# Vegeta2020/SE-SSD

Measured on AMD Instinct MI355X. Metric: KITTI frames/sec (voxelize->backbone->head->NMS), higher is better.
Workload: dtype f32

## Files before the change

### se-ssd_amd/csrc/dense_conv.hip

```cpp
#include "common.hpp"
#include "sessd_hip_types.h"

namespace {

using f32x16 = __attribute__((ext_vector_type(16))) float;

struct ConvArgs {
  const float* in;
  const float* wpk;
  float* out;
  const float* scale;
  const float* shift;
  const float* residual;
  int cin, hin, win;
  int cout, cout_pad, hout, wout;
  int ht, wt;
  int in_mul, out_mul, out_py, out_px;
  int relu;
  int cgroup;
  int dy[9], dx[9];
  int dc[9];
  const int* tile_list;
  const int* n_list;
  int list_cap, ntiles2, tw2, lbatch;
// ... 610 lines not shown
      }
    }
  }
}

template <int NTAPS, int CT, int PT, int WC, int WP, bool DEEP = false>
int launch_conv(const ConvArgs* A, int nconv, int batch, hipStream_t stream) {
  const int npix = A[0].ht * A[0].wt;
  dim3 grid(sessd_divup(npix, WP * PT * 32) * sessd_divup(A[0].cout_pad, WC * CT * 32), 1, batch * (nconv > 1 ? 4 : 1));
  if (nconv == 1) {
    SESSD_LAUNCH((conv2d_mfma_kernel<NTAPS, CT, PT, WC, WP, DEEP>), grid, dim3(256), 0, stream, A[0]);
  } else {
    ConvArgs4 A4;
    for (int i = 0; i < 4; ++i) A4.c[i] = A[i];
    SESSD_LAUNCH((conv2d_mfma4_kernel<NTAPS, CT, PT, WC, WP, DEEP>), grid, dim3(256), 0, stream, A4);
  }
  SESSD_CHECK_LAUNCH();
  return SESSD_OK;
}

template <int CT, int PT, int WC, int WP, bool DEEP>
int launch_conv8(const ConvArgs* A, int batch, hipStream_t stream) {
  const int npix = A[0].ht * A[0].wt;
  const bool list = A[0].tile_list != nullptr;
  dim3 grid(sessd_divup(npix * (list ? batch : 1), WP * PT * 32) * sessd_divup(A[0].cout_pad, WC * CT * 32), 1, (list ? 1 : batch) * 8);
  ConvArgs8 A8;
  for (int i = 0; i < 8; ++i) A8.c[i] = A[i];
  if (list)
    SESSD_LAUNCH((conv2d_mfma8_kernel<4, CT, PT, WC, WP, DEEP, true>), grid, dim3(256), 0, stream, A8);
  else
    SESSD_LAUNCH((conv2d_mfma8_kernel<4, CT, PT, WC, WP, DEEP>), grid, dim3(256), 0, stream, A8);
  SESSD_CHECK_LAUNCH();
  return SESSD_OK;
}

template <int CT, int PT, int WC, int WP, bool DEEP>
int launch_conv_list(const ConvArgs& A, int batch, hipStream_t stream) {
  const int npix = A.ht * A.wt;
  dim3 grid(sessd_divup(npix * batch, WP * PT * 32) * sessd_divup(A.cout_pad, WC * CT * 32), 1, 1);
  SESSD_LAUNCH((conv2d_mfma_kernel<4, CT, PT, WC, WP, DEEP, true>), grid, dim3(256), 0, stream, A);
  SESSD_CHECK_LAUNCH();
  return SESSD_OK;
}

template <int NTAPS>
int dispatch_tile(const ConvArgs* A, int nconv, int batch, int tile_cfg, hipStream_t stream) {
  switch (tile_cfg) {
    case 0: return launch_conv<NTAPS, 2, 2, 2, 2>(A, nconv, batch, stream);
    case 1: return launch_conv<NTAPS, 2, 1, 2, 2>(A, nconv, batch, stream);
    case 2: return launch_conv<NTAPS, 1, 2, 4, 1>(A, nconv, batch, stream);
    case 3: return launch_conv<NTAPS, 1, 1, 4, 1>(A, nconv, batch, stream);
    case 4: return launch_conv<NTAPS, 1, 1, 1, 4>(A, nconv, batch, stream);
    case 5: return launch_conv<NTAPS, 2, 1, 4, 1>(A, nconv, batch, stream);
    case 6: return launch_conv<NTAPS, 2, 1, 1, 4>(A, nconv, batch, stream);
    case 7: return launch_conv<NTAPS, 2, 2, 1, 4>(A, nconv, batch, stream);
    case 8: return launch_conv<NTAPS, 4, 1, 1, 4>(A, nconv, batch, stream);
    case 11: return launch_conv<NTAPS, 1, 1, 1, 4, true>(A, nconv, batch, stream);
    case 12: return launch_conv<NTAPS, 1, 1, 4, 1, true>(A, nconv, batch, stream);
    case 13: if (nconv == 1) return launch_conv<NTAPS, 1, 2, 4, 1, true>(A, nconv, batch, stream); return SESSD_EINVAL;
    default: return SESSD_EINVAL;
  }
}

inline bool out_fits(int cout, int hout, int wout) { return (long long)cout * hout * wout * 4 < 0x7fffffffLL; }

int fill_args(ConvArgs& A, const float* in, int cin, int hin, int win, const float* wpk, int ntaps, const int* dy,
              const int* dx, int in_mul, int tile_h, int tile_w, float* out, int cout, int hout, int wout, int out_mul,
              int py, int px, const float* scale, const float* shift, int relu, const float* residual) {
  A.in = in; A.wpk = wpk; A.out = out; A.scale = scale; A.shift = shift; A.residual = residual;
  A.cin = cin; A.hin = hin; A.win = win;
  A.cout = cout; A.cout_pad = sessd_divup(cout, 32) * 32; A.hout = hout; A.wout = wout;
  A.ht = tile_h; A.wt = tile_w;
  A.in_mul = in_mul; A.out_mul = out_mul; A.out_py = py; A.out_px = px;
  A.relu = relu;
  A.tile_list = nullptr; A.n_list = nullptr; A.list_cap = 0; A.ntiles2 = 1; A.tw2 = 1; A.lbatch = 1;
  int group = 1;
  const int pairs = cin / 2;
  if (ntaps == 1 && pairs % 4 == 0) group = 4;
  else if (ntaps == 2 && pairs % 2 == 0) group = 2;
  A.cgroup = group;
  const int eff = ntaps * group;
  for (int v = 0; v < 9; ++v) {
    const int t = v < eff ? v % ntaps : 0, g = v < eff ? v / ntaps : 0;
    A.dy[v] = dy[t]; A.dx[v] = dx[t]; A.dc[v] = g;
  }
  return eff;
}

}

extern "C" {

int sessd_conv2d_mfma(const float* in, int batch, int cin, int hin, int win, const float* wpk, int ntaps,
                      const int* taps_dy, const int* taps_dx, int in_mul, int tile_h, int tile_w, float* out, int cout,
                      int hout, int wout, int out_mul, int out_py, int out_px, const float* scale, const float* shift,
                      int relu, const float* residual, int tile_cfg, hipStream_t stream) {
  if (cin % 2 || ntaps < 1 || ntaps > 9 || batch < 1 || cout < 1 || !out_fits(cout, hout, wout)) return SESSD_EINVAL;
  ConvArgs A;
  const int eff = fill_args(A, in, cin, hin, win, wpk, ntaps, taps_dy, taps_dx, in_mul, tile_h, tile_w, out, cout, hout,
                            wout, out_mul, out_py, out_px, scale, shift, relu, residual);
  if (tile_cfg == 10) {
    if (eff != 9 || in_mul != 1 || out_mul != 1 || cin % 16 || hin != tile_h || win != tile_w) return SESSD_EINVAL;
    dim3 grid(sessd_divup(tile_h * tile_w, 32), sessd_divup(A.cout_pad, 128), batch);
    SESSD_LAUNCH(conv3x3s1_lds_kernel, grid, dim3(256), 0, stream, A);
    SESSD_CHECK_LAUNCH();
    return SESSD_OK;
  }
  switch (eff) {
    case 1: return dispatch_tile<1>(&A, 1, batch, tile_cfg, stream);
    case 2: return dispatch_tile<2>(&A, 1, batch, tile_cfg, stream);
    case 4: return dispatch_tile<4>(&A, 1, batch, tile_cfg, stream);
    case 9: return dispatch_tile<9>(&A, 1, batch, tile_cfg, stream);
    default: return SESSD_EINVAL;
  }
}

int sessd_conv3x3_winograd(const float* in, int batch, int cin, int h, int w, const float* upk, float* out, int cout,
                           const float* scale, const float* shift, int relu, const float* residual, int variant,
                           hipStream_t stream) {
  if (cin % 8 || (h & 1) || (w & 1) || batch < 1 || cout < 1) return SESSD_EINVAL;
  if (variant < 0 || variant > 1 || (variant == 1 && cin % 32)) return SESSD_EINVAL;
  ConvArgs A;
  const int z9[9] = {0, 0, 0, 0, 0, 0, 0, 0, 0};
  fill_args(A, in, cin, h, w, upk, 9, z9, z9, 1, h, w, out, cout, h, w, 1, 0, 0, scale, shift, relu, residual);
  const int ntiles = (h / 2) * (w / 2);
  dim3 grid(sessd_divup(ntiles, 32) * sessd_divup(A.cout_pad, 32), 1, batch);
  if (variant == 1)
    SESSD_LAUNCH(conv3x3s1_winograd_kernel<true>, grid, dim3(256), 0, stream, A);
  else
    SESSD_LAUNCH(conv3x3s1_winograd_kernel<false>, grid, dim3(256), 0, stream, A);
  SESSD_CHECK_LAUNCH();
  return SESSD_OK;
}

}
namespace {
struct PackArgs {
  const float* w;
  long long so, sc;
  int tap_off[16];
  int co, ci, nt, cp;
};
__global__ __launch_bounds__(256) void pack_taps_kernel(PackArgs A, float* __restrict__ out) {
  const size_t total = (size_t)(A.ci >> 1) * A.nt * 2 * A.cp;
  const size_t idx = (size_t)blockIdx.x * 256 + threadIdx.x;
  if (idx >= total) return;
  const int o = (int)(idx % A.cp);
  size_t r = idx / A.cp;
  const int h = (int)(r & 1); r >>= 1;
  const int t = (int)(r % A.nt);
  const int kp = (int)(r / A.nt);
  out[idx] = o < A.co ? A.w[(long long)o * A.so + (long long)(2 * kp + h) * A.sc + A.tap_off[t]] : 0.f;
}
__device__ __forceinline__ void winograd_pack_body(const PackArgs& A, int flip, int layout, float* __restrict__ out, size_t idx) {
  const int cpad = layout == 0 ? A.cp : ((layout == 1 || layout == 3) ? (A.co + 127) / 128 * 128 : (A.co + 63) / 64 * 64);
  if (idx >= (size_t)cpad * A.ci) return;
  const int o = (int)(idx % cpad), c = (int)(idx / cpad);
  double g[3][3];
#pragma unroll
  for (int a = 0; a < 3; ++a)
#pragma unroll
    for (int b = 0; b < 3; ++b) {
      const int t = flip ? 8 - (3 * a + b) : 3 * a + b;
      g[a][b] = o < A.co ? (double)A.w[(long long)o * A.so + (long long)c * A.sc + t] : 0.0;
    }
  double t0[4][3];
#pragma unroll
  for (int b = 0; b < 3; ++b) {
    t0[0][b] = g[0][b];
    t0[1][b] = 0.5 * g[0][b] + 0.5 * g[1][b] + 0.5 * g[2][b];
    t0[2][b] = 0.5 * g[0][b] - 0.5 * g[1][b] + 0.5 * g[2][b];
    t0[3][b] = g[2][b];
  }
  const int kp = c >> 1, h = c & 1;
#pragma unroll
  for (int a = 0; a < 4; ++a) {
    const double u[4] = {t0[a][0], 0.5 * t0[a][0] + 0.5 * t0[a][1] + 0.5 * t0[a][2], 0.5 * t0[a][0] - 0.5 * t0[a][1] + 0.5 * t0[a][2],
                         t0[a][2]};
#pragma unroll
    for (int b = 0; b < 4; ++b) {
      const int xi = a * 4 + b;
      size_t dst;
      if (layout == 0) {
        dst = ((((size_t)kp * 4 + (xi >> 2)) * 2 + h) * cpad + o) * 4 + (xi & 3);
      } else if (layout == 1) {
        const int grp = o >> 7, cb = (o >> 5) & 3, j = o & 31, wave = xi >> 1, xl = xi & 1;
        dst = ((((((size_t)grp * (A.ci >> 1) + kp) * 8 + wave) * 2 + h) * 32 + j) * 4 + cb) * 2 + xl;
      } else if (layout == 3) {
        const int grp = o >> 7, wave = (o >> 5) & 3, j = o & 31;
        dst = (((((size_t)grp * (A.ci >> 1) + kp) * 4 + wave) * 2 + h) * 32 + j) * 16 + xi;
      } else {
        const int grp = o >> 6, cb = (o >> 5) & 1, j = o & 31, wave = xi >> 2, xl = xi & 3;
        dst = ((((((size_t)grp * (A.ci >> 1) + kp) * 4 + wave) * 2 + h) * 32 + j) * 2 + cb) * 4 + xl;
      }
      out[dst] = (float)u[b];
    }
  }
}
__global__ __launch_bounds__(256) void winograd_pack_kernel(PackArgs A, int flip, int layout, float* __restrict__ out) {
  winograd_pack_body(A, flip, layout, out, (size_t)blockIdx.x * 256 + threadIdx.x);
}
__global__ __launch_bounds__(256) void dense_pack_batch_kernel(const sessd_dense_pack_job_t* __restrict__ jobs, int n) {
  int lo = 0, hi = n - 1;
  while (lo < hi) {
    const int mid = (lo + hi + 1) >> 1;
    if (jobs[mid].block_start <= (int)blockIdx.x) lo = mid; else hi = mid - 1;
  }
  const sessd_dense_pack_job_t* J = jobs + lo;
  const size_t idx = (size_t)((int)blockIdx.x - J->block_start) * 256 + threadIdx.x;
  const int co = J->cout, ci = J->cin, cp = sessd_divup(co, 32) * 32;
  const float* __restrict__ w = J->w;
  float* __restrict__ out = J->out;
  const long long so = J->out_stride, sc = J->in_stride;
  if (J->kind == 0) {
    const int nt = J->ntaps;
    const size_t total = (size_t)(ci >> 1) * nt * 2 * cp;
    if (idx >= total) return;
    const int o = (int)(idx % cp);
    size_t r = idx / cp;
    const int h = (int)(r & 1); r >>= 1;
    const int t = (int)(r % nt);
    const int kp = (int)(r / nt);
    out[idx] = o < co ? w[(long long)o * so + (long long)(2 * kp + h) * sc + J->tap_off[t]] : 0.f;
    return;
  }
  PackArgs A;
  A.w = w; A.so = so; A.sc = sc; A.co = co; A.ci = ci; A.nt = 9; A.cp = cp;
  winograd_pack_body(A, J->flip, J->layout, out, idx);
}
}
extern "C" {

int sessd_dense_pack_batch(const sessd_dense_pack_job_t* jobs_dev, int n_jobs, int total_blocks, hipStream_t stream) {
  if (!jobs_dev || n_jobs < 1 || total_blocks < 1) return SESSD_EINVAL;
  SESSD_LAUNCH(dense_pack_batch_kernel, dim3(total_blocks), dim3(256), 0, stream, jobs_dev, n_jobs);
  SESSD_CHECK_LAUNCH();
  return SESSD_OK;
}

int sessd_conv2d_pack_taps(const float* w, long long out_stride, long long in_stride, const int* tap_offsets, int ntaps, int cout,
                           int cin, float* out, hipStream_t stream) {
  if (ntaps < 1 || ntaps > 16 || cout < 1 || cin < 2 || (cin & 1)) return SESSD_EINVAL;
  PackArgs A;
  A.w = w; A.so = out_stride; A.sc = in_stride; A.co = cout; A.ci = cin; A.nt = ntaps; A.cp = sessd_divup(cout, 32) * 32;
  for (int t = 0; t < 16; ++t) A.tap_off[t] = t < ntaps ? tap_offsets[t] : 0;
  const size_t total = (size_t)(cin >> 1) * ntaps * 2 * A.cp;
  SESSD_LAUNCH(pack_taps_kernel, dim3((unsigned)((total + 255) / 256)), dim3(256), 0, stream, A, out);
  SESSD_CHECK_LAUNCH();
  return SESSD_OK;
}

int sessd_conv3x3_winograd_pack(const float* w, long long out_stride, long long in_stride, int flip, int cout, int cin, int layout,
                                float* out, hipStream_t stream) {
  if (cout < 1 || cin < 2 || (cin & 1) || layout < 0 || layout > 3) return SESSD_EINVAL;
  PackArgs A;
  A.w = w; A.so = out_stride; A.sc = in_stride; A.co = cout; A.ci = cin; A.nt = 9; A.cp = sessd_divup(cout, 32) * 32;
  for (int t = 0; t < 16; ++t) A.tap_off[t] = 0;
  const int cpad = layout == 0 ? A.cp : ((layout == 1 || layout == 3) ? sessd_divup(cout, 128) * 128 : sessd_divup(cout, 64) * 64);
  const size_t total = (size_t)cpad * cin;
  SESSD_LAUNCH(winograd_pack_kernel, dim3((unsigned)((total + 255) / 256)), dim3(256), 0, stream, A, flip, layout, out);
  SESSD_CHECK_LAUNCH();
  return SESSD_OK;
}

}
int sessd_deconv_pair_launch(const float* in, int batch, int cin, int hin, int win, const float* const* wpk4, float* out, int cout,
                             const float* scale, const float* shift, int relu, const float* residual, int variant,
                             hipStream_t stream);
extern "C" {

int sessd_deconv2d_s2_mfma(const float* in, int batch, int cin, int hin, int win, const float* const* wpk4,
                           const int* ntaps4, const int* taps_dy4, const int* taps_dx4, float* out, int cout,
                           const float* scale, const float* shift, int relu, const float* residual, int tile_cfg,
                           hipStream_t stream) {
  if (cin % 8 || batch < 1 || cout < 1 || !out_fits(cout, 2 * hin, 2 * win)) return SESSD_EINVAL;
  if (tile_cfg >= 40 && tile_cfg <= 42) {
    static const int nt[4] = {1, 2, 2, 4};
    static const int dy[16] = {0, 0, 0, 0, 0, 0, 0, 0, 1, 0, 0, 0, 1, 1, 0, 0};
    static const int dx[16] = {0, 0, 0, 0, 1, 0, 0, 0, 0, 0, 0, 0, 1, 0, 1, 0};
    for (int c = 0; c < 4; ++c) {
      if (ntaps4[c] != nt[c]) return SESSD_EINVAL;
      for (int t = 0; t < nt[c]; ++t)
        if (taps_dy4[4 * c + t] != dy[4 * c + t] || taps_dx4[4 * c + t] != dx[4 * c + t]) return SESSD_EINVAL;
    }
    return sessd_deconv_pair_launch(in, batch, cin, hin, win, wpk4, out, cout, scale, shift, relu, residual, tile_cfg - 40, stream);
  }
  ConvArgs A[4];
  for (int c = 0; c < 4; ++c) {
    const int eff = fill_args(A[c], in, cin, hin, win, wpk4[c], ntaps4[c], taps_dy4 + 4 * c, taps_dx4 + 4 * c, 1, hin, win,
                              out, cout, 2 * hin, 2 * win, 2, c >> 1, c & 1, scale, shift, relu, residual);
    if (eff != 4) return SESSD_EINVAL;
  }
  return dispatch_tile<4>(A, 4, batch, tile_cfg, stream);
}

int sessd_deconv2d_s2_mfma_pair(const float* in, int batch, int cin, int hin, int win, const float* const* wpk4_a,
                                const float* const* wpk4_b, const int* ntaps4, const int* taps_dy4, const int* taps_dx4,
                                float* out_a, float* out_b, int cout, const float* scale_a, const float* shift_a,
                                const float* scale_b, const float* shift_b, int relu, const float* residual_a,
                                const float* residual_b, int tile_cfg, hipStream_t stream) {
  if (cin % 8 || batch < 1 || cout < 1 || !out_fits(cout, 2 * hin, 2 * win)) return SESSD_EINVAL;
  ConvArgs A[8];
  for (int c = 0; c < 4; ++c)
    for (int l = 0; l < 2; ++l) {
      const int eff = fill_args(A[2 * c + l], in, cin, hin, win, (l ? wpk4_b : wpk4_a)[c], ntaps4[c], taps_dy4 + 4 * c, taps_dx4 + 4 * c,
                                1, hin, win, l ? out_b : out_a, cout, 2 * hin, 2 * win, 2, c >> 1, c & 1, l ? scale_b : scale_a,
                                l ? shift_b : shift_a, relu, l ? residual_b : residual_a);
      if (eff != 4) return SESSD_EINVAL;
    }
  switch (tile_cfg) {
    case 3: return launch_conv8<1, 1, 4, 1, false>(A, batch, stream);
    case 4: return launch_conv8<1, 1, 1, 4, false>(A, batch, stream);
    case 11: return launch_conv8<1, 1, 1, 4, true>(A, batch, stream);
    case 12: return launch_conv8<1, 1, 4, 1, true>(A, batch, stream);
    default: return SESSD_EINVAL;
  }
}

int sessd_conv2d_mfma_active(const float* in, int batch, int cin, int hin, int win, const float* wpk, int ntaps, const int* taps_dy,
                             const int* taps_dx, int in_mul, int tile_h, int tile_w, float* out, int cout, int hout, int wout,
                             int out_mul, int out_py, int out_px, const float* scale, const float* shift, int relu,
                             const float* residual, const int32_t* tile_list, const int32_t* n_list, int list_cap, int tile_cfg,
                             hipStream_t stream) {
  if (cin % 2 || ntaps < 1 || ntaps > 9 || batch < 1 || cout < 1 || !tile_list || !n_list || list_cap < 1 || (tile_h & 1) || (tile_w & 1))
    return SESSD_EINVAL;
  if ((long long)batch * cout * hout * wout * 4 >= 0x7fffffffLL || (long long)batch * cin * hin * win * 4 >= 0x7fffffffLL) return SESSD_EINVAL;
  ConvArgs A;
  const int eff = fill_args(A, in, cin, hin, win, wpk, ntaps, taps_dy, taps_dx, in_mul, tile_h, tile_w, out, cout, hout, wout, out_mul,
                            out_py, out_px, scale, shift, relu, residual);
  if (eff != 4) return SESSD_EINVAL;
  A.tile_list = tile_list; A.n_list = n_list; A.list_cap = list_cap; A.ntiles2 = (tile_h / 2) * (tile_w / 2); A.tw2 = tile_w / 2;
  A.lbatch = batch;
  switch (tile_cfg) {
    case 3: return launch_conv_list<1, 1, 4, 1, false>(A, batch, stream);
    case 4: return launch_conv_list<1, 1, 1, 4, false>(A, batch, stream);
    case 11: return launch_conv_list<1, 1, 1, 4, true>(A, batch, stream);
    case 12: return launch_conv_list<1, 1, 4, 1, true>(A, batch, stream);
    default: return SESSD_EINVAL;
  }
}

int sessd_deconv2d_s2_mfma_pair_active(const float* in, int batch, int cin, int hin, int win, const float* const* wpk4_a,
                                       const float* const* wpk4_b, const int* ntaps4, const int* taps_dy4, const int* taps_dx4,
                                       float* out_a, float* out_b, int cout, const float* scale_a, const float* shift_a,
                                       const float* scale_b, const float* shift_b, int relu, const float* residual_a,
                                       const float* residual_b, const int32_t* tile_list, const int32_t* n_list, int list_cap,
                                       int tile_cfg, hipStream_t stream) {
  if (cin % 8 || batch < 1 || cout < 1 || !tile_list || !n_list || list_cap < 1 || (hin & 1) || (win & 1)) return SESSD_EINVAL;
  if ((long long)batch * cout * 4 * hin * win * 4 >= 0x7fffffffLL || (long long)batch * cin * hin * win * 4 >= 0x7fffffffLL) return SESSD_EINVAL;
  ConvArgs A[8];
  for (int c = 0; c < 4; ++c)
    for (int l = 0; l < 2; ++l) {
      ConvArgs& C = A[2 * c + l];
      const int eff = fill_args(C, in, cin, hin, win, (l ? wpk4_b : wpk4_a)[c], ntaps4[c], taps_dy4 + 4 * c, taps_dx4 + 4 * c, 1, hin, win,
                                l ? out_b : out_a, cout, 2 * hin, 2 * win, 2, c >> 1, c & 1, l ? scale_b : scale_a,
                                l ? shift_b : shift_a, relu, l ? residual_b : residual_a);
      if (eff != 4) return SESSD_EINVAL;
      C.tile_list = tile_list; C.n_list = n_list; C.list_cap = list_cap; C.ntiles2 = (hin / 2) * (win / 2); C.tw2 = win / 2;
      C.lbatch = batch;
    }
  switch (tile_cfg) {
    case 3: return launch_conv8<1, 1, 4, 1, false>(A, batch, stream);
    case 4: return launch_conv8<1, 1, 1, 4, false>(A, batch, stream);
    case 11: return launch_conv8<1, 1, 1, 4, true>(A, batch, stream);
    case 12: return launch_conv8<1, 1, 4, 1, true>(A, batch, stream);
    default: return SESSD_EINVAL;
  }
}

int sessd_ssfa_fuse(const float* x0, const float* x1, const float* w0, const float* w1, float bn_scale0,
                    float bn_shift0, float bn_scale1, float bn_shift1, int batch, int channels, int num_pixels,
                    float* out, hipStream_t stream) {
  if (batch < 1 || channels < 1 || num_pixels < 1) return SESSD_EINVAL;
  if (channels % 4) return SESSD_EINVAL;
  SESSD_LAUNCH(ssfa_fuse_kernel, dim3(sessd_divup(num_pixels, 64), batch), dim3(256), 0, stream, x0, x1, w0, w1,
                     bn_scale0, bn_shift0, bn_scale1, bn_shift1, channels, num_pixels, out);
  SESSD_CHECK_LAUNCH();
  return SESSD_OK;
}


int sessd_ssfa_fuse_head_keys(const float* x0, const float* x1, const float* w0, const float* w1, float bn_scale0, float bn_shift0,
                              float bn_scale1, float bn_shift1, int batch, int channels, int num_pixels, float* out,
                              const float* head_w, const float* head_b, int nout, float* head_out, float score_thresh,
                              unsigned long long* keys, int key_cap, int* key_count, hipStream_t stream) {
  if (batch < 1 || (channels != 128 && channels != 64) || num_pixels < 1 || nout != 22) return SESSD_EINVAL;
  if ((long long)channels * num_pixels * 4 >= 0x7fffffffLL) return SESSD_EINVAL;
  if ((keys == nullptr) != (key_count == nullptr) || (keys && key_cap < 1)) return SESSD_EINVAL;
  const dim3 grid(sessd_divup(num_pixels, 64), batch);
  if (channels == 128)
    SESSD_LAUNCH((ssfa_fuse_head_kernel<22, 32>), grid, dim3(256), 0, stream, x0, x1, w0, w1, bn_scale0, bn_shift0, bn_scale1,
                 bn_shift1, num_pixels, out, head_w, head_b, head_out, score_thresh, keys, key_cap, key_count);
  else
    SESSD_LAUNCH((ssfa_fuse_head_kernel<22, 16>), grid, dim3(256), 0, stream, x0, x1, w0, w1, bn_scale0, bn_shift0, bn_scale1,
                 bn_shift1, num_pixels, out, head_w, head_b, head_out, score_thresh, keys, key_cap, key_count);
  SESSD_CHECK_LAUNCH();
  return SESSD_OK;
}

int sessd_ssfa_fuse_head(const float* x0, const float* x1, const float* w0, const float* w1, float bn_scale0, float bn_shift0,
                         float bn_scale1, float bn_shift1, int batch, int channels, int num_pixels, float* out,
                         const float* head_w, const float* head_b, int nout, float* head_out, hipStream_t stream) {
  return sessd_ssfa_fuse_head_keys(x0, x1, w0, w1, bn_scale0, bn_shift0, bn_scale1, bn_shift1, batch, channels, num_pixels, out,
                                   head_w, head_b, nout, head_out, 0.f, nullptr, 0, nullptr, stream);
}

}
```

### se-ssd_amd/csrc/dense_wino_sk.hip

```cpp
#include <cstdlib>
#include "common.hpp"

namespace {

using f32x16 = __attribute__((ext_vector_type(16))) float;
using f32x4v = __attribute__((ext_vector_type(4))) float;
using f32x2v = __attribute__((ext_vector_type(2))) float;
typedef unsigned int u32x4g __attribute__((__vector_size__(16)));

typedef __amdgpu_buffer_rsrc_t rsrc_t;
__device__ __forceinline__ rsrc_t make_rsrc(const void* base, unsigned bytes) {
  return __builtin_amdgcn_make_buffer_rsrc(const_cast<void*>(base), (short)0, (int)bytes, 0x00020000);
}
#define SESSD_OOB 0x80000000u
#define SESSD_LDS_BARRIER() asm volatile("s_waitcnt lgkmcnt(0)\n\ts_barrier" ::: "memory")
#define SESSD_SYSTEM_SCOPE 17

__device__ __forceinline__ float sadd(float a, float b) {
  float r;
  asm volatile("v_add_f32 %0, %1, %2" : "=v"(r) : "v"(a), "v"(b));
  return r;
}

struct WinoArgs {
  const float* in;
  const float* upk;
  float* out;
  const float* scale;
  const float* shift;
  const float* residual;
  float* scratch;
  unsigned* counters;
  int cin, hin, win, cout, relu;
  int tw, ntiles, tblocks, ngroups, rpu, total_rounds;
  int bper;
  int ss_stride;
  long long upk_stride;
  const int* tile_list;
  const int* n_list;
  int list_cap, min_rounds, batch;
};

template <int NW, int CBN, int VAR = 0, bool LIST = false>
__global__ __launch_bounds__(NW * 64, 8 / NW) void conv3x3s1_winograd_sk_kernel(WinoArgs A) {
  constexpr int XW = 16 / NW;
  static_assert(XW * CBN == 8, "8 accumulators per wave");
  constexpr int NT = NW * 64;
  constexpr unsigned WSTEP = NW * 2u * 32u * 32u;
  constexpr int VBUF = NW * 1024;
  constexpr int SLOT = CBN * 32 * 32 * 4;
  constexpr int NPT = 1024 / NT;
  constexpr int RING = NW;
  __shared__ __attribute__((aligned(16))) float lds[16384];
  __shared__ int s_last, s_pend;
  const int tid = threadIdx.x, lane = tid & 63;
  const int wave = __builtin_amdgcn_readfirstlane(tid >> 6);
  const int j = lane & 31, h = lane >> 5;
  int G = gridDim.x;
  long long R = A.total_rounds;
  int n_list = 0;
  if constexpr (LIST) {
    n_list = __builtin_amdgcn_readfirstlane(min(A.n_list[0], A.list_cap));
    R = (long long)((n_list + 31) >> 5) * A.ngroups * A.rpu;
    if (R == 0) return;
    if (A.min_rounds < 0) {
      const long long U = R / A.rpu;
      long long g = U / (-A.min_rounds);
      g = g < 1 ? 1 : (g > G ? G : g);
      G = (int)g;
      if ((int)blockIdx.x >= G) return;
    } else {
      long long g = R / A.min_rounds;
      g = g < 1 ? 1 : (g > G ? G : g);
      G = (int)(g >= 8 ? (g & ~7LL) : g);
      if ((G & 7) ? ((int)blockIdx.x >= G) : ((int)(blockIdx.x >> 3) >= (G >> 3))) return;
    }
  }
  const bool whole_units = LIST && A.min_rounds < 0;
  const int w = (whole_units || (G & 7)) ? (int)blockIdx.x : (int)((blockIdx.x & 7) * (G >> 3) + (blockIdx.x >> 3));
  int r = whole_units ? (int)((long long)w * (R / A.rpu) / G) * A.rpu : (int)((long long)w * R / G);
  const int r_stop = whole_units ? (int)((long long)(w + 1) * (R / A.rpu) / G) * A.rpu : (int)((long long)(w + 1) * R / G);
  const int in_plane = A.hin * A.win;
  const size_t out_plane = (size_t)in_plane;
  const unsigned xstep = 2u * (unsigned)in_plane * 4u;
  const unsigned wo = (unsigned)(((wave * 2 + h) * 32 + j) * 32);

  int pend_state = 0, pend_u = 0, pend_first = 0, pend_last = 0, pend_tbase = 0, pend_mbase = 0, pend_b = 0;
#define SESSD_SK_SIGNAL()                                                                          \
  {                                                                                                \
    __builtin_amdgcn_s_waitcnt(0);                                                                 \
    __syncthreads();                                                                               \
    if (tid == 0) {                                                                                \
      const unsigned old = __hip_atomic_fetch_add(A.counters + pend_u, 1u, __ATOMIC_RELAXED, __HIP_MEMORY_SCOPE_AGENT); \
      s_pend = (old == (unsigned)(pend_last - pend_first)) ? 1 : 0;                                \
    }                                                                                              \
    __syncthreads();                                                                               \
    pend_state = s_pend ? 2 : 0;                                                                   \
  }

#define SESSD_SK_FINALIZE(Y, CO, SC, SH)                                                            \
  if (tok && (CO) < e_cout) {                                                                       \
    _Pragma("unroll") for (int a = 0; a < 2; ++a) {                                                 \
      const size_t o = (size_t)(CO) * out_plane + pix + (size_t)a * e_win;                          \
      float v0 = fmaf((Y)[2 * a], (SC), (SH)), v1 = fmaf((Y)[2 * a + 1], (SC), (SH));              \
      if (e_relu) { v0 = fmaxf(v0, 0.f); v1 = fmaxf(v1, 0.f); }                                 \
      if (resb) { v0 += resb[o]; v1 += resb[o + 1]; }                                               \
      *reinterpret_cast<float2*>(outb + o) = make_float2(v0, v1);                                   \
    }                                                                                               \
  }
#define SESSD_SK_FINISH_PENDING()                                                                  \
  {                                                                                                \
    const __attribute__((address_space(4))) WinoArgs* Fp =                                         \
        (const __attribute__((address_space(4))) WinoArgs*)__builtin_amdgcn_kernarg_segment_ptr(); \
    asm volatile("" : "+s"(Fp));                                                                   \
    const int f_set = pend_b / Fp->bper;                                                           \
    const float* f_scale = Fp->scale ? Fp->scale + (size_t)f_set * Fp->ss_stride : nullptr;        \
    const float* f_shift = Fp->shift ? Fp->shift + (size_t)f_set * Fp->ss_stride : nullptr;        \
    const int e_cout = Fp->cout, e_relu = Fp->relu, e_win = Fp->win, f_tw = Fp->tw;                \
    const rsrc_t fr = make_rsrc(Fp->scratch, (unsigned)(2 * G) * SLOT * 4u);                       \
    float* outb = Fp->out + (size_t)pend_b * e_cout * out_plane;                                   \
    const float* resb = Fp->residual ? Fp->residual + (size_t)pend_b * e_cout * out_plane : nullptr; \
    const int tl = tid & 31, col0 = tid >> 5;                                                      \
    int tt = pend_tbase + tl;                                                                      \
    bool tok = tt < Fp->ntiles;                                                                    \
    size_t pix = 0;                                                                                \
    if constexpr (LIST) {                                                                          \
      const int fe = tt < n_list ? Fp->tile_list[tt] : -1;                                         \
      tok = fe >= 0;                                                                               \
      const int fb = tok ? fe / Fp->ntiles : 0;                                                    \
      tt = tok ? fe - fb * Fp->ntiles : 0;                                                         \
      pix = (size_t)fb * e_cout * out_plane;                                                       \
    }                                                                                              \
    const int oty = tok ? tt / f_tw : 0, otx = tok ? tt - (tt / f_tw) * f_tw : 0;                  \
    pix += (size_t)(2 * oty) * e_win + 2 * otx;                                                    \
    _Pragma("unroll 1") for (int cb = 0; cb < CBN; ++cb) {                                         \
      f32x4v ysum[NPT];                                                                            \
      _Pragma("unroll") for (int n = 0; n < NPT; ++n) ysum[n] = 0.f;                               \
      for (int wq = pend_first; wq <= pend_last; ++wq) {                                           \
        const unsigned slot = (unsigned)(2 * wq + (wq == pend_first ? 1 : 0)) * (unsigned)(SLOT * 4); \
        f32x4v p[NPT];                                                                             \
        _Pragma("unroll") for (int n = 0; n < NPT; ++n)                                            \
          p[n] = __builtin_bit_cast(f32x4v, __builtin_amdgcn_raw_buffer_load_b128(                 \
              fr, (int)(slot + (unsigned)(((cb * 32 + col0 + (NT / 32) * n) * 32 + tl) * 16)), 0, SESSD_SYSTEM_SCOPE)); \
        _Pragma("unroll") for (int n = 0; n < NPT; ++n) ysum[n] += p[n];                           \
      }                                                                                            \
      _Pragma("unroll") for (int n = 0; n < NPT; ++n) {                                            \
        const int co = pend_mbase + cb * 32 + col0 + (NT / 32) * n;                                \
        const float scv = (f_scale && co < e_cout) ? f_scale[co] : 1.f, shv = (f_shift && co < e_cout) ? f_shift[co] : 0.f; \
        const float z[4] = {ysum[n].x, ysum[n].y, ysum[n].z, ysum[n].w};                           \
        SESSD_SK_FINALIZE(z, co, scv, shv)                                                         \
      }                                                                                            \
    }                                                                                              \
    if (tid == 0) __hip_atomic_store(Fp->counters + pend_u, 0u, __ATOMIC_RELAXED, __HIP_MEMORY_SCOPE_AGENT); \
    pend_state = 0;                                                                                \
  }

  while (r < r_stop) {
    const int u = __builtin_amdgcn_readfirstlane(r / A.rpu);
    const int r0 = __builtin_amdgcn_readfirstlane(r - u * A.rpu);
    const int r1 = __builtin_amdgcn_readfirstlane(min(r_stop - u * A.rpu, A.rpu));
    r = u * A.rpu + r1;
    const int cg = __builtin_amdgcn_readfirstlane(u % A.ngroups), ub = u / A.ngroups;
    const int tb = LIST ? __builtin_amdgcn_readfirstlane(ub) : __builtin_amdgcn_readfirstlane(ub % A.tblocks);
    const int b = LIST ? 0 : __builtin_amdgcn_readfirstlane(ub / A.tblocks);
    const int t_base = tb * 32, m_base = cg * (CBN * 32);
    const rsrc_t xr = LIST ? make_rsrc(A.in, (unsigned)A.batch * (unsigned)A.cin * (unsigned)in_plane * 4u)
                           : make_rsrc(A.in + (size_t)b * A.cin * in_plane, (unsigned)A.cin * in_plane * 4u);
    const int wset = LIST ? 0 : __builtin_amdgcn_readfirstlane(b / A.bper);
    const rsrc_t wr = make_rsrc(A.upk + (size_t)wset * A.upk_stride + (size_t)cg * (A.cin >> 1) * (WSTEP / 4), (unsigned)(A.cin >> 1) * WSTEP);

    int t = t_base + j;
    bool tlive = t < A.ntiles;
    unsigned img_off = 0;
    if constexpr (LIST) {
      const int e = t < n_list ? A.tile_list[t] : -1;
      tlive = e >= 0;
      const int bl = tlive ? e / A.ntiles : 0;
      t = tlive ? e - bl * A.ntiles : 0;
      img_off = (unsigned)bl * (unsigned)A.cin * (unsigned)in_plane * 4u;
    }
    const int ty = tlive ? t / A.tw : 0, tx = tlive ? t - (t / A.tw) * A.tw : 0;
    const int y0 = 2 * ty - 1, x0 = 2 * tx - 1;
    unsigned ro[4];
#pragma unroll
    for (int q = 0; q < 4; ++q) {
      const int y = y0 + q;
      ro[q] = (tlive && y >= 0 && y < A.hin) ? img_off + (unsigned)((h * in_plane + y * A.win + max(x0, 0)) * 4) : SESSD_OOB;
    }
    const bool mask_l = (tx == 0), mask_r = (tx == A.tw - 1);
    const bool edge = __builtin_amdgcn_ballot_w64(tlive && (mask_l || mask_r)) != 0;
    const int klast = r1 * NW - 1;

    f32x16 acc[XW][CBN];
#pragma unroll
    for (int x = 0; x < XW; ++x)
#pragma unroll
      for (int c = 0; c < CBN; ++c)
#pragma unroll
        for (int q = 0; q < 16; ++q) acc[x][c][q] = 0.f;
    f32x4v pr[4];
    f32x4v ua[RING][2];
    float bv[2][XW];

#define SESSD_SK_LOADP(ROUND)                                                                      \
  {                                                                                                \
    const unsigned xs = (unsigned)(min((ROUND), r1 - 1) * NW + wave) * xstep;                      \
    _Pragma("unroll") for (int q = 0; q < 4; ++q)                                                  \
      pr[q] = __builtin_bit_cast(f32x4v, __builtin_amdgcn_raw_buffer_load_b128(xr, (int)ro[q], (int)xs, 0)); \
  }
#define SESSD_SK_LOADU(SET, KG)                                                                    \
  {                                                                                                \
    const unsigned ws = (unsigned)min((KG), klast) * WSTEP;                                        \
    ua[SET][0] = __builtin_bit_cast(f32x4v, __builtin_amdgcn_raw_buffer_load_b128(wr, (int)wo, (int)ws, 0));        \
    __builtin_amdgcn_sched_barrier(0);                                                             \
    ua[SET][1] = __builtin_bit_cast(f32x4v, __builtin_amdgcn_raw_buffer_load_b128(wr, (int)(wo + 16u), (int)ws, 0)); \
  }
#define SESSD_SK_TRANSFORM(VOFF)                                                                   \
  {                                                                                                \
    if (edge) {                                                                                    \
      _Pragma("unroll") for (int q = 0; q < 4; ++q) {                                              \
        const f32x4v p = pr[q];                                                                    \
        pr[q].x = mask_l ? 0.f : p.x; pr[q].y = mask_l ? p.x : p.y;                                \
        pr[q].z = mask_l ? p.y : p.z; pr[q].w = mask_l ? p.z : (mask_r ? 0.f : p.w);               \
      }                                                                                            \
    }                                                                                              \
    f32x2v tl[4], tr[4];                                                                           \
    if constexpr (VAR & 1) {                                                                       \
      tl[0].x = sadd(pr[0].x, -pr[2].x); tl[0].y = sadd(pr[0].y, -pr[2].y); tr[0].x = sadd(pr[0].z, -pr[2].z); tr[0].y = sadd(pr[0].w, -pr[2].w); \
      tl[1].x = sadd(pr[1].x, pr[2].x); tl[1].y = sadd(pr[1].y, pr[2].y); tr[1].x = sadd(pr[1].z, pr[2].z); tr[1].y = sadd(pr[1].w, pr[2].w); \
      tl[2].x = sadd(pr[2].x, -pr[1].x); tl[2].y = sadd(pr[2].y, -pr[1].y); tr[2].x = sadd(pr[2].z, -pr[1].z); tr[2].y = sadd(pr[2].w, -pr[1].w); \
      tl[3].x = sadd(pr[1].x, -pr[3].x); tl[3].y = sadd(pr[1].y, -pr[3].y); tr[3].x = sadd(pr[1].z, -pr[3].z); tr[3].y = sadd(pr[1].w, -pr[3].w); \
    } else {                                                                                       \
    tl[0] = pr[0].xy - pr[2].xy; tr[0] = pr[0].zw - pr[2].zw;                                      \
    tl[1] = pr[1].xy + pr[2].xy; tr[1] = pr[1].zw + pr[2].zw;                                      \
    tl[2] = pr[2].xy - pr[1].xy; tr[2] = pr[2].zw - pr[1].zw;                                      \
    tl[3] = pr[1].xy - pr[3].xy; tr[3] = pr[1].zw - pr[3].zw;                                      \
    }                                                                                              \
    float* dst = &lds[(VOFF) + wave * 1024 + h * 32 + j];                                          \
    _Pragma("unroll") for (int a = 0; a < 4; ++a) {                                                \
      dst[(a * 4 + 0) * 64] = tl[a].x - tr[a].x;                                                   \
      dst[(a * 4 + 1) * 64] = tl[a].y + tr[a].x;                                                   \
      dst[(a * 4 + 2) * 64] = tr[a].x - tl[a].y;                                                   \
      dst[(a * 4 + 3) * 64] = tl[a].y - tr[a].y;                                                   \
    }                                                                                              \
  }
#define SESSD_SK_READV(P, KS, VOFF)                                                                \
  {                                                                                                \
    const float* vb = &lds[(VOFF) + (KS)*1024 + wave * (XW * 64) + h * 32 + j];                    \
    _Pragma("unroll") for (int x = 0; x < XW; ++x) bv[P][x] = vb[x * 64];                          \
  }
#define SESSD_SK_MMA(SET, P)                                                                       \
  {                                                                                                \
    if constexpr (VAR & 2) __builtin_amdgcn_s_setprio(3);                                          \
    _Pragma("unroll") for (int c = 0; c < CBN; ++c)                                                \
      _Pragma("unroll") for (int x = 0; x < XW; ++x)                                               \
        acc[x][c] = __builtin_amdgcn_mfma_f32_32x32x2f32(ua[SET][(c * XW + x) >> 2][(c * XW + x) & 3], bv[P][x], acc[x][c], 0, 0, 0); \
    if constexpr (VAR & 2) __builtin_amdgcn_s_setprio(0);                                          \
  }
#define SESSD_SK_STEP(KS)                                                                          \
  {                                                                                                \
    SESSD_SK_LOADU(((KS) + RING - 1) & (RING - 1), kg0 + (KS) + RING - 1)                          \
    if ((KS) < NW - 1) SESSD_SK_READV(((KS) + 1) & 1, (KS) + 1, voff)                              \
    __builtin_amdgcn_sched_barrier(0);                                                             \
    SESSD_SK_MMA((KS) & (RING - 1), (KS) & 1)                                                      \
    __builtin_amdgcn_sched_barrier(0);                                                             \
  }
#define SESSD_SK_ROUND()                                                                           \
  {                                                                                                \
    const int kg0 = rr * NW;                                                                       \
    SESSD_SK_LOADP(rr + 1)                                                                         \
    SESSD_SK_READV(0, 0, voff)                                                                     \
    __builtin_amdgcn_sched_barrier(0);                                                             \
    SESSD_SK_STEP(0)                                                                               \
    SESSD_SK_STEP(1)                                                                               \
    SESSD_SK_STEP(2)                                                                               \
    SESSD_SK_STEP(3)                                                                               \
    if constexpr (NW == 8) {                                                                       \
      SESSD_SK_STEP(4)                                                                             \
      SESSD_SK_STEP(5)                                                                             \
      SESSD_SK_STEP(6)                                                                             \
      SESSD_SK_STEP(7)                                                                             \
    }                                                                                              \
    SESSD_SK_TRANSFORM(voff ^ VBUF)                                                                \
    __syncthreads();                                                                               \
    voff ^= VBUF;                                                                                  \
    ++rr;                                                                                          \
  }

    SESSD_SK_LOADP(r0)
    __builtin_amdgcn_sched_barrier(0);
#pragma unroll
    for (int s = 0; s < RING - 1; ++s) {
      SESSD_SK_LOADU(s, r0 * NW + s)
      __builtin_amdgcn_sched_barrier(0);
    }
    SESSD_SK_TRANSFORM(0)
    __syncthreads();
    if (pend_state == 1) {
      if (tid == 0) {
        const unsigned old = __hip_atomic_fetch_add(A.counters + pend_u, 1u, __ATOMIC_RELAXED, __HIP_MEMORY_SCOPE_AGENT);
        s_pend = (old == (unsigned)(pend_last - pend_first)) ? 1 : 0;
      }
      pend_state = 3;
    }
    int voff = 0;
    int rr = r0;
    while (rr < r1) SESSD_SK_ROUND()
#undef SESSD_SK_LOADP
#undef SESSD_SK_LOADU
#undef SESSD_SK_TRANSFORM
#undef SESSD_SK_READV
#undef SESSD_SK_MMA
#undef SESSD_SK_STEP
#undef SESSD_SK_ROUND

    if (pend_state == 3) {
      SESSD_LDS_BARRIER();
      pend_state = s_pend ? 2 : 0;
    }
    const __attribute__((address_space(4))) WinoArgs* Ep =
        (const __attribute__((address_space(4))) WinoArgs*)__builtin_amdgcn_kernarg_segment_ptr();
    asm volatile("" : "+s"(Ep));
    const float* e_scale = Ep->scale ? Ep->scale + (size_t)wset * Ep->ss_stride : nullptr;
    const float* e_shift = Ep->shift ? Ep->shift + (size_t)wset * Ep->ss_stride : nullptr;
    const int e_cout = Ep->cout, e_relu = Ep->relu, e_win = Ep->win, e_tw = Ep->tw, e_ntiles = Ep->ntiles;
    unsigned* e_counter = Ep->counters + u;
    const rsrc_t sr = make_rsrc(Ep->scratch, (unsigned)(2 * G) * SLOT * 4u);
    const bool full = (r0 == 0 && r1 == Ep->rpu);
    float* outb = Ep->out + (size_t)b * e_cout * out_plane;
    const float* resb = Ep->residual ? Ep->residual + (size_t)b * e_cout * out_plane : nullptr;
    const int tl = tid & 31, col0 = tid >> 5;
    int tt = t_base + tl;
    bool tok = tt < e_ntiles;
    size_t pix = 0;
    if constexpr (LIST) {
      const int ee = tt < n_list ? Ep->tile_list[tt] : -1;
      tok = ee >= 0;
      const int eb = tok ? ee / e_ntiles : 0;
      tt = tok ? ee - eb * e_ntiles : 0;
      pix = (size_t)eb * e_cout * out_plane;
    }
    const int oty = tok ? tt / e_tw : 0, otx = tok ? tt - (tt / e_tw) * e_tw : 0;
    pix += (size_t)(2 * oty) * e_win + 2 * otx;
    const int w_first = (int)((((long long)u * Ep->rpu + 1) * G - 1) / R);
    const int w_last = (int)((((long long)u * Ep->rpu + Ep->rpu) * G - 1) / R);
    const unsigned my_slot = (unsigned)(2 * w + (r0 == 0 ? 1 : 0)) * (unsigned)(SLOT * 4);
    bool certain = false;
    unsigned oslot = 0;
    if (!full && w_last == w_first + 1) {
      if (tid == 0) s_last = __hip_atomic_load(e_counter, __ATOMIC_RELAXED, __HIP_MEMORY_SCOPE_AGENT) == 1u ? 1 : 0;
      __syncthreads();
      certain = s_last != 0;
      const int wq = (w == w_first) ? w_last : w_first;
      oslot = (unsigned)(2 * wq + (wq == w_first ? 1 : 0)) * (unsigned)(SLOT * 4);
    }
    const bool writes_out = full || certain;
    f32x4v onext[NPT];
    float scn[NPT], shn[NPT];
#define SESSD_SK_FETCH(CB)                                                                          \
  _Pragma("unroll") for (int n = 0; n < NPT; ++n) {                                                 \
    const int co_ = m_base + (CB)*32 + col0 + (NT / 32) * n;                                        \
    if (certain)                                                                                    \
      onext[n] = __builtin_bit_cast(                                                                \
          f32x4v, __builtin_amdgcn_raw_buffer_load_b128(                                            \
                      sr, (int)(oslot + (unsigned)((((CB)*32 + col0 + (NT / 32) * n) * 32 + tl) * 16)), 0, SESSD_SYSTEM_SCOPE)); \
    else                                                                                            \
      onext[n] = 0.f;                                                                               \
    scn[n] = (writes_out && e_scale && co_ < e_cout) ? e_scale[co_] : 1.f;                          \
    shn[n] = (writes_out && e_shift && co_ < e_cout) ? e_shift[co_] : 0.f;                          \
  }
    SESSD_SK_FETCH(0)
#pragma unroll
    for (int cb = 0; cb < CBN; ++cb) {
      if (cb) SESSD_LDS_BARRIER();
#pragma unroll
      for (int x = 0; x < XW; ++x)
#pragma unroll
        for (int q = 0; q < 16; ++q) {
          const int co = (q & 3) + 8 * (q >> 2) + 4 * h;
          lds[((wave * XW + x) * 32 + co) * 32 + j] = acc[x][cb][q];
        }
      f32x4v other[NPT];
      float sc[NPT], sh[NPT];
#pragma unroll
      for (int n = 0; n < NPT; ++n) { other[n] = onext[n]; sc[n] = scn[n]; sh[n] = shn[n]; }
      if (cb + 1 < CBN) { SESSD_SK_FETCH(cb + 1) }
      SESSD_LDS_BARRIER();
#pragma unroll
      for (int n = 0; n < NPT; ++n) {
        const int col = col0 + (NT / 32) * n;
        float m[16];
#pragma unroll
        for (int x = 0; x < 16; ++x) m[x] = lds[(x * 32 + col) * 32 + tl];
        float q0[4], q1[4];
#pragma unroll
        for (int c = 0; c < 4; ++c) {
          q0[c] = m[0 * 4 + c] + m[1 * 4 + c] + m[2 * 4 + c];
          q1[c] = m[1 * 4 + c] - m[2 * 4 + c] - m[3 * 4 + c];
        }
        float y[4];
        y[0] = q0[0] + q0[1] + q0[2]; y[1] = q0[1] - q0[2] - q0[3];
        y[2] = q1[0] + q1[1] + q1[2]; y[3] = q1[1] - q1[2] - q1[3];
        const int co = m_base + cb * 32 + col;
        if (full) {
          SESSD_SK_FINALIZE(y, co, sc[n], sh[n])
        } else if (certain) {
          const f32x4v o4 = other[n];
          const bool mine_first = (w == w_first);
          float z[4];
          z[0] = mine_first ? (0.f + y[0]) + o4.x : (0.f + o4.x) + y[0];
          z[1] = mine_first ? (0.f + y[1]) + o4.y : (0.f + o4.y) + y[1];
          z[2] = mine_first ? (0.f + y[2]) + o4.z : (0.f + o4.z) + y[2];
          z[3] = mine_first ? (0.f + y[3]) + o4.w : (0.f + o4.w) + y[3];
          SESSD_SK_FINALIZE(z, co, sc[n], sh[n])
        } else {
          f32x4v v;
          v.x = y[0]; v.y = y[1]; v.z = y[2]; v.w = y[3];
          __builtin_amdgcn_raw_buffer_store_b128(__builtin_bit_cast(u32x4g, v), sr,
                                                 (int)(my_slot + (unsigned)(((cb * 32 + col) * 32 + tl) * 16)), 0, SESSD_SYSTEM_SCOPE);
        }
      }
    }
    if (certain) {
      if (tid == 0) __hip_atomic_store(e_counter, 0u, __ATOMIC_RELAXED, __HIP_MEMORY_SCOPE_AGENT);
    } else if (!full) {
      if (pend_state == 2) SESSD_SK_FINISH_PENDING()
      pend_u = u; pend_first = w_first; pend_last = w_last; pend_tbase = t_base; pend_mbase = m_base; pend_b = b;
      pend_state = 1;
    }
#undef SESSD_SK_FETCH
    SESSD_LDS_BARRIER();
  }
  if (pend_state == 1) SESSD_SK_SIGNAL()
  if (pend_state == 2) SESSD_SK_FINISH_PENDING()
#undef SESSD_SK_FINALIZE
#undef SESSD_SK_SIGNAL
#undef SESSD_SK_FINISH_PENDING
}


template <int VAR = 0>
__global__ __launch_bounds__(256, 1) void conv3x3s1_winograd_rk_kernel(WinoArgs A) {
  constexpr int NW = 4, KR = 8, RING = 4;
  constexpr int NT = NW * 64;
  constexpr unsigned WSTEP = 4u * 2u * 32u * 16u * 4u;
  constexpr int VBUF = KR * 1024;
  constexpr int SLOT = 4 * 32 * 32 * 4;
  constexpr int NPT = 1024 / NT;
  __shared__ __attribute__((aligned(16))) float lds[2 * VBUF];
  __shared__ int s_last, s_pend;
  const int tid = threadIdx.x, lane = tid & 63;
  const int wave = __builtin_amdgcn_readfirstlane(tid >> 6);
  const int j = lane & 31, h = lane >> 5;
  const int G = gridDim.x;
  const int w = (G & 7) ? (int)blockIdx.x : (int)((blockIdx.x & 7) * (G >> 3) + (blockIdx.x >> 3));
  const long long R = A.total_rounds;
  int r = (int)((long long)w * R / G);
  const int r_stop = (int)((long long)(w + 1) * R / G);
  const int in_plane = A.hin * A.win;
  const size_t out_plane = (size_t)in_plane;
  const unsigned xstep = 2u * (unsigned)in_plane * 4u;
  const unsigned wo = (unsigned)(((wave * 2 + h) * 32 + j) * 64);

  int pend_state = 0, pend_u = 0, pend_first = 0, pend_last = 0, pend_tbase = 0, pend_mbase = 0, pend_b = 0;
#define SESSD_RK_SIGNAL()                                                                          \
  {                                                                                                \
    __builtin_amdgcn_s_waitcnt(0);                                                                 \
// ... 168 lines not shown
    __builtin_amdgcn_sched_barrier(0);
#pragma unroll
    for (int s = 0; s < RING - 1; ++s) {
      SESSD_RK_LOADU(s, r0 * KR + s)
      __builtin_amdgcn_sched_barrier(0);
    }
    SESSD_RK_TRANSFORM(0, 0)
    SESSD_RK_LOADP(r0, 1)
    __builtin_amdgcn_sched_barrier(0);
    SESSD_RK_TRANSFORM(0, 1)
    __syncthreads();
    if (pend_state == 1) {
      if (tid == 0) {
        const unsigned old = __hip_atomic_fetch_add(A.counters + pend_u, 1u, __ATOMIC_RELAXED, __HIP_MEMORY_SCOPE_AGENT);
        s_pend = (old == (unsigned)(pend_last - pend_first)) ? 1 : 0;
      }
      pend_state = 3;
    }
    int voff = 0;
    int rr = r0;
    while (rr < r1) SESSD_RK_ROUND()
#undef SESSD_RK_LOADP
#undef SESSD_RK_LOADU
#undef SESSD_RK_TRANSFORM
#undef SESSD_RK_READV
#undef SESSD_RK_MMA
#undef SESSD_RK_STEP
#undef SESSD_RK_ROUND

    if (pend_state == 3) {
      SESSD_LDS_BARRIER();
      pend_state = s_pend ? 2 : 0;
    }
    const __attribute__((address_space(4))) WinoArgs* Ep =
        (const __attribute__((address_space(4))) WinoArgs*)__builtin_amdgcn_kernarg_segment_ptr();
    asm volatile("" : "+s"(Ep));
    const float* e_scale = Ep->scale ? Ep->scale + (size_t)wset * Ep->ss_stride : nullptr;
    const float* e_shift = Ep->shift ? Ep->shift + (size_t)wset * Ep->ss_stride : nullptr;
    const int e_cout = Ep->cout, e_relu = Ep->relu, e_win = Ep->win, e_tw = Ep->tw, e_ntiles = Ep->ntiles;
    unsigned* e_counter = Ep->counters + u;
    const rsrc_t sr = make_rsrc(Ep->scratch, (unsigned)(2 * G) * SLOT * 4u);
    const bool full = (r0 == 0 && r1 == Ep->rpu);
    float* outb = Ep->out + (size_t)b * e_cout * out_plane;
    const float* resb = Ep->residual ? Ep->residual + (size_t)b * e_cout * out_plane : nullptr;
    const int tt = t_base + j;
    const bool tok = tt < e_ntiles;
    const int oty = tok ? tt / e_tw : 0, otx = tok ? tt - (tt / e_tw) * e_tw : 0;
    const size_t pix = (size_t)(2 * oty) * e_win + 2 * otx;
    const int w_first = (int)((((long long)u * Ep->rpu + 1) * G - 1) / R);
    const int w_last = (int)((((long long)u * Ep->rpu + Ep->rpu) * G - 1) / R);
    const unsigned my_slot = (unsigned)(2 * w + (r0 == 0 ? 1 : 0)) * (unsigned)(SLOT * 4);
    bool certain = false;
    unsigned oslot = 0;
    if (!full && w_last == w_first + 1) {
      if (tid == 0) s_last = __hip_atomic_load(e_counter, __ATOMIC_RELAXED, __HIP_MEMORY_SCOPE_AGENT) == 1u ? 1 : 0;
      __syncthreads();
      certain = s_last != 0;
      const int wq = (w == w_first) ? w_last : w_first;
      oslot = (unsigned)(2 * wq + (wq == w_first ? 1 : 0)) * (unsigned)(SLOT * 4);
    }
    const bool writes_out = full || certain;
    const int col_base = wave * 32 + 4 * h;
#pragma unroll
    for (int half = 0; half < 2; ++half) {
      float sc[8], sh[8];
      f32x4v other[8];
#pragma unroll
      for (int e = 0; e < 8; ++e) {
        const int q = half * 8 + e;
        const int col = col_base + (q & 3) + 8 * (q >> 2);
        const int co_ = m_base + col;
        sc[e] = (writes_out && e_scale && co_ < e_cout) ? e_scale[co_] : 1.f;
        sh[e] = (writes_out && e_shift && co_ < e_cout) ? e_shift[co_] : 0.f;
        if (certain)
          other[e] = __builtin_bit_cast(f32x4v, __builtin_amdgcn_raw_buffer_load_b128(
                                                    sr, (int)(oslot + (unsigned)((col * 32 + j) * 16)), 0, SESSD_SYSTEM_SCOPE));
        else
          other[e] = 0.f;
      }
#pragma unroll
      for (int e = 0; e < 8; ++e) {
        const int q = half * 8 + e;
        const int col = col_base + (q & 3) + 8 * (q >> 2);
        float q0[4], q1[4];
#pragma unroll
        for (int c = 0; c < 4; ++c) {
          q0[c] = acc[0 * 4 + c][q] + acc[1 * 4 + c][q] + acc[2 * 4 + c][q];
          q1[c] = acc[1 * 4 + c][q] - acc[2 * 4 + c][q] - acc[3 * 4 + c][q];
        }
        float y[4];
        y[0] = q0[0] + q0[1] + q0[2]; y[1] = q0[1] - q0[2] - q0[3];
        y[2] = q1[0] + q1[1] + q1[2]; y[3] = q1[1] - q1[2] - q1[3];
        const int co = m_base + col;
        if (full) {
          SESSD_RK_FINALIZE(y, co, sc[e], sh[e])
        } else if (certain) {
          const f32x4v o4 = other[e];
          const bool mine_first = (w == w_first);
          float z[4];
          z[0] = mine_first ? (0.f + y[0]) + o4.x : (0.f + o4.x) + y[0];
          z[1] = mine_first ? (0.f + y[1]) + o4.y : (0.f + o4.y) + y[1];
          z[2] = mine_first ? (0.f + y[2]) + o4.z : (0.f + o4.z) + y[2];
          z[3] = mine_first ? (0.f + y[3]) + o4.w : (0.f + o4.w) + y[3];
          SESSD_RK_FINALIZE(z, co, sc[e], sh[e])
        } else {
          f32x4v v;
          v.x = y[0]; v.y = y[1]; v.z = y[2]; v.w = y[3];
          __builtin_amdgcn_raw_buffer_store_b128(__builtin_bit_cast(u32x4g, v), sr, (int)(my_slot + (unsigned)((col * 32 + j) * 16)), 0,
                                                 SESSD_SYSTEM_SCOPE);
        }
      }
    }
    if (certain) {
      if (tid == 0) __hip_atomic_store(e_counter, 0u, __ATOMIC_RELAXED, __HIP_MEMORY_SCOPE_AGENT);
    } else if (!full) {
      if (pend_state == 2) SESSD_RK_FINISH_PENDING()
      pend_u = u; pend_first = w_first; pend_last = w_last; pend_tbase = t_base; pend_mbase = m_base; pend_b = b;
      pend_state = 1;
    }
  }
  if (pend_state == 1) SESSD_RK_SIGNAL()
  if (pend_state == 2) SESSD_RK_FINISH_PENDING()
#undef SESSD_RK_FINALIZE
#undef SESSD_RK_SIGNAL
#undef SESSD_RK_FINISH_PENDING
}

int launch_rk(const float* in, int batch, int nsets, int cin, int h, int w, const float* upk, float* out, int cout, const float* scale,
              const float* shift, int relu, const float* residual, void* workspace, size_t workspace_bytes, int workgroups,
              hipStream_t stream) {
  constexpr int SLOT = 4 * 32 * 32 * 4;
  if (cin % 16) return SESSD_EINVAL;
  WinoArgs A;
  A.in = in; A.upk = upk; A.out = out; A.scale = scale; A.shift = shift; A.residual = residual;
  A.cin = cin; A.hin = h; A.win = w; A.cout = cout; A.relu = relu;
  A.tw = w / 2; A.ntiles = (h / 2) * (w / 2); A.tblocks = sessd_divup(A.ntiles, 32); A.ngroups = sessd_divup(cout, 128);
  A.rpu = cin / 16;
  A.bper = batch / nsets; A.ss_stride = nsets > 1 ? cout : 0;
  A.upk_stride = nsets > 1 ? (long long)sessd_divup(cout, 128) * (cin >> 1) * (4 * 2 * 32 * 16) : 0;
  A.tile_list = nullptr; A.n_list = nullptr; A.list_cap = 0; A.min_rounds = 1; A.batch = batch;
  const long long units = (long long)batch * A.tblocks * A.ngroups;
  if (units * A.rpu > 0x7fffffffLL) return SESSD_EINVAL;
  A.total_rounds = (int)(units * A.rpu);
  const size_t need = sessd_align((size_t)units * 4, 256) + (size_t)2 * workgroups * SLOT * 4;
  if (need > workspace_bytes) return SESSD_EWORKSPACE;
  if (workgroups > A.total_rounds) workgroups = A.total_rounds >= 8 ? (A.total_rounds & ~7) : A.total_rounds;
  A.counters = (unsigned*)workspace;
  A.scratch = (float*)((char*)workspace + sessd_align((size_t)units * 4, 256));
  SESSD_LAUNCH((conv3x3s1_winograd_rk_kernel<0>), dim3(workgroups), dim3(256), 0, stream, A);
  SESSD_CHECK_LAUNCH();
  return SESSD_OK;
}

template <int NW, int CBN>
int launch_sk(const float* in, int batch, int nsets, int cin, int h, int w, const float* upk, float* out, int cout, const float* scale,
              const float* shift, int relu, const float* residual, void* workspace, size_t workspace_bytes, int workgroups,
              hipStream_t stream, const int* tile_list = nullptr, const int* n_list = nullptr, int list_cap = 0, int min_rounds = 1) {
  constexpr int SLOT = CBN * 32 * 32 * 4;
  if (cin % (2 * NW)) return SESSD_EINVAL;
  if (tile_list && (nsets != 1 || !n_list || list_cap < 1 || (size_t)batch * cin * h * w * 4 >= 0xFFFFFFFFull)) return SESSD_EINVAL;
  WinoArgs A;
  A.in = in; A.upk = upk; A.out = out; A.scale = scale; A.shift = shift; A.residual = residual;
  A.cin = cin; A.hin = h; A.win = w; A.cout = cout; A.relu = relu;
  A.tw = w / 2; A.ntiles = (h / 2) * (w / 2); A.tblocks = sessd_divup(A.ntiles, 32); A.ngroups = sessd_divup(cout, CBN * 32);
  A.rpu = cin / (2 * NW);
  A.bper = batch / nsets; A.ss_stride = nsets > 1 ? cout : 0;
  A.upk_stride = nsets > 1 ? (long long)sessd_divup(cout, CBN * 32) * (cin >> 1) * (NW * 2 * 32 * 32 / 4) : 0;
  A.tile_list = tile_list; A.n_list = n_list; A.list_cap = list_cap; A.min_rounds = (min_rounds < 0 && tile_list) ? min_rounds : (min_rounds < 1 ? 1 : min_rounds); A.batch = batch;
  const long long units = (long long)batch * A.tblocks * A.ngroups;
  if (units * A.rpu > 0x7fffffffLL) return SESSD_EINVAL;
  A.total_rounds = (int)(units * A.rpu);
  const size_t need = sessd_align((size_t)units * 4, 256) + (size_t)2 * workgroups * SLOT * 4;
  if (need > workspace_bytes) return SESSD_EWORKSPACE;
  if (workgroups > A.total_rounds) workgroups = A.total_rounds >= 8 ? (A.total_rounds & ~7) : A.total_rounds;
  A.counters = (unsigned*)workspace;
  A.scratch = (float*)((char*)workspace + sessd_align((size_t)units * 4, 256));
  if (tile_list) {
    SESSD_LAUNCH((conv3x3s1_winograd_sk_kernel<NW, CBN, 0, true>), dim3(workgroups), dim3(NW * 64), 0, stream, A);
    SESSD_CHECK_LAUNCH();
    return SESSD_OK;
  }
  static const int var = [] { const char* e = getenv("SESSD_WINO_VAR"); return e ? atoi(e) & 3 : 0; }();
  switch (var) {
    case 1: SESSD_LAUNCH((conv3x3s1_winograd_sk_kernel<NW, CBN, 1>), dim3(workgroups), dim3(NW * 64), 0, stream, A); break;
    case 2: SESSD_LAUNCH((conv3x3s1_winograd_sk_kernel<NW, CBN, 2>), dim3(workgroups), dim3(NW * 64), 0, stream, A); break;
    case 3: SESSD_LAUNCH((conv3x3s1_winograd_sk_kernel<NW, CBN, 3>), dim3(workgroups), dim3(NW * 64), 0, stream, A); break;
    default: SESSD_LAUNCH((conv3x3s1_winograd_sk_kernel<NW, CBN, 0>), dim3(workgroups), dim3(NW * 64), 0, stream, A); break;
  }
  SESSD_CHECK_LAUNCH();
  return SESSD_OK;
}

int default_workgroups(int shape, int* out) {
  int dev = 0, cus = 0;
  SESSD_TRY(hipGetDevice(&dev));
  SESSD_TRY(hipDeviceGetAttribute(&cus, hipDeviceAttributeMultiprocessorCount, dev));
  *out = ((shape == 1 ? 2 : 1) * cus) & ~7;
  return *out >= 8 ? SESSD_OK : SESSD_EINVAL;
}

}

extern "C" {

size_t sessd_conv3x3_winograd_sk_workspace_bytes(int batch, int h, int w, int cout, int shape, int workgroups) {
  if (batch < 1 || h < 2 || w < 2 || cout < 1 || workgroups < 0 || shape < 0 || shape > 2) return 0;
  if (workgroups == 0 && default_workgroups(shape, &workgroups) != SESSD_OK) return 0;
  const int cpu = shape == 1 ? 64 : 128;
  const size_t units = (size_t)batch * sessd_divup((h / 2) * (w / 2), 32) * sessd_divup(cout, cpu);
  return sessd_align(units * 4, 256) + (size_t)2 * workgroups * (cpu * 32 * 4) * 4;
}

int sessd_conv3x3_winograd_sk_sets(const float* in, int batch, int nsets, int cin, int h, int w, const float* upk, float* out,
                                   int cout, const float* scale, const float* shift, int relu, const float* residual,
                                   void* workspace, size_t workspace_bytes, int shape, int workgroups, hipStream_t stream) {
  if ((h & 1) || (w & 1) || batch < 1 || nsets < 1 || batch % nsets || cout < 1 || workgroups < 0 || (workgroups & 7) || shape < 0 ||
      shape > 2)
    return SESSD_EINVAL;
  if (workgroups == 0) {
    const int rc = default_workgroups(shape, &workgroups);
    if (rc != SESSD_OK) return rc;
  }
  if (shape == 2)
    return launch_rk(in, batch, nsets, cin, h, w, upk, out, cout, scale, shift, relu, residual, workspace, workspace_bytes, workgroups, stream);
  if (shape == 1)
    return launch_sk<4, 2>(in, batch, nsets, cin, h, w, upk, out, cout, scale, shift, relu, residual, workspace, workspace_bytes, workgroups, stream);
  return launch_sk<8, 4>(in, batch, nsets, cin, h, w, upk, out, cout, scale, shift, relu, residual, workspace, workspace_bytes, workgroups, stream);
}

int sessd_conv3x3_winograd_sk_active(const float* in, int batch, int cin, int h, int w, const float* upk, float* out, int cout,
                                     const float* scale, const float* shift, int relu, const float* residual,
                                     const int32_t* tile_list, const int32_t* n_list, int list_cap, int min_rounds, void* workspace,
                                     size_t workspace_bytes, int shape, int workgroups, hipStream_t stream) {
  if ((h & 1) || (w & 1) || batch < 1 || cout < 1 || workgroups < 0 || (workgroups & 7) || shape < 0 || shape > 1 || !tile_list ||
      !n_list || list_cap < 1)
    return SESSD_EINVAL;
  if (workgroups == 0) {
    const int rc = default_workgroups(shape, &workgroups);
    if (rc != SESSD_OK) return rc;
  }
  if (shape == 1)
    return launch_sk<4, 2>(in, batch, 1, cin, h, w, upk, out, cout, scale, shift, relu, residual, workspace, workspace_bytes, workgroups,
                           stream, tile_list, n_list, list_cap, min_rounds);
  return launch_sk<8, 4>(in, batch, 1, cin, h, w, upk, out, cout, scale, shift, relu, residual, workspace, workspace_bytes, workgroups,
                         stream, tile_list, n_list, list_cap, min_rounds);
}

int sessd_conv3x3_winograd_sk(const float* in, int batch, int cin, int h, int w, const float* upk, float* out, int cout,
                              const float* scale, const float* shift, int relu, const float* residual, void* workspace,
                              size_t workspace_bytes, int shape, int workgroups, hipStream_t stream) {
  return sessd_conv3x3_winograd_sk_sets(in, batch, 1, cin, h, w, upk, out, cout, scale, shift, relu, residual, workspace,
                                        workspace_bytes, shape, workgroups, stream);
}

}
```

### se-ssd_amd/sessd_hip/engine.py

```python
import math

import numpy as np
import torch

from ._lib import lib, check
from . import ops


def _round_up(v, m):
    return (int(v) + m - 1) // m * m


def fold_bn(bn):
    w = bn.weight.detach().float() if bn.weight is not None else torch.ones_like(bn.running_mean)
    b = bn.bias.detach().float() if bn.bias is not None else torch.zeros_like(bn.running_mean)
    scale = w / torch.sqrt(bn.running_var.detach().float() + bn.eps)
    shift = b - bn.running_mean.detach().float() * scale
    return scale.contiguous(), shift.contiguous()


SPMIDDLE_LAYERS = [
    ("subm", 4, 16, 3, 1, 0, "subm0"), ("subm", 16, 16, 3, 1, 0, "subm0"),
    ("conv", 16, 32, 3, 2, 1, None),
    ("subm", 32, 32, 3, 1, 0, "subm1"), ("subm", 32, 32, 3, 1, 0, "subm1"),
    ("conv", 32, 64, 3, 2, 1, None),
    ("subm", 64, 64, 3, 1, 0, "subm2"), ("subm", 64, 64, 3, 1, 0, "subm2"), ("subm", 64, 64, 3, 1, 0, "subm2"),
    ("conv", 64, 64, 3, 2, [0, 1, 1], None),
    ("subm", 64, 64, 3, 1, 0, "subm3"), ("subm", 64, 64, 3, 1, 0, "subm3"), ("subm", 64, 64, 3, 1, 0, "subm3"),
    ("conv", 64, 64, (3, 1, 1), (2, 1, 1), 0, None),
]


def _t3(v):
    return [int(v)] * 3 if isinstance(v, int) else [int(x) for x in v]


class SparsePlan:

    def __init__(self, convs, bns, layers, device):
        self.layers = []
        for (kind, cin, cout, ks, st, pd, key), conv, bn in zip(layers, convs, bns):
            w = conv.weight.detach().to(device=device, dtype=torch.float32).contiguous()
            assert tuple(w.shape[-2:]) == (cin, cout), (w.shape, cin, cout)
            scale, shift = fold_bn(bn)
            self.layers.append(dict(kind=kind, cin=cin, cout=cout, ks=_t3(ks), st=_t3(st), pd=_t3(pd), key=key,
                                    wpk=ops.sparse_pack_weight(w), scale=scale.to(device), shift=shift.to(device)))


def active_tile_constants(neck):
    b0, b1 = neck.bottom_up_block_0, neck.bottom_up_block_1
    def step(seq, ci, bi, c):
        s_, t_ = fold_bn(seq[bi])
        return torch.relu(s_.double().cpu() * (seq[ci].weight.detach().double().cpu().sum((2, 3)) @ c) + t_.double().cpu())
    def dstep(seq, c):
        s_, t_ = fold_bn(seq[1])
        w = seq[0].weight.detach().double().cpu()
        K = {0: [1], 1: [0, 2]}
        rows = []
        for py in (0, 1):
            for px in (0, 1):
                ws = sum(w[:, :, ky, kx] for ky in K[py] for kx in K[px])
                rows.append(torch.relu(s_.double().cpu() * (c @ ws) + t_.double().cpu()))
        return torch.stack(rows)
    c = torch.zeros(b0[1].weight.shape[1], dtype=torch.float64)
    chain = []
    for seq, ci, bi in ((b0, 1, 2), (b0, 4, 5), (b0, 7, 8), (b1, 0, 1), (b1, 3, 4), (b1, 6, 7)):
        c = step(seq, ci, bi, c)
        chain.append(c)
    chain += [step(neck.trans_0, 0, 1, chain[2]), step(neck.trans_1, 0, 1, chain[5])]
    chain.append((dstep(neck.deconv_block_0, chain[7]) + chain[6][None], dstep(neck.deconv_block_1, chain[7])))
    def pstep(seq, cpar):
        s_, t_ = fold_bn(seq[1])
        w = seq[0].weight.detach().double().cpu()
        rows = []
        for py in (0, 1):
            for px in (0, 1):
                acc = sum(w[:, :, ky, kx] @ cpar[((py + ky - 1) & 1) * 2 + ((px + kx - 1) & 1)] for ky in range(3) for kx in range(3))
                rows.append(torch.relu(s_.double().cpu() * acc + t_.double().cpu()))
        return torch.stack(rows)
    chain.append((pstep(neck.conv_0, chain[8][0]), pstep(neck.conv_1, chain[8][1])))
    return chain


class DensePlan:

    def __init__(self, neck, head_task, device):
        def cbr(seq, ci, bi, deconv=False):
            conv, bn = seq[ci], seq[bi]
            w = conv.weight.detach().to(device)
            pc = ops.pack_deconv2d_s2(w) if deconv else ops.pack_conv2d(w, conv.stride[0])
            s, t = fold_bn(bn)
            return pc, s.to(device), t.to(device)

        b0, b1 = neck.bottom_up_block_0, neck.bottom_up_block_1
        self.b0 = [cbr(b0, 1, 2), cbr(b0, 4, 5), cbr(b0, 7, 8)]
        chain = active_tile_constants(neck)
        self.act_const = [v.float().to(device).contiguous() for v in chain[:8]]
        self.act_const.append((chain[8][0].float().to(device).contiguous(), chain[8][1].float().to(device).contiguous()))
        self.act_const.append((chain[9][0].float().to(device).contiguous(), chain[9][1].float().to(device).contiguous()))
        self.b1 = [cbr(b1, 0, 1), cbr(b1, 3, 4), cbr(b1, 6, 7)]
        self.trans_0 = cbr(neck.trans_0, 0, 1)
        self.trans_1 = cbr(neck.trans_1, 0, 1)
        self.deconv_0 = cbr(neck.deconv_block_0, 0, 1, True)
        self.deconv_1 = cbr(neck.deconv_block_1, 0, 1, True)
        self.conv_0 = cbr(neck.conv_0, 0, 1)
        self.conv_1 = cbr(neck.conv_1, 0, 1)
        self.w0 = neck.w_0[0].weight.detach().to(device).reshape(-1).float().contiguous()
        self.w1 = neck.w_1[0].weight.detach().to(device).reshape(-1).float().contiguous()
        s0, t0 = fold_bn(neck.w_0[1])
        s1, t1 = fold_bn(neck.w_1[1])
        self.wbn = (float(s0), float(t0), float(s1), float(t1))
        hw = torch.cat([head_task.conv_box.weight, head_task.conv_cls.weight, head_task.conv_dir.weight,
                        head_task.conv_iou.weight], 0).detach().to(device)
        hb = torch.cat([head_task.conv_box.bias, head_task.conv_cls.bias, head_task.conv_dir.bias,
                        head_task.conv_iou.bias], 0).detach().to(device).float().contiguous()
        assert hw.shape[0] == 22, "engine supports the single-task car head (14+2+4+2 channels)"
        self.head = (ops.pack_conv2d(hw), None, hb)
        self.head_w = hw.reshape(22, -1).float().contiguous()
        self.head_b = hb


class InferenceEngine:
    def __init__(self, model, voxel_range, voxel_size, max_points_per_voxel, max_voxels, test_cfg, batch_size=1,
                 max_points_per_frame=32768, device=None, growth=(1.5, 1.0, 0.75, 0.75), anchors=None,
                 use_frustum=False, allow_winograd=True, sort_sites=False, sort_tiles=False, active_tiles=True):
        self.dev = torch.device("cuda:0") if device is None else device
        dev = self.dev
        self.B = int(batch_size)
        self.max_voxels = int(max_voxels)
        self.max_points = int(max_points_per_voxel)
        self.P_cap = _round_up(max_points_per_frame, 256)
        self.vrange = torch.tensor(voxel_range, dtype=torch.float32)
        self.vsize = torch.tensor(voxel_size, dtype=torch.float32)
        self.grid = torch.round((self.vrange[3:] - self.vrange[:3]) / self.vsize).to(torch.int32)
        gx, gy, gz = [int(v) for v in self.grid]
        self.sparse_shape = [gz + 1, gy, gx]
        convs = [m for m in model.backbone.middle_conv if hasattr(m, "indice_key")]
        bns = [m for m in model.backbone.middle_conv if isinstance(m, torch.nn.BatchNorm1d)]
        self.sp = SparsePlan(convs, bns, SPMIDDLE_LAYERS, dev)
        self.dn = DensePlan(model.neck, model.bbox_head.tasks[0], dev)
        nms = test_cfg["nms"] if isinstance(test_cfg, dict) else test_cfg.nms
        self.score_thresh = float(test_cfg["score_threshold"])
        self.pre_max = int(nms["nms_pre_max_size"])
        self.post_max = int(nms["nms_post_max_size"])
        self.nms_thresh = float(nms["nms_iou_threshold"])
        self.post_range = torch.tensor([float(v) for v in test_cfg["post_center_limit_range"]], dtype=torch.float32)
        self.dir_offset = float(getattr(model.bbox_head, "direction_offset", 0.0))
        self.use_frustum = use_frustum
        self.allow_winograd = allow_winograd
        B = self.B
        self.levels = []
        shape = list(self.sparse_shape)
        cap = _round_up(B * self.max_voxels, 64)
        self.levels.append(dict(shape=shape, hash_dims=[gz, gy, gx], cap=cap))
        if isinstance(growth, (int, float)):
            growth = (growth,) * 4
        gi = 0
        for (kind, cin, cout, ks, st, pd, key) in SPMIDDLE_LAYERS:
            if kind == "conv":
                ks3, st3, pd3 = _t3(ks), _t3(st), _t3(pd)
                shape = [(d + 2 * p - k) // s + 1 for d, k, s, p in zip(shape, ks3, st3, pd3)]
                cells = B * shape[0] * shape[1] * shape[2]
                cap = _round_up(min(int(growth[gi] * cap), cells), 64)
                gi += 1
                self.levels.append(dict(shape=shape, hash_dims=shape, cap=cap))
        self.bev_c = 64 * self.levels[-1]["shape"][0]
        self.H, self.W = self.levels[-1]["shape"][1], self.levels[-1]["shape"][2]
        H, W = self.H, self.W
        f32, i32 = torch.float32, torch.int32
        E = lambda *s, dt=f32: torch.empty(s, dtype=dt, device=dev)
        self.points = torch.full((B, self.P_cap, 4), -1.0e6, dtype=f32, device=dev)
        cap0 = self.levels[0]["cap"]
# ... 111 lines not shown
        self.allow_offset_split = True
        self.sk_workgroups = 0
        self.cu_budget = 0
        self.tune_report = {}
        self._tuning = None
        self._kmarks = None
        self.sparse_split = {}
        self.sparse_sorted = {}
        self._tuning_sparse = None

    def _i3(self, v):
        key = tuple(_t3(v))
        t = self._ks.get(key)
        if t is None:
            t = torch.tensor(key, dtype=torch.int32)
            self._ks[key] = t
        return t

    def _wgs(self, shape):
        if self.sk_workgroups:
            return self.sk_workgroups
        if not self.cu_budget:
            return 0
        return max(8, ((2 if shape == 1 else 1) * int(self.cu_budget)) & ~7)

    def _wgs_cfg(self, cfg):
        return self._wgs(1 if cfg == 23 else (2 if cfg == 30 else 0))

    def set_points(self, points_list, frustum=None):
        assert len(points_list) == self.B
        for b, p in enumerate(points_list):
            n = p.shape[0]
            if n > self.P_cap:
                raise ValueError("frame has %d points, engine capacity is %d" % (n, self.P_cap))
            if p.dtype != torch.float32 or not p.is_contiguous() or p.shape[1] != 4 or not p.is_cuda:
                raise ValueError("points must be contiguous (P,4) float32 device tensors")
            check(lib.sessd_stage_points(p.data_ptr(), n, self.points[b].data_ptr(), self.P_cap,
                                         torch.cuda.current_stream().cuda_stream), "stage_points")
        if frustum is not None and self.frustum is not None:
            self.frustum.copy_(frustum.reshape(self.frustum.shape), non_blocking=True)

    def _n(self, li):
        L = self.levels[li]
        return self.prefix.data_ptr() + 4 * self.B if li == 0 else L["n"].data_ptr()

    def _sconv(self, lay, in_feat, nbr, tm, out_li, out_feat, s, dense=False, idx=None):
        Lo = self.levels[out_li]
        kv = lay["ks"][0] * lay["ks"][1] * lay["ks"][2]
        dd = self._i3(Lo["shape"]).data_ptr() if dense else 0
        perm = 0
        if self.chain.sort_tiles and self.sparse_sorted.get(idx, True):
            j = self._job_of[idx]
            if self.chain.nbr[j] is nbr:
                tm, perm = self.chain.tile_mask_sorted[j], self.chain.perm[j].data_ptr()
        check(lib.sessd_sparse_conv_sorted(in_feat.data_ptr(), lay["cin"], nbr.data_ptr(), tm.data_ptr(), kv, self._n(out_li),
                                           Lo["cap"], lay["wpk"].data_ptr(), lay["scale"].data_ptr(), lay["shift"].data_ptr(), 1,
                                           0 if dense else out_feat.data_ptr(), lay["cout"],
                                           Lo["indices"].data_ptr() if dense else 0, self.bev.data_ptr() if dense else 0, dd,
                                           self.sparse_split.get(idx, 0), perm, s), "sparse_conv_sorted")
        if self._tuning_sparse is not None and not dense:
            self._tuning_sparse.append((idx, lay, in_feat, nbr, tm, out_li, out_feat))

    def _branch_sets(self, shape):
        key = "_sets%d" % shape
        if not hasattr(self, key):
            d = self.dn
            (p0, s0, t0), (p1, s1, t1) = d.conv_0, d.conv_1
            u0, u1 = p0.upk_sk(shape), p1.upk_sk(shape)
            ok = u0 is not None and u1 is not None and p0.cout == p1.cout == 128 and p0.cin == p1.cin and s0 is not None and s1 is not None
            need = int(lib.sessd_conv3x3_winograd_sk_workspace_bytes(2 * self.B, self.H, self.W, 128, shape, 0)) if ok else 0
            if ok and self.sk_ws is not None and self.sk_ws.numel() < need:
                self.sk_ws = torch.zeros(need, dtype=torch.uint8, device=self.dev)
            setattr(self, key, dict(upk=torch.cat([u0.reshape(-1), u1.reshape(-1)]), scale=torch.stack([s0, s1]).contiguous(),
                                    shift=torch.stack([t0, t1]).contiguous()) if ok else None)
        return getattr(self, key)

    NEAR_READER = {0: 1, 1: 2, 3: 4, 4: 5}

    def _fill_jobs(self, ids):
        outs, vals, slots, tiles, near, kinds = [], [], [], [], [], []
        ids = list(ids)
        for l in ids:
            if l in (self.ACTIVE_PAIR, self.ACTIVE_CONV):
                for o, v in zip(self.ACTIVE_SLOTS[l][3], self.dn.act_const[l]):
                    outs.append(o); vals.append(v); slots.append(self.ACTIVE_MASK[l]); tiles.append(4 if l == self.ACTIVE_PAIR else 6)
                    near.append(None); kinds.append(0)
                continue
            nr, kind = None, 0
            if self.near_fill:
                rd = self.NEAR_READER.get(l)
                if rd is not None and rd in ids and rd not in self.ACTIVE_SK:
                    nr = self.ACTIVE_MASK[rd]
                elif self.coarse_fill and l == 2 and 3 in ids and 6 in ids:
                    nr, kind = self.ACTIVE_MASK[3], 2
                elif self.coarse_fill and l == 6 and self.ACTIVE_PAIR in ids:
                    nr, kind = self.ACTIVE_MASK[self.ACTIVE_PAIR], 1
                elif self.coarse_fill and l == 5 and 7 in ids:
                    continue
            outs.append(self.ACTIVE_SLOTS[l][3]); vals.append(self.dn.act_const[l]); slots.append(self.ACTIVE_MASK[l]); tiles.append(2)
            near.append(nr); kinds.append(kind)
        return outs, vals, slots, tiles, near, kinds

    def _active_layers(self):
        if self.ta is None or self._tuning is not None or self.sk_ws is None:
            return []
        return sorted(self.active_cfg)

    def _conv(self, x, layer, out, relu=True, residual=None, name=None, active=None):
        pc, scale, shift = layer
        if active is not None:
            shape, min_rounds = self.active_cfg[active]
            m = self.ACTIVE_MASK[active]
            if active in self.ACTIVE_SK and shape != 30:
                call = lambda: ops.conv2d_mfma_active(x, pc, scale, shift, relu, out, self.ta.tile_list[m], self.ta.n_list[m:m + 1],
                                                      tile_cfg=shape, residual=residual)
            elif active in self.ACTIVE_SK:
                call = lambda: ops.conv2d_sk_active(x, pc, scale, shift, relu, out, self.sk_ws, self.ta.tile_list[m],
                                                    self.ta.n_list[m:m + 1], workgroups=self._wgs(2), residual=residual,
                                                    min_rounds=min_rounds)
            else:
                call = lambda: ops.conv2d_winograd_sk_active(x, pc.upk_sk(shape), pc.cout, scale, shift, relu, out, shape, self.sk_ws,
                                                             self.ta.tile_list[m], self.ta.n_list[m:m + 1],
                                                             workgroups=self._wgs(shape), residual=residual, min_rounds=min_rounds)
            if self._kmarks is not None:
                e0, e1 = torch.cuda.Event(enable_timing=True), torch.cuda.Event(enable_timing=True)
                e0.record()
                r = call()
                e1.record()
                self._kmarks.append((name, e0, e1))
                return r
            return call()
        if self._tuning is not None:
            self._tuning.append((name, x, layer, out, relu, residual))
        if self._kmarks is not None:
            e0, e1 = torch.cuda.Event(enable_timing=True), torch.cuda.Event(enable_timing=True)
            e0.record()
            r = ops.conv2d(x, pc, scale, shift, relu, residual, out, self.tile_cfg.get(name), workspace=self.sk_ws, workgroups=self._wgs_cfg(self.tile_cfg.get(name)))
            e1.record()
            self._kmarks.append((name, e0, e1))
            return r
        return ops.conv2d(x, pc, scale, shift, relu, residual, out, self.tile_cfg.get(name), workspace=self.sk_ws, workgroups=self._wgs_cfg(self.tile_cfg.get(name)))

    def adopt_tuning(self, other):
        self.tile_cfg = dict(other.tile_cfg)
        self.active_cfg = dict(other.active_cfg) if self.ta is not None else {}
        self.sparse_split = dict(other.sparse_split)
        self.sparse_sorted = dict(other.sparse_sorted)
        self.sk_workgroups = other.sk_workgroups
        self.cu_budget = other.cu_budget
        self.merge_branch_convs = other.merge_branch_convs
        self.sk_ws = torch.zeros_like(other.sk_ws) if other.sk_ws is not None else None

    DEFAULT_ACTIVE_CFG = {0: (1, 4), 1: (0, 1), 2: (1, 2), 3: (30, 4), 4: (1, 2), 5: (0, 1), 6: (11, 0), 7: (30, 8), 8: (4, 0), 9: (0, 8)}

    def force_active_tiles(self, active_cfg=None):
        if self.ta is None:
            raise RuntimeError("this engine has no tile-activity program (active_tiles=False or an unsupported BEV size)")
        self.tile_cfg.update({"b0.0": 22, "b0.1": 22, "b0.2": 23, "b1.0": 30, "b1.1": 23, "b1.2": 22, "trans_0": 30, "trans_1": 30,
                              "conv_0": 22, "conv_1": 22})
        B = self.B
        need = max([int(lib.sessd_conv3x3_winograd_sk_workspace_bytes(2 * B, self.H, self.W, 256, sh, 0)) for sh in (0, 1)] +
                   [int(lib.sessd_conv2d_sk_workspace_bytes(B, self.H, self.W, 256, 1, 0))])
        if self.sk_ws is None or self.sk_ws.numel() < need:
            self.sk_ws = torch.zeros(need, dtype=torch.uint8, device=self.dev)
        self.active_cfg = dict(self.DEFAULT_ACTIVE_CFG if active_cfg is None else active_cfg)
        return self.active_cfg

    def autotune(self, candidates=(1, 2, 3, 4, 6, 11, 12), reps=5):
        self._tuning, self._tuning_sparse = [], []
        self.enqueue()
        torch.cuda.synchronize()
        todo, self._tuning = self._tuning, None
        todo_sp, self._tuning_sparse = self._tuning_sparse, None
        st = torch.cuda.current_stream().cuda_stream
        for idx, lay, in_feat, nbr, tm, out_li, out_feat in todo_sp:
            best = (None, 1e30)
            cands = [(a, b, c) for c in ((0, 1) if self.allow_offset_split else (0,)) for a in (1, 2, 4) for b in (2, 3, 4)]
            cands += [(a, 2, 2) for a in (1, 2, 4)]
            if self.levels[out_li]["cap"] >= 65536 or getattr(self, "sparse_mt_candidates", False):
                cands += [(a, b, c) for c in (16, 32) for a in (1, 2, 4) for b in (2, 3)]
            for split, depth, ks in cands:
                if (lay["cout"] // 16) % split or (ks == 1 and depth == 4):
                    continue
                for srt in ((True, False) if self.chain.sort_tiles else (False,)):
                    self.sparse_split[idx] = split + 256 * depth + 65536 * ks
                    self.sparse_sorted[idx] = srt
                    for _ in range(2):
                        self._sconv(lay, in_feat, nbr, tm, out_li, out_feat, st, idx=idx)
                    e0, e1 = torch.cuda.Event(enable_timing=True), torch.cuda.Event(enable_timing=True)
                    e0.record()
                    for _ in range(reps):
                        self._sconv(lay, in_feat, nbr, tm, out_li, out_feat, st, idx=idx)
                    e1.record()
                    torch.cuda.synchronize()
                    t = e0.elapsed_time(e1) / reps
                    if t < best[1]:
                        best = (split + 256 * depth + 65536 * ks + (1 << 24 if srt else 0), t)
            self.sparse_split[idx] = best[0] & 0xFFFFFF
            self.sparse_sorted[idx] = bool(best[0] >> 24)
            self.tune_report["sparse%d" % idx] = best
        for idx, (tun, srt) in getattr(self, "force_sparse", {}).items():
            if tun is not None:
                self.sparse_split[idx] = int(tun)
            if srt is not None and self.chain.sort_tiles:
                self.sparse_sorted[idx] = bool(srt)
        for name, x, layer, out, relu, residual in todo:
            pc, scale, shift = layer
            best = (None, 1e30)
            cands = list(candidates)
            if pc.kind == "conv" and pc.stride == 1 and pc.launches[0]["ntaps"] == 9 and pc.cin % 16 == 0:
                cands.append(10)
                if getattr(pc, "upk", None) is not None and x.shape[2] % 2 == 0 and x.shape[3] % 2 == 0 and self.allow_winograd:
                    cands.append(20)
                    if pc.cin % 32 == 0:
                        cands.append(21)
                    for cfg, shape in ((22, 0), (23, 1)) if self.allow_streamk else ():
                        if pc.upk_sk(shape) is not None:
                            need = int(lib.sessd_conv3x3_winograd_sk_workspace_bytes(x.shape[0], x.shape[2], x.shape[3], pc.cout, shape, 0))
                            if self.sk_ws is None or self.sk_ws.numel() < need:
                                self.sk_ws = torch.zeros(need, dtype=torch.uint8, device=x.device)
                            cands.append(cfg)
            if self.allow_streamk and pc.cout > 32 and not (pc.kind == "conv" and pc.stride == 1 and pc.launches[0]["ntaps"] == 9) \
                    and pc.sk_args() is not None:
                th, tw = (out.shape[2], out.shape[3]) if pc.kind == "conv" else (x.shape[2], x.shape[3])
                need = int(lib.sessd_conv2d_sk_workspace_bytes(x.shape[0], th, tw, pc.cout, len(pc.launches), 0))
                if self.sk_ws is None or self.sk_ws.numel() < need:
                    self.sk_ws = torch.zeros(need, dtype=torch.uint8, device=x.device)
                cands.append(30)
            if pc.kind == "deconv":
                cands += [40, 41, 42]
            for cfg in cands:
                if pc.cout <= 32 and cfg != 4:
                    continue
                if cfg == 13 and pc.kind != "conv":
                    continue
                for _ in range(2):
                    ops.conv2d(x, pc, scale, shift, relu, residual, out, cfg, workspace=self.sk_ws, workgroups=self._wgs_cfg(cfg))
                e0, e1 = torch.cuda.Event(enable_timing=True), torch.cuda.Event(enable_timing=True)
                e0.record()
                for _ in range(reps):
                    ops.conv2d(x, pc, scale, shift, relu, residual, out, cfg, workspace=self.sk_ws, workgroups=self._wgs_cfg(cfg))
                e1.record()
                torch.cuda.synchronize()
                t = e0.elapsed_time(e1) / reps
                if t < best[1]:
                    best = (cfg, t)
            self.tile_cfg[name] = best[0]
            self.tune_report[name] = best
        self._autotune_active_tiles(reps)
        self.enqueue()
        torch.cuda.synchronize()
        return self.tune_report

    def _autotune_active_tiles(self, reps):
        self.active_cfg = {}
        if self.ta is None or not self.allow_streamk or not self.allow_winograd:
            return
        def timed(fn, n=reps):
            for _ in range(2):
                fn()
            e0, e1 = torch.cuda.Event(enable_timing=True), torch.cuda.Event(enable_timing=True)
            e0.record()
            for _ in range(n):
                fn()
            e1.record()
            torch.cuda.synchronize()
            return e0.elapsed_time(e1) / n
        L4, d = self.levels[-1], self.dn
        self.ta.run(L4["indices"], L4["n"], L4["cap"])
        pick, gain, pair_dense_t, special_dense = {}, 0.0, 0.0, {}
        t = self.t
        for l, (name, layer, x_in, x_out) in self.ACTIVE_SLOTS.items():
            best = (None, 1e30)
            m = self.ACTIVE_MASK[l]
            if l == self.ACTIVE_PAIR:
                (pa, sa, ta_), (pb, sb, tb_) = layer
                tr0 = t["tr0"]
                cd0, cd1 = self.tile_cfg.get("deconv_0"), self.tile_cfg.get("deconv_1")
                if self.merge_branch_convs and cd0 in (3, 4, 11, 12) and cd1 in (3, 4, 11, 12):
                    dense_t = timed(lambda: ops.deconv2d_s2_pair(x_in, pa, pb, sa, ta_, sb, tb_, True, x_out[0], x_out[1], residual_a=tr0,
                                                                 tile_cfg=cd0))
                else:
                    dense_t = self.tune_report.get("deconv_0", (None, 0.0))[1] + self.tune_report.get("deconv_1", (None, 0.0))[1]
                for cfg in (3, 4, 11, 12):
                    tt = timed(lambda: ops.deconv2d_s2_pair_active(x_in, pa, pb, sa, ta_, sb, tb_, True, x_out[0], x_out[1],
                                                                   self.ta.tile_list[m], self.ta.n_list[m:m + 1], residual_a=tr0,
                                                                   tile_cfg=cfg))
                    if tt < best[1]:
                        best = ((cfg, 0), tt)
                pair_dense_t = dense_t
                if best[1] < dense_t:
                    pick[l] = best
                    gain += dense_t - best[1]
                continue
            if l == self.ACTIVE_CONV and not self.allow_active_conv:
                continue
            if l == self.ACTIVE_CONV:
                (p0, s0, t0_), (p1, s1, t1_) = layer
                c01 = self.tile_cfg.get("conv_0")
                if self.merge_branch_convs and c01 in (22, 23, 24) and self.tile_cfg.get("conv_1") == c01 and self._branch_sets(c01 - 22) is not None:
                    sets = self._branch_sets(c01 - 22)
                    dense_t = timed(lambda: ops.conv2d_winograd_sk_sets(t["mid"], sets["upk"], 2, 128, sets["scale"], sets["shift"], True, t["o"],
                                                                        c01 - 22, self.sk_ws, self._wgs(c01 - 22)))
                else:
                    dense_t = self.tune_report.get("conv_0", (None, 0.0))[1] + self.tune_report.get("conv_1", (None, 0.0))[1]
                for shape in (0, 1):
                    if p0.upk_sk(shape) is None or p1.upk_sk(shape) is None:
                        continue
                    need = int(lib.sessd_conv3x3_winograd_sk_workspace_bytes(self.B, self.H, self.W, p0.cout, shape, 0))
                    if self.sk_ws is None or self.sk_ws.numel() < need:
                        self.sk_ws = torch.zeros(need, dtype=torch.uint8, device=self.dev)
                    for mr in (4, 8, 16, -1):
                        def both(shape=shape, mr=mr):
                            for (pc_, sc_, sh_), xi, xo in ((layer[0], x_in[0], x_out[0]), (layer[1], x_in[1], x_out[1])):
                                ops.conv2d_winograd_sk_active(xi, pc_.upk_sk(shape), pc_.cout, sc_, sh_, True, xo, shape, self.sk_ws,
                                                              self.ta.tile_list[m], self.ta.n_list[m:m + 1], workgroups=self._wgs(shape), min_rounds=mr)
                        tt = timed(both)
                        if tt < best[1]:
                            best = ((shape, mr), tt)
                special_dense[l] = dense_t
                if best[0] is not None and best[1] < dense_t:
                    pick[l] = best
                    gain += dense_t - best[1]
                continue
            pc, scale, shift = layer
            if l in self.ACTIVE_SK:
                if pc.launches[0]["ntaps"] == 1 and pc.cin % 8 == 0:
                    for cfg in (3, 4, 11, 12):
                        tt = timed(lambda: ops.conv2d_mfma_active(x_in, pc, scale, shift, True, x_out, self.ta.tile_list[m],
                                                                  self.ta.n_list[m:m + 1], tile_cfg=cfg))
                        if tt < best[1]:
                            best = ((cfg, 0), tt)
                if pc.sk_args() is not None:
                    need = int(lib.sessd_conv2d_sk_workspace_bytes(self.B, x_out.shape[2], x_out.shape[3], pc.cout, len(pc.launches), 0))
                    if self.sk_ws is None or self.sk_ws.numel() < need:
                        self.sk_ws = torch.zeros(need, dtype=torch.uint8, device=self.dev)
                    for mr in (1, 4, 8, 16):
                        tt = timed(lambda: ops.conv2d_sk_active(x_in, pc, scale, shift, True, x_out, self.sk_ws, self.ta.tile_list[m],
                                                                self.ta.n_list[m:m + 1], workgroups=self._wgs(2), min_rounds=mr))
                        if tt < best[1]:
                            best = ((30, mr), tt)
            else:
                for shape in (0, 1):
                    if pc.upk_sk(shape) is None:
                        continue
                    need = int(lib.sessd_conv3x3_winograd_sk_workspace_bytes(self.B, x_in.shape[2], x_in.shape[3], pc.cout, shape, 0))
                    if self.sk_ws is None or self.sk_ws.numel() < need:
                        self.sk_ws = torch.zeros(need, dtype=torch.uint8, device=self.dev)
                    for mr in self.list_share_candidates:
                        tt = timed(lambda: ops.conv2d_winograd_sk_active(x_in, pc.upk_sk(shape), pc.cout, scale, shift, True, x_out, shape,
                                                                         self.sk_ws, self.ta.tile_list[m], self.ta.n_list[m:m + 1],
                                                                         workgroups=self._wgs(shape), min_rounds=mr))
                        if tt < best[1]:
                            best = ((shape, mr), tt)
            dense_t = self.tune_report.get(name, (None, 0.0))[1]
            if best[0] is not None and best[1] < dense_t:
                pick[l] = best
                gain += dense_t - best[1]
        def overhead(ids):
            fj = self._fill_jobs(ids)
            return timed(lambda: (self.ta.run(L4["indices"], L4["n"], L4["cap"]), self.ta.fill(fj[0], fj[1], layers=fj[2], tiles=fj[3], near=fj[4], near_kind=fj[5])),
                         4 * reps)
        sl = sorted(pick)
        over = overhead(sl) if pick else 0.0
        for l in (self.ACTIVE_CONV, self.ACTIVE_PAIR, 7, 6):
            if l in pick and len(pick) > 1:
                rest = [q for q in sl if q != l]
                over_wo = overhead(rest)
                g = (special_dense[l] if l in special_dense else
                     self.tune_report.get(self.ACTIVE_SLOTS[l][0], (None, 0.0))[1] if l != self.ACTIVE_PAIR else pair_dense_t) - pick[l][1]
                if over - over_wo >= g:
                    del pick[l]
                    sl, over, gain = rest, over_wo, gain - g
        if pick and gain > over:
            self.active_cfg = {l: pick[l][0] for l in pick}
        self.tune_report["active_tiles"] = ({self.ACTIVE_SLOTS[l][0]: v for l, v in self.active_cfg.items()}, gain - over, over,
                                            {self.ACTIVE_SLOTS[l][0]: pick[l][1] for l in pick})

    def set_list_shares(self, mode):
        for l, (shape, mr) in list(self.active_cfg.items()):
            if l in self.ACTIVE_SK or l in (self.ACTIVE_PAIR, self.ACTIVE_CONV):
                continue
            if mode == "whole":
                self.active_cfg[l] = (shape, -1)
            elif mode == "cut" and mr < 0:
                self.active_cfg[l] = (shape, 4)

    def active_tile_fractions(self):
        act = self._active_layers()
        if not act:
            return {}
        n = self.ta.n_list.cpu().numpy()
        M = self.ACTIVE_MASK
        return {self.ACTIVE_SLOTS[l][0]: float(n[M[l]]) / (self.B * (self.ta.dims[M[l]][0] // 2) * (self.ta.dims[M[l]][1] // 2)) for l in act}

    def enqueue(self, part=None):
        s = torch.cuda.current_stream().cuda_stream
        B = self.B
        if part == "back":
            return self._enqueue_body(s, "back")
        if self.cu_budget and (self.fork_front or self.fork_active):
            raise RuntimeError("fork_front / fork_active put part of the frame on an unmasked side stream: not available to an engine "
                               "that runs on a CU set (cu_budget = %d)" % self.cu_budget)
        ops.fill_multi([(self.zero_arena, 0), (self.arena, 0x7F7F7F7F), (self.bev, 0)])
        lib.sessd_set_external_clear(1)
        try:
            return self._enqueue_body(s, part)
        finally:
            lib.sessd_set_external_clear(0)

    def _enqueue_body(self, s, part=None):
        B = self.B
        forked_active = False
        if part != "back":
            if self.batched_voxelizer:
                check(lib.sessd_voxelize_frames(self.points.data_ptr(), B, self.P_cap, 4, self.vrange.data_ptr(), self.vsize.data_ptr(),
                                                self.grid.data_ptr(), self.max_points, self.max_voxels, self.hash0.keys.data_ptr(),
                                                self.hash0.vals.data_ptr(), self.hash0.capacity, self.voxels.data_ptr(),
                                                self.coors.data_ptr(), 4, self.nump.data_ptr(), self.vfeat.data_ptr(),
                                                self.prefix.data_ptr(), self.vox_ws.data_ptr(), self.vox_ws.numel(), s), "voxelize_frames")
            else:
                for b in range(B):
                    check(lib.sessd_voxelize_frame(self.points[b].data_ptr(), self.P_cap, 4, self.vrange.data_ptr(),
                                                   self.vsize.data_ptr(), self.grid.data_ptr(), self.max_points, self.max_voxels,
                                                   b, self.hash0.keys.data_ptr(), self.hash0.vals.data_ptr(), self.hash0.capacity,
                                                   self.voxels.data_ptr(), self.coors.data_ptr(), 4, self.nump.data_ptr(),
                                                   self.vfeat.data_ptr(), self.prefix.data_ptr(), self.vox_ws.data_ptr(),
                                                   self.vox_ws.numel(), s), "voxelize_frame")
            feat = self.vfeat
            if self.sort_sites:
                check(lib.sessd_sparse_renumber_sites(self.coors.data_ptr(), self._n(0), self.levels[0]["cap"], B,
                                                      self._hash0_dims.data_ptr(), self.vfeat.data_ptr(), 4,
                                                      self.hash0.keys.data_ptr(), self.hash0.vals.data_ptr(), self.hash0.capacity,
                                                      self.coors_s.data_ptr(), self.vfeat_s.data_ptr(), self.renum_ws.data_ptr(),
                                                      self.renum_ws.numel(), s), "sparse_renumber_sites")
                feat = self.vfeat_s
            self._mark("voxelize")
            L0 = self.levels[0]
            n_layers = len(self.sp.layers)
            lead = 0
            while lead < n_layers and self.sp.layers[lead]["kind"] == "subm":
                lead += 1
            lead_jobs = 1 + max([self._job_of[i] for i in range(lead)] + [-1])
            fork = self.fork_front and lead > 0 and self._tuning_sparse is None and self._marks is None
            forked_active = False

            def run_layers(lo, hi, feat, li, st):
                for idx in range(lo, hi):
                    lay = self.sp.layers[idx]
                    last = idx == n_layers - 1
                    j = self._job_of[idx]
                    nbr, tm = self.chain.nbr[j], self.chain.tile_mask[j]
                    if lay["kind"] == "subm":
                        L = self.levels[li]
                        out = L["feat_a"] if feat is not L["feat_a"] else L["feat_b"]
                        self._sconv(lay, feat, nbr, tm, li, out, st, idx=idx)
                        feat = out
                    else:
                        Lo = self.levels[li + 1]
                        if last:
                            self._sconv(lay, feat, nbr, tm, li + 1, None, st, dense=True, idx=idx)
                        else:
                            self._sconv(lay, feat, nbr, tm, li + 1, Lo["feat_a"], st, idx=idx)
                            feat = Lo["feat_a"]
                        li += 1
                return feat, li

            if fork:
                main = torch.cuda.current_stream()
                side = self.side_stream
                side.wait_stream(main)
                with torch.cuda.stream(side):
                    s2 = side.cuda_stream
                    self.chain.run_rulebooks(L0["indices"], self._n(0), L0["cap"], L0["hash"], 0, lead_jobs, stream=s2)
                    feat, li = run_layers(0, lead, feat, 0, s2)
                self.chain.run_sites(L0["indices"], self._n(0), L0["cap"], self.err, clear=False, stream=s)
                self.chain.run_rulebooks(L0["indices"], self._n(0), L0["cap"], L0["hash"], lead_jobs, len(self.chain.jobs), stream=s)
                main.wait_stream(side)
                feat, li = run_layers(lead, n_layers, feat, li, s)
            else:
                self.chain.run(L0["indices"], self._n(0), L0["cap"], L0["hash"], self.err, clear=False, stream=s)
                forked_active = self.fork_active and self._marks is None and self._kmarks is None and bool(self._active_layers())
                if forked_active:
                    main, side = torch.cuda.current_stream(), self.side_stream
                    side.wait_stream(main)
                    with torch.cuda.stream(side):
                        L4 = self.levels[-1]
                        self.ta.run(L4["indices"], L4["n"], L4["cap"])
                        fj = self._fill_jobs(self._active_layers())
                        self.ta.fill(fj[0], fj[1], layers=fj[2], tiles=fj[3], near=fj[4], near_kind=fj[5])
                feat, li = run_layers(0, n_layers, feat, 0, s)
                if forked_active:
                    main.wait_stream(side)
        if part != "back":
            self._mark("spmiddle")
        t, h, d = self.t, self.h, self.dn
        act = self._active_layers()
        if act and not forked_active and part != "back":
            L4 = self.levels[-1]
            if self._kmarks is not None:
                e0, e1 = torch.cuda.Event(enable_timing=True), torch.cuda.Event(enable_timing=True)
                e0.record()
            self.ta.run(L4["indices"], L4["n"], L4["cap"])
            fj = self._fill_jobs(act)
            self.ta.fill(fj[0], fj[1], layers=fj[2], tiles=fj[3], near=fj[4], near_kind=fj[5])
            if self._kmarks is not None:
                e1.record()
                self._kmarks.append(("tile_activity+fill", e0, e1))
        if part == "front":
            return self.out
        x = self._conv(self.bev, d.b0[0], t["a"], name="b0.0", active=0 if 0 in act else None)
        x = self._conv(x, d.b0[1], t["b"], name="b0.1", active=1 if 1 in act else None)
        x0 = self._conv(x, d.b0[2], t["x0"], name="b0.2", active=2 if 2 in act else None)
        y = self._conv(x0, d.b1[0], h["a"], name="b1.0", active=3 if 3 in act else None)
        y = self._conv(y, d.b1[1], h["b"], name="b1.1", active=4 if 4 in act else None)
        x1 = self._conv(y, d.b1[2], h["x1"], name="b1.2", active=5 if 5 in act else None)
        tr0 = self._conv(x0, d.trans_0, t["tr0"], name="trans_0", active=6 if 6 in act else None)
        tr1 = self._conv(x1, d.trans_1, h["tr1"], name="trans_1", active=7 if 7 in act else None)
        cd = self.tile_cfg.get("deconv_0")
        if self.ACTIVE_PAIR in act:
            (pa, sa, ta), (pb, sb, tb) = d.deconv_0, d.deconv_1
            mp = self.ACTIVE_MASK[self.ACTIVE_PAIR]
            if self._kmarks is not None:
                e0, e1 = torch.cuda.Event(enable_timing=True), torch.cuda.Event(enable_timing=True)
                e0.record()
            ops.deconv2d_s2_pair_active(tr1, pa, pb, sa, ta, sb, tb, True, t["mid0"], t["mid1"], self.ta.tile_list[mp],
                                        self.ta.n_list[mp:mp + 1], residual_a=tr0, tile_cfg=self.active_cfg[self.ACTIVE_PAIR][0])
            if self._kmarks is not None:
                e1.record()
                self._kmarks.append(("deconv_0+deconv_1", e0, e1))
            mid0, mid1 = t["mid0"], t["mid1"]
        elif self.merge_branch_convs and cd in (3, 4, 11, 12) and self.tile_cfg.get("deconv_1") in (3, 4, 11, 12) and self._tuning is None:
            (pa, sa, ta), (pb, sb, tb) = d.deconv_0, d.deconv_1
            if self._kmarks is not None:
                e0, e1 = torch.cuda.Event(enable_timing=True), torch.cuda.Event(enable_timing=True)
                e0.record()
            ops.deconv2d_s2_pair(tr1, pa, pb, sa, ta, sb, tb, True, t["mid0"], t["mid1"], residual_a=tr0, tile_cfg=cd)
            if self._kmarks is not None:
                e1.record()
                self._kmarks.append(("deconv_0+deconv_1", e0, e1))
            mid0, mid1 = t["mid0"], t["mid1"]
        else:
            mid0 = self._conv(tr1, d.deconv_0, t["mid0"], residual=tr0, name="deconv_0")
            mid1 = self._conv(tr1, d.deconv_1, t["mid1"], name="deconv_1")
        c01 = self.tile_cfg.get("conv_0")
        if self.ACTIVE_CONV in act:
            shape, mr = self.active_cfg[self.ACTIVE_CONV]
            mc = self.ACTIVE_MASK[self.ACTIVE_CONV]
            if self._kmarks is not None:
                e0, e1 = torch.cuda.Event(enable_timing=True), torch.cuda.Event(enable_timing=True)
                e0.record()
            for (pc, sc, sh), xin, xout in ((d.conv_0, mid0, t["o0"]), (d.conv_1, mid1, t["o1"])):
                ops.conv2d_winograd_sk_active(xin, pc.upk_sk(shape), pc.cout, sc, sh, True, xout, shape, self.sk_ws, self.ta.tile_list[mc],
                                              self.ta.n_list[mc:mc + 1], workgroups=self._wgs(shape), min_rounds=mr)
            if self._kmarks is not None:
                e1.record()
                self._kmarks.append(("conv_0+conv_1", e0, e1))
            o0, o1 = t["o0"], t["o1"]
        elif self.merge_branch_convs and c01 in (22, 23, 24) and self.tile_cfg.get("conv_1") == c01 and self._tuning is None \
                and self.sk_ws is not None and self._branch_sets(c01 - 22) is not None:
            sets = self._branch_sets(c01 - 22)
            if self._kmarks is not None:
                e0, e1 = torch.cuda.Event(enable_timing=True), torch.cuda.Event(enable_timing=True)
                e0.record()
            ops.conv2d_winograd_sk_sets(t["mid"], sets["upk"], 2, 128, sets["scale"], sets["shift"], True, t["o"], c01 - 22,
                                        self.sk_ws, self._wgs(c01 - 22))
            if self._kmarks is not None:
                e1.record()
                self._kmarks.append(("conv_0+conv_1", e0, e1))
            o0, o1 = t["o0"], t["o1"]
        else:
            o0 = self._conv(mid0, d.conv_0, t["o0"], name="conv_0")
            o1 = self._conv(mid1, d.conv_1, t["o1"], name="conv_1")
        fused_keys = False
        if self.fuse_head and d.head_w.shape[1] in (64, 128) and self._tuning is None:
            if self._kmarks is not None:
                e0, e1 = torch.cuda.Event(enable_timing=True), torch.cuda.Event(enable_timing=True)
                e0.record()
            fused_keys = True
            ops.ssfa_fuse_head(o0, o1, d.w0, d.w1, *d.wbn, d.head_w, d.head_b, head_out=self.head,
                               out=t["out"] if self.keep_ssfa else None, score_thresh=self.score_thresh,
                               keys=self.keys if self.fuse_predict else None, key_count=self.key_count if self.fuse_predict else None)
            if self._kmarks is not None:
                e1.record()
                self._kmarks.append(("ssfa_tail+head", e0, e1))
        else:
            ops.ssfa_fuse(o0, o1, d.w0, d.w1, *d.wbn, out=t["out"])
            self._conv(t["out"], d.head, self.head.view(B, 22, self.H, self.W), relu=False, name="head")
        self._mark("ssfa_head")
        use_keys = fused_keys and self.fuse_predict
        rec = self.records is not None
        check(lib.sessd_predict_fused(self.head.data_ptr(), B, self.H * self.W, self.anchors.data_ptr(), 0,
                                      0 if self.frustum is None else self.frustum.data_ptr(), self.score_thresh, self.pre_max,
                                      self.post_max, self.nms_thresh, self.post_range.data_ptr(), self.dir_offset,
                                      self.out["box"].data_ptr(), self.out["score"].data_ptr(), self.out["label"].data_ptr(),
                                      self.out["count"].data_ptr(), self.keys.data_ptr() if use_keys else 0,
                                      self.key_count.data_ptr() if use_keys else 0,
                                      self.records.data_ptr() if rec else 0, self.record_counts.data_ptr() if rec else 0,
                                      self.records.shape[0] if rec else 0, self.record_cursor.data_ptr() if rec else 0,
                                      self.pred_ws.data_ptr(), self.pred_ws.numel(), s), "predict_fused")
        self._mark("predict")
        return self.out

    def attach_records(self, capacity_frames):
        cap = max(int(capacity_frames), self.B)
        self.records = torch.zeros((cap, self.post_max, 9), dtype=torch.float32, device=self.dev)
        self.record_counts = torch.zeros((cap,), dtype=torch.int32, device=self.dev)
        self.record_cursor = torch.zeros((1,), dtype=torch.int32, device=self.dev)
        return self.records, self.record_counts

    def _mark(self, name):
        if self._marks is not None:
            ev = torch.cuda.Event(enable_timing=True)
            ev.record()
            self._marks.append((name, ev))

    def stage_times(self, reps=10):
        acc = {}
        for _ in range(2):
            self.enqueue()
        for _ in range(reps):
            self._marks = []
            e0 = torch.cuda.Event(enable_timing=True)
            e0.record()
            self.enqueue()
            marks, self._marks = self._marks, None
            torch.cuda.synchronize()
            prev = e0
            for name, ev in marks:
                acc[name] = acc.get(name, 0.0) + prev.elapsed_time(ev) / reps
                prev = ev
        return acc

    def spmiddle_algorithmic_bytes(self):
        ns = [int(self.prefix[self.B].item())] + [int(L["n"].item()) for L in self.levels[1:]]
        total, li = 0, 0
        for lay in self.sp.layers:
            kv = lay["ks"][0] * lay["ks"][1] * lay["ks"][2]
            n_in = ns[li]
            if lay["kind"] != "subm":
                li += 1
            n_out = ns[li]
            total += (n_in * lay["cin"] + n_out * lay["cout"]) * 4 + kv * lay["cin"] * lay["cout"] * 4 + (n_in + n_out) * 16
        total -= ns[-1] * self.sp.layers[-1]["cout"] * 4
        total += self.bev.numel() * 4
        return total, ns

    def dense_layer_times(self, reps=10):
        acc = {}
        for _ in range(2):
            self.enqueue()
        for _ in range(reps):
            self._kmarks = []
            self.enqueue()
            marks, self._kmarks = self._kmarks, None
            torch.cuda.synchronize()
            for name, e0, e1 in marks:
                acc[name] = acc.get(name, 0.0) + e0.elapsed_time(e1) / reps
        return acc

    def spmiddle_mfma_report(self, reps=10):
        self._tuning_sparse = []
        self.enqueue()
        torch.cuda.synchronize()
        todo, self._tuning_sparse = self._tuning_sparse, None
        ns = [int(self.prefix[self.B].item())] + [int(L["n"].item()) for L in self.levels[1:]]
        st = torch.cuda.current_stream().cuda_stream
        rows, tot_ms, tot_use, tot_exe = [], 0.0, 0.0, 0.0
        last_idx = len(self.sp.layers) - 1
        jl = self._job_of[last_idx]
        todo = list(todo) + [(last_idx, self.sp.layers[last_idx], None, self.chain.nbr[jl], self.chain.tile_mask[jl], len(self.levels) - 1, None)]
        feat_last = None
        for idx, lay, in_feat, nbr, tm, out_li, out_feat in todo:
            n = ns[out_li]
            kv = lay["ks"][0] * lay["ks"][1] * lay["ks"][2]
            pairs = int((nbr[:kv, :n] >= 0).sum().item())
            srt = bool(self.chain.sort_tiles and self.sparse_sorted.get(idx, True))
            masks = self.chain.tile_mask_sorted[self._job_of[idx]] if srt else tm[:(n + 15) // 16]
            steps = int(sum(int(((masks >> k) & 1).sum().item()) for k in range(kv)))
            if in_feat is None:
                in_feat, dense = feat_last, True
            else:
                dense = False
            for _ in range(2):
                self._sconv(lay, in_feat, nbr, tm, out_li, out_feat, st, dense=dense, idx=idx)
            e0, e1 = torch.cuda.Event(enable_timing=True), torch.cuda.Event(enable_timing=True)
            e0.record()
            for _ in range(reps):
                self._sconv(lay, in_feat, nbr, tm, out_li, out_feat, st, dense=dense, idx=idx)
            e1.record()
            torch.cuda.synchronize()
            ms = e0.elapsed_time(e1) / reps
            use, exe = 2.0 * pairs * lay["cin"] * lay["cout"] / 1e9, 2.0 * steps * 16 * lay["cin"] * lay["cout"] / 1e9
            rows.append(dict(layer=idx, kind=lay["kind"], cin=lay["cin"], cout=lay["cout"], sites=n, pairs=pairs, tile_steps=steps,
                             sorted_tiles=srt,
                             ms=round(ms, 5), useful_gflop=round(use, 4), executed_gflop=round(exe, 4),
                             executed_tflops=round(exe / ms, 2) if ms > 0 else 0.0))
            tot_ms, tot_use, tot_exe = tot_ms + ms, tot_use + use, tot_exe + exe
            feat_last = out_feat if out_feat is not None else feat_last
        self.enqueue()
        torch.cuda.synchronize()
        return dict(layers=rows, conv_ms=round(tot_ms, 5), useful_gflop=round(tot_use, 3), executed_gflop=round(tot_exe, 3),
                    executed_tflops=round(tot_exe / tot_ms, 2), executed_frac_of_f32_mfma_peak=round(tot_exe / tot_ms / 157.3, 4),
                    useful_row_fraction=round(tot_use / tot_exe, 4))

    def capture(self, warmup=2, split=False):
        side = torch.cuda.Stream()
        side.wait_stream(torch.cuda.current_stream())
        with torch.cuda.stream(side):
            for _ in range(warmup):
                self.enqueue()
        torch.cuda.current_stream().wait_stream(side)
# ... 37 lines not shown
```

### se-ssd_amd/sessd_hip/ops.py

```python
import os

import torch

from ._lib import lib, check, SessdError


def _stream():
    return torch.cuda.current_stream().cuda_stream


def _p(t):
    return 0 if t is None else t.data_ptr()


def _req(t, dtype, name):
    if not t.is_cuda:
        raise ValueError("%s must be a CUDA (HIP) tensor: the SE-SSD hot path has no CPU fallback" % name)
    if t.dtype != dtype:
        raise TypeError("%s must be %s, got %s" % (name, dtype, t.dtype))
    if not t.is_contiguous():
        raise ValueError("%s must be contiguous" % name)
    return t


# ... 437 lines not shown
            ks, st, pd = _t3(ks), _t3(st), _t3(pd)
            shp = [(d + 2 * p - k) // s + 1 for d, k, s, p in zip(shp, ks, st, pd)]
            for d in range(3):
                lv[l].ksize[d], lv[l].stride[d], lv[l].pad[d], lv[l].out_dims[d] = ks[d], st[d], pd[d], shp[d]
            lv[l].cap = int(cap)
        return int(lib.sessd_sparse_chain_workspace_bytes(int(batch), len(steps), lv))

    def bind_tables(self, n0_cap):
        for j, (li, lo, ks) in enumerate(self._job_spec):
            cap = int(n0_cap) if lo == 0 else self.caps[lo - 1]
            kv = ks[0] * ks[1] * ks[2]
            self.nbr[j] = torch.empty((kv, cap), dtype=torch.int32, device=self.dev)
            self.tile_mask[j] = torch.empty(((cap + 15) // 16,), dtype=torch.int32, device=self.dev)
            self.jobs[j].nbr, self.jobs[j].tile_mask = self.nbr[j].data_ptr(), self.tile_mask[j].data_ptr()
            if self.sort_tiles:
                groups = (cap + 255) // 256
                self.site_mask[j] = torch.zeros((cap,), dtype=torch.int32, device=self.dev)
                self.perm[j] = torch.zeros((groups * 256,), dtype=torch.uint8, device=self.dev)
                self.tile_mask_sorted[j] = torch.zeros((groups * 16,), dtype=torch.int32, device=self.dev)
                self.jobs[j].site_mask, self.jobs[j].perm = self.site_mask[j].data_ptr(), self.perm[j].data_ptr()
                self.jobs[j].tile_mask_sorted = self.tile_mask_sorted[j].data_ptr()

    def run(self, indices0, n0_dev_ptr, n0_cap, hash0, err_flag, clear=True, stream=None):
        self.run_sites(indices0, n0_dev_ptr, n0_cap, err_flag, clear, stream)
        self.run_rulebooks(indices0, n0_dev_ptr, n0_cap, hash0, 0, len(self.jobs), stream)

    def run_sites(self, indices0, n0_dev_ptr, n0_cap, err_flag, clear=True, stream=None):
        s = _stream() if stream is None else stream
        if self.nbr and self.nbr[0] is None:
            self.bind_tables(n0_cap)
        check(lib.sessd_sparse_chain_sites(indices0.data_ptr(), n0_dev_ptr, int(n0_cap), self.batch, len(self.levels),
                                           self.levels, self.ws.data_ptr(), self.ws.numel(), 1 if clear else 0,
                                           err_flag.data_ptr(), s), "sparse_chain_sites")

    def run_rulebooks(self, indices0, n0_dev_ptr, n0_cap, hash0, job_lo, job_hi, stream=None):
        import ctypes
        from ._lib import RulebookJob
        s = _stream() if stream is None else stream
        if self.nbr and self.nbr[0] is None:
            self.bind_tables(n0_cap)
        n = int(job_hi) - int(job_lo)
        if n <= 0:
            return
        sub = (RulebookJob * n).from_address(ctypes.addressof(self.jobs) + int(job_lo) * ctypes.sizeof(RulebookJob))
        check(lib.sessd_sparse_chain_rulebooks(indices0.data_ptr(), n0_dev_ptr, int(n0_cap), hash0.keys.data_ptr(),
                                               hash0.vals.data_ptr(), hash0.capacity, hash0._dims_t.data_ptr(), self.batch,
                                               len(self.levels), self.levels, self.ws.data_ptr(), n, sub, s), "sparse_chain_rulebooks")


def _t3(v):
    return [int(v)] * 3 if isinstance(v, int) else [int(x) for x in v]


_REPACK = [None]


class RepackRegistry:
    def __init__(self):
        self.objects = {}
        self.jobs = {"dense": [], "sparse": []}
        self._table = {"dense": None, "sparse": None}
        self.versions = {}
        self.gen = -1
        self._creating = 0
        self.refreshes = 0

    def recording(self):
        return self._creating > 0

    def note(self, kind, job):
        self.jobs[kind].append(job)
        self._table[kind] = None

    def cached(self, key, weight, factory):
        self.ensure_fresh(weight)
        obj = self.objects.get(key)
        if obj is None:
            self._creating += 1
            try:
                obj = factory()
            finally:
                self._creating -= 1
            self.objects[key] = obj
            self.versions[id(weight)] = [weight, weight._version]
            if isinstance(obj, PackedConv):
                obj._registry = self
                for la in obj.launches:
                    if isinstance(la, _Launch):
                        la["_registry"] = self
        return obj

    def create(self, factory):
        self._creating += 1
        try:
            return factory()
        finally:
            self._creating -= 1

    def ensure_fresh(self, weight=None):
        seen = self.versions.get(id(weight)) if weight is not None else None
        if self.gen == _PARAM_GENERATION[0] and (seen is None or seen[1] == weight._version):
            return
        self.refresh()

    def prepare(self):
        for kind in ("sparse", "dense"):
            if self.jobs[kind] and self._table[kind] is None:
                self._table[kind] = _repack_table(kind, self.jobs[kind])

    def refresh(self):
        for kind in ("sparse", "dense"):
            jobs = self.jobs[kind]
            if not jobs:
                continue
            if self._table[kind] is None:
                if torch.cuda.is_current_stream_capturing():
                    raise RuntimeError("RepackRegistry: a packing was recorded that no eager iteration has run yet; run one warm-up "
                                       "iteration (or registry.prepare()) before capturing")
                self._table[kind] = _repack_table(kind, jobs)
            table, n, blocks = self._table[kind]
            fn = lib.sessd_sparse_pack_batch if kind == "sparse" else lib.sessd_dense_pack_batch
            with torch.cuda.device(table.device):
                check(fn(table.data_ptr(), n, blocks, _stream()), "%s_pack_batch" % kind)
        self.gen = _PARAM_GENERATION[0]
        for rec in self.versions.values():
            rec[1] = rec[0]._version
        self.refreshes += 1


def _repack_table(kind, jobs):
    import ctypes
    i32, vp, i64 = ctypes.c_int32, ctypes.c_void_p, ctypes.c_longlong
    if kind == "dense":
        class Job(ctypes.Structure):
            _fields_ = [("w", vp), ("out", vp), ("so", i64), ("sc", i64), ("tap_off", i32 * 16), ("cout", i32), ("cin", i32),
                        ("ntaps", i32), ("kind", i32), ("flip", i32), ("layout", i32), ("block_start", i32), ("pad_", i32)]
    else:
        class Job(ctypes.Structure):
            _fields_ = [("w", vp), ("out", vp), ("kv", i32), ("cin", i32), ("cout", i32), ("adjoint", i32), ("reverse_k", i32),
                        ("block_start", i32)]
    arr = (Job * len(jobs))()
    start = 0
    for a, j in zip(arr, jobs):
        a.w, a.out, a.block_start = j["w"].data_ptr(), j["out"].data_ptr(), start
        if kind == "dense":
            a.so, a.sc, a.cout, a.cin, a.kind, a.flip, a.layout = j["so"], j["sc"], j["cout"], j["cin"], j["kind"], j["flip"], j["layout"]
            a.ntaps = len(j["taps"])
            for t, off in enumerate(j["taps"]):
                a.tap_off[t] = int(off)
            cp = (j["cout"] + 31) // 32 * 32
            if j["kind"] == 0:
                total = (j["cin"] // 2) * len(j["taps"]) * 2 * cp
            else:
                cpad = cp if j["layout"] == 0 else ((j["cout"] + 127) // 128 * 128 if j["layout"] == 1 else (j["cout"] + 63) // 64 * 64)
                total = cpad * j["cin"]
        else:
            a.kv, a.cin, a.cout, a.adjoint, a.reverse_k = j["kv"], j["cin"], j["cout"], j["adjoint"], j["reverse_k"]
            total = j["kv"] * j["cin"] * j["cout"]
        start += (total + 255) // 256
    dev = jobs[0]["out"].device
    table = torch.frombuffer(bytearray(bytes(arr)), dtype=torch.uint8).to(dev)
    return table, len(jobs), start


class batched_repack:

    def __init__(self, registry):
        self.registry = registry

    def __enter__(self):
        self.prev = _REPACK[0]
        _REPACK[0] = self.registry
        return self.registry

    def __exit__(self, *exc):
        _REPACK[0] = self.prev
        return False


def _repack_note(group, **job):
    reg = _REPACK[0]
    if reg is not None and reg.recording():
        reg.note(group, job)


def _registry_for(weight):
    reg = _REPACK[0]
    return reg if reg is not None and isinstance(weight, torch.nn.Parameter) and weight.is_cuda else None


def packed_sparse_weight(weight, mode="fwd"):
    make = {"fwd": lambda: sparse_pack_weight(weight), "adj": lambda: sparse_pack_weight_adjoint(weight, False),
            "adj_rev": lambda: sparse_pack_weight_adjoint(weight, True)}[mode]
    reg = _registry_for(weight)
    if reg is None:
        return make()
    return reg.cached(("sparse", weight.data_ptr(), tuple(weight.shape), mode), weight, make)


def packed_conv2d(weight, stride=1, adjoint=False, transposed=False):
    make = (lambda: pack_deconv2d_s2(weight)) if transposed else (lambda: pack_conv2d(weight, stride, adjoint=adjoint))
    reg = _registry_for(weight)
    if reg is None:
        return make()
    return reg.cached(("dense", weight.data_ptr(), tuple(weight.shape), int(stride), bool(adjoint), bool(transposed)), weight, make)


def sparse_pack_weight(weight):
    w = weight.detach().to(torch.float32).contiguous()
    if not w.is_cuda:
        raise ValueError("weight must be on the HIP device")
    cin, cout = w.shape[-2], w.shape[-1]
    kv = w.numel() // (cin * cout)
    out = torch.empty_like(w).view(-1)
    check(lib.sessd_sparse_pack_weight(w.data_ptr(), kv, cin, cout, out.data_ptr(), _stream()), "sparse_pack_weight")
    _repack_note("sparse", w=w, out=out, kv=kv, cin=cin, cout=cout, adjoint=0, reverse_k=0)
    return out


def sparse_pack_weight_adjoint(weight, reverse_offsets):
    w = weight.detach().to(torch.float32).contiguous()
    cin, cout = w.shape[-2], w.shape[-1]
    kv = w.numel() // (cin * cout)
    out = torch.empty_like(w).view(-1)
    check(lib.sessd_sparse_pack_weight_adjoint(w.data_ptr(), kv, cin, cout, 1 if reverse_offsets else 0, out.data_ptr(), _stream()),
          "sparse_pack_weight_adjoint")
    _repack_note("sparse", w=w, out=out, kv=kv, cin=cin, cout=cout, adjoint=1, reverse_k=1 if reverse_offsets else 0)
    return out


def sparse_conv(in_feat, nbr, tile_mask, n_out_dev, packed_weight, cin, cout, scale=None, shift=None, relu=True,
                out=None, dense_out=None, out_indices=None, dense_dims=None, cout_split=0, depth=0, offset_split=0, share_w=0, perm=None, tiles_per_wave=1):
    _req(in_feat, torch.float32, "in_feat")
    kv, cap = nbr.shape
    dd = None
    if dense_out is None:
        if out is None:
            out = torch.empty((cap, cout), dtype=torch.float32, device=in_feat.device)
    else:
        dd = _i3(dense_dims)
    check(lib.sessd_sparse_conv_sorted(in_feat.data_ptr(), cin, nbr.data_ptr(), tile_mask.data_ptr(), kv, n_out_dev.data_ptr(),
                                       cap, packed_weight.data_ptr(), _p(scale), _p(shift), 1 if relu else 0, _p(out), cout,
                                       _p(out_indices), _p(dense_out), 0 if dd is None else dd.data_ptr(),
                                       int(cout_split) + 256 * int(depth) + 65536 * int(bool(offset_split)) + 131072 * int(bool(share_w))
                                       + ({1: 0, 2: 1, 4: 2}[int(tiles_per_wave)] << 20), _p(perm), _stream()),
          "sparse_conv")
    return out if dense_out is None else dense_out


def sparse_renumber_sites(indices, n_dev, feat, site_hash, batch):
    _req(indices, torch.int32, "indices")
    _req(feat, torch.float32, "feat")
    cap, ch = indices.shape[0], feat.shape[1]
    out_idx, out_feat = torch.empty_like(indices), torch.empty_like(feat)
    ws = workspace(lib.sessd_sparse_renumber_workspace_bytes(int(batch), site_hash._dims_t.data_ptr()), indices.device, "renumber")
    check(lib.sessd_sparse_renumber_sites(indices.data_ptr(), n_dev.data_ptr(), cap, int(batch), site_hash._dims_t.data_ptr(),
                                          feat.data_ptr(), ch, site_hash.keys.data_ptr(), site_hash.vals.data_ptr(),
                                          site_hash.capacity, out_idx.data_ptr(), out_feat.data_ptr(), ws.data_ptr(), ws.numel(),
                                          _stream()), "sparse_renumber_sites")
    return out_idx, out_feat


class BnReluTrainFunction(torch.autograd.Function):

    @staticmethod
    def forward(ctx, x, n_dev, gamma, beta, running_mean, running_var, eps, momentum, relu):
        x = x.float().contiguous()
        _req(x, torch.float32, "x")
        cap, C = x.shape
        dev = x.device
        y = torch.empty_like(x)
        mean, invstd = torch.empty(C, device=dev), torch.empty(C, device=dev)
        ws = zeroed_workspace(lib.sessd_bn_relu_train_workspace_bytes(C), dev, "bn")
        g, b = gamma.detach().float().contiguous(), beta.detach().float().contiguous()
        check(lib.sessd_bn_relu_train_fwd(x.data_ptr(), n_dev.data_ptr(), cap, C, g.data_ptr(), b.data_ptr(), float(eps),
                                          float(momentum), 1 if relu else 0, _p(running_mean), _p(running_var), y.data_ptr(),
                                          mean.data_ptr(), invstd.data_ptr(), ws.data_ptr(), ws.numel(), _stream()), "bn_relu_train_fwd")
        ctx.save_for_backward(x, y, g, mean, invstd, n_dev)
        ctx.relu = bool(relu)
        return y

    @staticmethod
    def backward(ctx, dy):
        x, y, g, mean, invstd, n_dev = ctx.saved_tensors
        dy = dy.float().contiguous()
        cap, C = x.shape
        dx = torch.empty_like(x)
        dg, db = torch.empty(C, device=x.device), torch.empty(C, device=x.device)
        ws = zeroed_workspace(lib.sessd_bn_relu_train_workspace_bytes(C), x.device, "bn")
        check(lib.sessd_bn_relu_train_bwd(dy.data_ptr(), x.data_ptr(), y.data_ptr(), n_dev.data_ptr(), cap, C, g.data_ptr(),
                                          mean.data_ptr(), invstd.data_ptr(), 1 if ctx.relu else 0, dx.data_ptr(), dg.data_ptr(),
                                          db.data_ptr(), ws.data_ptr(), ws.numel(), _stream()), "bn_relu_train_bwd")
        return dx, None, dg, db, None, None, None, None, None


_NBT_DEFER = [False]
_NBT_PENDING = []


class deferred_batch_counts:

    def __enter__(self):
        self.prev = _NBT_DEFER[0]
        _NBT_DEFER[0] = True
        return self

    def __exit__(self, *exc):
# ... 221 lines not shown
    mask = torch.zeros((P, words), dtype=torch.int32, device=points.device)
    check(lib.sessd_points_in_bodies(points.data_ptr(), P, points.shape[1], planes.data_ptr(), M, F, mask.data_ptr(), _stream()),
          "points_in_bodies")
    bit = torch.arange(M, device=points.device)
    return ((mask[:, bit // 32] >> (bit % 32)) & 1).bool()


def box3d_overlap_eval(boxes, qboxes, criterion=-1, z_axis=1, z_center=1.0):
    _req(boxes, torch.float64, "boxes")
    _req(qboxes, torch.float64, "qboxes")
    out = torch.empty((boxes.shape[0], qboxes.shape[0]), dtype=torch.float64, device=boxes.device)
    check(lib.sessd_box3d_overlap_eval(boxes.data_ptr(), boxes.shape[0], qboxes.data_ptr(), qboxes.shape[0], int(criterion),
                                       int(z_axis), float(z_center), out.data_ptr(), _stream()), "box3d_overlap_eval")
    return out


class KittiStatistics:

    def __init__(self, overlaps, gt_datas, dt_datas, ign_gts, ign_dets, dontcares, device):
        import numpy as np
        F = len(overlaps)
        self.F, self.dev = F, device
        n_gt = np.array([g.shape[0] for g in gt_datas], np.int64)
        n_dt = np.array([d.shape[0] for d in dt_datas], np.int64)
        n_dc = np.array([c.shape[0] for c in dontcares], np.int64)
        off = lambda n: np.concatenate([[0], np.cumsum(n)]).astype(np.int32)
        self.gt_off_h, self.dt_off_h = off(n_gt), off(n_dt)
        ov_sizes = n_gt * n_dt
        ov_off = np.concatenate([[0], np.cumsum(ov_sizes)[:-1]]).astype(np.int64) if F else np.zeros((0,), np.int64)
        flat = np.concatenate([np.ascontiguousarray(o, np.float64).reshape(-1) for o in overlaps]) if F else np.zeros((0,), np.float64)
        cat = lambda lst, w, dt: (np.concatenate(lst, 0) if len(lst) and sum(x.shape[0] for x in lst) else np.zeros((0, w), dt)).astype(dt)
        t = lambda a: torch.from_numpy(np.ascontiguousarray(a)).to(device)
        self.ov, self.ov_off = t(flat if flat.size else np.zeros((1,), np.float64)), t(ov_off if F else np.zeros((1,), np.int64))
        self.gt_off, self.dt_off, self.dc_off = t(self.gt_off_h), t(self.dt_off_h), t(off(n_dc))
        pad = lambda a, w, dt: a if a.shape[0] else np.zeros((1, w), dt)
        self.gt = t(pad(cat(gt_datas, 5, np.float64), 5, np.float64))
        self.dt = t(pad(cat(dt_datas, 6, np.float64), 6, np.float64))
        self.dc = t(pad(cat(dontcares, 4, np.float64), 4, np.float64))
        ig = np.concatenate(ign_gts).astype(np.int32) if F else np.zeros((0,), np.int32)
        idt = np.concatenate(ign_dets).astype(np.int32) if F else np.zeros((0,), np.int32)
        self.ig, self.idt = t(ig if ig.size else np.zeros((1,), np.int32)), t(idt if idt.size else np.zeros((1,), np.int32))
        self.n_gt_total = int(n_gt.sum())
        self.err = torch.zeros((1,), dtype=torch.int32, device=device)

    def _run(self, metric, min_overlap, thresholds, compute_fp, compute_aos, tp_scores, stats):
        check(lib.sessd_kitti_statistics(self.ov.data_ptr(), self.ov_off.data_ptr(), self.gt_off.data_ptr(), self.dt_off.data_ptr(),
                                         self.dc_off.data_ptr(), self.gt.data_ptr(), self.dt.data_ptr(), self.ig.data_ptr(),
                                         self.idt.data_ptr(), self.dc.data_ptr(), self.F, int(metric), float(min_overlap),
                                         _p(thresholds), 0 if thresholds is None else int(thresholds.shape[0]),
                                         1 if compute_fp else 0, 1 if compute_aos else 0, _p(tp_scores), _p(stats),
                                         self.err.data_ptr(), _stream()), "kitti_statistics")

    def precision_table(self, metric, min_overlap, num_valid_gt, compute_aos=False, num_pts=41):
        import numpy as np
        tp_scores = torch.empty((max(self.n_gt_total, 1),), dtype=torch.float64, device=self.dev)
        self._run(metric, min_overlap, None, False, False, tp_scores, None)
        sc = tp_scores[:self.n_gt_total]
        sc = sc[~torch.isnan(sc)]
        if sc.numel() == 0 or num_valid_gt <= 0:
            return np.zeros((0,)), np.zeros((0, 4))
        sc, _ = torch.sort(sc, descending=True)
        thr = torch.zeros((num_pts,), dtype=torch.float64, device=self.dev)
        n_thr = torch.zeros((1,), dtype=torch.int32, device=self.dev)
        check(lib.sessd_kitti_thresholds(sc.data_ptr(), int(sc.numel()), int(num_valid_gt), int(num_pts), thr.data_ptr(),
                                         n_thr.data_ptr(), _stream()), "kitti_thresholds")
        n = int(n_thr.item())
        thr = thr[:n].contiguous()
        stats = torch.empty((self.F, n, 4), dtype=torch.float64, device=self.dev)
        self._run(metric, min_overlap, thr, True, compute_aos, None, stats)
        pr = torch.empty((n, 4), dtype=torch.float64, device=self.dev)
        check(lib.sessd_kitti_reduce(stats.data_ptr(), self.F, n, pr.data_ptr(), _stream()), "kitti_reduce")
        if int(self.err.item()):
            raise SessdError("a frame has more than 256 detections: not supported by the device evaluation")
        return thr.cpu().numpy(), pr.cpu().numpy()


def points_rigid_moves_(points, planes, centers, loc, rot, valid):
    import numpy as np
    _req(points, torch.float32, "points")
    _req(planes, torch.float32, "planes")
    M = planes.shape[0]
    dev = points.device
    rot = np.asarray(rot, np.float64)
    sc = np.stack([np.sin(rot), np.cos(rot)], 1).astype(np.float32)
    t = lambda a, dt: torch.from_numpy(np.ascontiguousarray(np.asarray(a).astype(dt))).to(dev)
    c, l, r, v = t(centers, np.float64), t(loc, np.float64), t(sc, np.float32), t(np.asarray(valid).astype(np.uint8), np.uint8)
    check(lib.sessd_points_rigid_moves(points.data_ptr(), points.shape[0], points.shape[1], planes.data_ptr(), c.data_ptr(),
                                       l.data_ptr(), r.data_ptr(), v.data_ptr(), M, _stream()), "points_rigid_moves")
    return points


def points_global_transform_(points, flip, angle, scale, raw_copy=None):
    import numpy as np
    _req(points, torch.float32, "points")
    if raw_copy is not None:
        _req(raw_copy, torch.float32, "raw_copy")
    check(lib.sessd_points_global_transform(points.data_ptr(), points.shape[0], points.shape[1], 1 if flip else 0,
                                            float(np.float32(np.sin(angle))), float(np.float32(np.cos(angle))),
                                            float(np.float32(scale)), _p(raw_copy), _stream()), "points_global_transform")
    return points


def farthest_point_sample(points, k):
    _req(points, torch.float32, "points")
    n = points.shape[0]
    out = torch.empty((k,), dtype=torch.int32, device=points.device)
    check(lib.sessd_farthest_point_sample(points.data_ptr(), n, points.shape[1], int(k), out.data_ptr(), _stream()), "farthest_point_sample")
    return out.long()


def points_compact(points, keep, out=None):
    _req(points, torch.float32, "points")
    k = keep.to(torch.uint8).contiguous()
    P, C = points.shape
    if out is None:
        out = torch.empty((max(P, 1), C), dtype=torch.float32, device=points.device)
    n_out = torch.zeros((1,), dtype=torch.int32, device=points.device)
    ws = workspace(lib.sessd_points_compact_workspace_bytes(P), points.device, "compact")
    check(lib.sessd_points_compact(points.data_ptr(), k.data_ptr(), P, C, out.data_ptr(), out.shape[0], n_out.data_ptr(),
                                   ws.data_ptr(), ws.numel(), _stream()), "points_compact")
    return out, n_out


def sparse_rulebook_transpose(nbr, n_out_dev, n_in_cap):
    kv, cap = nbr.shape
    nbr_t = torch.empty((kv, n_in_cap), dtype=torch.int32, device=nbr.device)
    tm_t = torch.empty(((n_in_cap + 15) // 16,), dtype=torch.int32, device=nbr.device)
    check(lib.sessd_sparse_rulebook_transpose(nbr.data_ptr(), kv, n_out_dev.data_ptr(), cap, n_in_cap, nbr_t.data_ptr(),
                                              tm_t.data_ptr(), _stream()), "sparse_rulebook_transpose")
    return nbr_t, tm_t


def sparse_conv_wgrad(in_feat, grad_out, nbr, tile_mask, n_out_dev, cin, cout):
    _req(in_feat, torch.float32, "in_feat")
    _req(grad_out, torch.float32, "grad_out")
    kv, cap = nbr.shape
    if grad_out.shape[0] < cap or grad_out.shape[1] != cout or in_feat.shape[1] != cin:
        raise ValueError("grad_out must be (n_out_cap, cout) and in_feat (n_in, cin)")
    gw = torch.empty((kv, cin, cout), dtype=torch.float32, device=in_feat.device)
    ws = torch.empty(int(lib.sessd_sparse_conv_wgrad_workspace_bytes(kv, cin, cout)), dtype=torch.uint8, device=in_feat.device)
    check(lib.sessd_sparse_conv_wgrad(in_feat.data_ptr(), cin, grad_out.data_ptr(), cout, nbr.data_ptr(), tile_mask.data_ptr(),
                                      kv, n_out_dev.data_ptr(), cap, gw.data_ptr(), ws.data_ptr(), ws.numel(), _stream()),
          "sparse_conv_wgrad")
    return gw


class PackedConv:

    def __init__(self, launches, cin, cout, kind, stride):
        self.launches = launches
        self.cin, self.cout, self.kind, self.stride = cin, cout, kind, stride
        self._w3 = None
        self._upk = None
        self._upk_sk = [None, None, None]
        self._sk = None
        self._registry = None

    @property
    def upk(self):
        if self._upk is None and self._w3 is not None and self.cin % 8 == 0:
            make = lambda: pack_winograd(self._w3[0], adjoint=self._w3[1])
            self._upk = self._registry.create(make) if self._registry is not None else make()
        return self._upk

    def upk_sk(self, shape):
        if self._upk_sk[shape] is None and self._w3 is not None and self.cin % (16, 8, 16)[shape] == 0:
            make = lambda: pack_winograd_sk(self._w3[0], shape, adjoint=self._w3[1])
            self._upk_sk[shape] = self._registry.create(make) if self._registry is not None else make()
        return self._upk_sk[shape]


    def sk_args(self):
        if self._sk is None:
            import ctypes
            n = len(self.launches)
            if self.cin % 16 or n > 4 or any("view" not in la or la["ntaps"] > 9 for la in self.launches):
                return None
            ncg = (self.cout + 127) // 128
            wpk, dy, dx = [], (ctypes.c_int * (9 * n))(), (ctypes.c_int * (9 * n))()
            for c, la in enumerate(self.launches):
                w, so, sc, taps = la["view"]
                nt = len(taps)
                out = torch.empty((ncg, self.cin // 16, nt, 2048), dtype=torch.float32, device=w.device)
                check(lib.sessd_conv2d_sk_pack(w.data_ptr(), int(so), int(sc), (ctypes.c_int * nt)(*[int(t) for t in taps]), nt,
                                               self.cout, self.cin, out.data_ptr(), _stream()), "conv2d_sk_pack")
                wpk.append(out)
                for t in range(nt):
                    dy[9 * c + t], dx[9 * c + t] = int(la["dy"][t]), int(la["dx"][t])
            self._sk = dict(wpk=wpk, wptr=(ctypes.c_void_p * n)(*[t.data_ptr() for t in wpk]),
                            ntaps=(ctypes.c_int * n)(*[la["ntaps"] for la in self.launches]), dy=dy, dx=dx,
                            py=(ctypes.c_int * n)(*[la["py"] for la in self.launches]),
                            px=(ctypes.c_int * n)(*[la["px"] for la in self.launches]), n=n)
        return self._sk


def _pack_taps_view(w, out_stride, in_stride, tap_offsets, cout, cin):
    import ctypes
    _req(w, torch.float32, "weight")
    nt = len(tap_offsets)
    cp = (cout + 31) // 32 * 32
    out = torch.empty((cin // 2, nt, 2, cp), dtype=torch.float32, device=w.device)
    check(lib.sessd_conv2d_pack_taps(w.data_ptr(), int(out_stride), int(in_stride), (ctypes.c_int * nt)(*[int(t) for t in tap_offsets]),
                                     nt, cout, cin, out.data_ptr(), _stream()), "conv2d_pack_taps")
    _repack_note("dense", w=w, out=out, so=int(out_stride), sc=int(in_stride), taps=[int(t) for t in tap_offsets], cout=int(cout),
                 cin=int(cin), kind=0, flip=0, layout=0)
    return out


class _Launch(dict):

    def __missing__(self, key):
        if key != "wpk":
            raise KeyError(key)
        w, so, sc, taps = self["view"]
        make = lambda: _pack_taps_view(w, so, sc, taps, self["_co"], self["_ci"])
        reg = dict.get(self, "_registry")
        self["wpk"] = reg.create(make) if reg is not None else make()
        return self["wpk"]


def _conv_view(w, adjoint):
    co, ci, kh, kw = w.shape
    kk = kh * kw
    return (ci, co, kk, ci * kk, True) if adjoint else (co, ci, ci * kk, kk, False)


def pack_conv2d(weight, stride=1, padding=None, adjoint=False):
    w = weight.detach().to(torch.float32).contiguous()
    kh, kw = w.shape[2], w.shape[3]
    assert kh == kw and kh in (1, 3) and not (adjoint and stride != 1)
    co, ci, so, sc, flip = _conv_view(w, adjoint)
    assert ci % 2 == 0
    pad = kh // 2 if padding is None else padding
    assert pad == kh // 2
    kk = kh * kw
    dy = [ky - pad for ky in range(kh) for kx in range(kw)]
    dx = [kx - pad for ky in range(kh) for kx in range(kw)]
    taps = [(kk - 1 - t) if flip else t for t in range(kk)]
    la = _Launch(dy=torch.tensor(dy, dtype=torch.int32), dx=torch.tensor(dx, dtype=torch.int32), in_mul=stride,
                 out_mul=1, py=0, px=0, ntaps=kh * kw, view=(w, so, sc, taps), _co=co, _ci=ci)
    pc = PackedConv([la], ci, co, "conv", stride)
    if kh == 3 and stride == 1:
        pc._w3 = (w, bool(adjoint))
    return pc


def _winograd_pack(weight, layout, adjoint):
    w = weight.detach().to(torch.float32).contiguous()
    _req(w, torch.float32, "weight")
    assert w.shape[2] == 3 and w.shape[3] == 3
    co, ci, so, sc, flip = _conv_view(w, adjoint)
    if layout == 0:
        out = torch.empty((ci // 2, 4, 2, (co + 31) // 32 * 32, 4), dtype=torch.float32, device=w.device)
    elif layout == 3:
        out = torch.empty(((co + 127) // 128, ci // 2, 4, 2, 32, 16), dtype=torch.float32, device=w.device)
    else:
        nw, c = ((8, 128), (4, 64))[layout - 1]
        out = torch.empty(((co + c - 1) // c, ci // 2, nw, 2, 32, c // 32, 16 // nw), dtype=torch.float32, device=w.device)
    check(lib.sessd_conv3x3_winograd_pack(w.data_ptr(), so, sc, 1 if flip else 0, co, ci, layout, out.data_ptr(), _stream()),
          "conv3x3_winograd_pack")
    _repack_note("dense", w=w, out=out, so=int(so), sc=int(sc), taps=[], cout=int(co), cin=int(ci), kind=1, flip=1 if flip else 0,
                 layout=int(layout))
    return out


def winograd_u(weight):
    w = weight.detach().to(torch.float64)
    co, ci, kh, kw = w.shape
    assert kh == 3 and kw == 3
    G = torch.tensor([[1, 0, 0], [0.5, 0.5, 0.5], [0.5, -0.5, 0.5], [0, 0, 1]], dtype=torch.float64, device=w.device)
    return torch.einsum("ia,ocab,jb->ocij", G, w, G).to(torch.float32).reshape(co, ci, 16)


def pack_winograd_sk(weight, shape=0, adjoint=False):
    return _winograd_pack(weight, 1 + shape, adjoint)


_SK_WS = {}
_SK_WS_RETIRED = []


def winograd_sk_workspace(batch, h, w, cout, device, workgroups=0, shape=0):
    with torch.cuda.device(device):
        n = int(lib.sessd_conv3x3_winograd_sk_workspace_bytes(batch, h, w, cout, shape, workgroups))
    if n == 0:
        raise ValueError("winograd_sk_workspace: bad arguments")
    return torch.zeros(n, dtype=torch.uint8, device=device)


def conv2d_sk_workspace(batch, tile_h, tile_w, cout, nclass, device, workgroups=0):
    with torch.cuda.device(device):
        n = int(lib.sessd_conv2d_sk_workspace_bytes(batch, tile_h, tile_w, cout, nclass, workgroups))
    if n == 0:
        raise ValueError("conv2d_sk_workspace: bad arguments")
    return torch.zeros(n, dtype=torch.uint8, device=device)


def conv2d_winograd_sk_sets(x, upk_sets, nsets, cout, scale, shift, relu, out, shape, workspace, workgroups=0, residual=None):
    _req(x, torch.float32, "x")
    NB, ci, H, W = x.shape
    check(lib.sessd_conv3x3_winograd_sk_sets(x.data_ptr(), NB, int(nsets), ci, H, W, upk_sets.data_ptr(), out.data_ptr(), int(cout),
                                             _p(scale), _p(shift), 1 if relu else 0, _p(residual), workspace.data_ptr(),
                                             workspace.numel(), int(shape), int(workgroups), _stream()), "conv3x3_winograd_sk_sets")
    return out


def conv2d_winograd_sk_active(x, upk, cout, scale, shift, relu, out, shape, workspace, tile_list, n_list, workgroups=0, residual=None,
                              min_rounds=2):
    _req(x, torch.float32, "x"); _req(tile_list, torch.int32, "tile_list"); _req(n_list, torch.int32, "n_list")
    B, ci, H, W = x.shape
    check(lib.sessd_conv3x3_winograd_sk_active(x.data_ptr(), B, ci, H, W, upk.data_ptr(), out.data_ptr(), int(cout), _p(scale), _p(shift),
                                               1 if relu else 0, _p(residual), tile_list.data_ptr(), n_list.data_ptr(),
                                               tile_list.numel(), int(min_rounds), workspace.data_ptr(), workspace.numel(), int(shape),
                                               int(workgroups), _stream()), "conv3x3_winograd_sk_active")
    return out


def conv2d_sk_active(x, pc, scale, shift, relu, out, workspace, tile_list, n_list, workgroups=0, residual=None, min_rounds=4):
    import ctypes
    _req(x, torch.float32, "x"); _req(tile_list, torch.int32, "tile_list"); _req(n_list, torch.int32, "n_list")
    B, ci, H, W = x.shape
    sk = pc.sk_args()
    if sk is None:
        raise ValueError("conv2d_sk_active needs cin % 16 == 0")
    if pc.kind == "conv":
        Ho, Wo = (H + pc.stride - 1) // pc.stride, (W + pc.stride - 1) // pc.stride
        th, tw = Ho, Wo
    else:
        Ho, Wo, th, tw = 2 * H, 2 * W, H, W
    la = pc.launches[0]
    check(lib.sessd_conv2d_sk_active(x.data_ptr(), B, ci, H, W, sk["n"], ctypes.cast(sk["wptr"], ctypes.c_void_p).value,
                                     ctypes.cast(sk["ntaps"], ctypes.c_void_p).value, ctypes.cast(sk["dy"], ctypes.c_void_p).value,
                                     ctypes.cast(sk["dx"], ctypes.c_void_p).value, la["in_mul"], th, tw, out.data_ptr(), pc.cout,
                                     Ho, Wo, la["out_mul"], ctypes.cast(sk["py"], ctypes.c_void_p).value,
                                     ctypes.cast(sk["px"], ctypes.c_void_p).value, _p(scale), _p(shift), 1 if relu else 0,
                                     _p(residual), tile_list.data_ptr(), n_list.data_ptr(), tile_list.numel(), int(min_rounds),
                                     workspace.data_ptr(), workspace.numel(), int(workgroups), _stream()), "conv2d_sk_active")
    return out


def conv2d_mfma_active(x, pc, scale, shift, relu, out, tile_list, n_list, tile_cfg=11, residual=None):
    _req(x, torch.float32, "x"); _req(tile_list, torch.int32, "tile_list"); _req(n_list, torch.int32, "n_list")
    B, ci, H, W = x.shape
    assert pc.kind == "conv" and pc.stride == 1 and len(pc.launches) == 1 and pc.launches[0]["ntaps"] == 1 and ci % 8 == 0
    la = pc.launches[0]
    check(lib.sessd_conv2d_mfma_active(x.data_ptr(), B, ci, H, W, la["wpk"].data_ptr(), 1, la["dy"].data_ptr(), la["dx"].data_ptr(), 1, H, W,
                                       out.data_ptr(), pc.cout, H, W, 1, 0, 0, _p(scale), _p(shift), 1 if relu else 0, _p(residual),
                                       tile_list.data_ptr(), n_list.data_ptr(), tile_list.numel(), int(tile_cfg), _stream()),
          "conv2d_mfma_active")
    return out


def deconv2d_s2_pair_active(x, pc_a, pc_b, scale_a, shift_a, scale_b, shift_b, relu, out_a, out_b, tile_list, n_list, residual_a=None,
                            residual_b=None, tile_cfg=11):
    import ctypes
    _req(x, torch.float32, "x"); _req(tile_list, torch.int32, "tile_list"); _req(n_list, torch.int32, "n_list")
    B, ci, H, W = x.shape
    assert pc_a.kind == pc_b.kind == "deconv" and pc_a.cin == pc_b.cin == ci and pc_a.cout == pc_b.cout
    check(lib.sessd_deconv2d_s2_mfma_pair_active(x.data_ptr(), B, ci, H, W, ctypes.cast(pc_a.wpk4, ctypes.c_void_p).value,
                                                 ctypes.cast(pc_b.wpk4, ctypes.c_void_p).value, pc_a.ntaps4.data_ptr(),
                                                 pc_a.dy4.data_ptr(), pc_a.dx4.data_ptr(), out_a.data_ptr(), out_b.data_ptr(), pc_a.cout,
                                                 _p(scale_a), _p(shift_a), _p(scale_b), _p(shift_b), 1 if relu else 0, _p(residual_a),
                                                 _p(residual_b), tile_list.data_ptr(), n_list.data_ptr(), tile_list.numel(),
                                                 int(tile_cfg), _stream()), "deconv2d_s2_mfma_pair_active")
    return out_a, out_b


class TileActivity:

    def __init__(self, batch, H, W, steps, device):
        import ctypes
        steps = [0] * steps if isinstance(steps, int) else [int(v) for v in steps]
        self.batch, self.H, self.W, self.steps = int(batch), int(H), int(W), steps
        self.dims, h, w = [], H, W
        for k in steps:
            if k in (0, 3):
                self.dims.append((h, w))
            elif k == 4:
                h, w = 2 * h, 2 * w
            else:
                h, w = h // 2, w // 2
                if k == 2:
                    self.dims.append((h, w))
        self.n_slots = self.n_layers = len(self.dims)
        self._steps = (ctypes.c_int32 * len(steps))(*steps)
        tiles = (H // 2) * (W // 2)
        self.tile_mask = torch.zeros((self.n_slots, batch, H // 2, 2), dtype=torch.int64, device=device)
        self.tile_list = torch.zeros((self.n_slots, batch * tiles), dtype=torch.int32, device=device)
        self.n_list = torch.zeros(self.n_slots, dtype=torch.int32, device=device)
        self.ws = torch.zeros(max(256, int(lib.sessd_bev_tile_activity_workspace_bytes(batch, self.n_slots))), dtype=torch.uint8, device=device)
        self._jobs = None

    def run(self, indices, n_dev, n_cap):
        _req(indices, torch.int32, "indices"); _req(n_dev, torch.int32, "n_dev")
        check(lib.sessd_bev_tile_activity(indices.data_ptr(), n_dev.data_ptr(), int(n_cap), self.batch, self.H, self.W, self._steps,
                                          len(self.steps), self.tile_mask.data_ptr(), self.tile_list.data_ptr(), self.n_list.data_ptr(),
                                          self.tile_list.shape[1], self.ws.data_ptr(), self.ws.numel(), _stream()), "bev_tile_activity")

    def mask_bool(self, slot):
        import numpy as np
        h, w = self.dims[slot]
        m = self.tile_mask[slot].cpu().numpy().view("uint64")[:, :h // 2]
        tx = np.arange(w // 2)
        return torch.from_numpy(((m[:, :, tx >> 6] >> (tx & 63).astype("uint64")) & np.uint64(1)).astype(bool))

    def fill(self, outs, values, layers=None, tiles=None, near=None, near_kind=None):
        from ._lib import FillTilesJob
        layers = list(range(len(outs))) if layers is None else list(layers)
        tiles = [2] * len(outs) if tiles is None else list(tiles)
        near = [None] * len(outs) if near is None else list(near)
        near_kind = [0] * len(outs) if near_kind is None else list(near_kind)
        key = tuple((o.data_ptr(), v.data_ptr(), l, t, n, k) for o, v, l, t, n, k in zip(outs, values, layers, tiles, near, near_kind))
        if self._jobs is None or self._jobs[0] != key:
            arr = (FillTilesJob * len(outs))()
            for i, (o, v, l, t) in enumerate(zip(outs, values, layers, tiles)):
                _req(o, torch.float32, "out"); _req(v, torch.float32, "value")
                up = 2 if t == 4 else 1
                assert tuple(o.shape[2:]) == (up * self.dims[l][0], up * self.dims[l][1]) and o.shape[0] == self.batch
                assert v.numel() == (4 if t in (4, 6) else 1) * o.shape[1]
                arr[i].out, arr[i].value, arr[i].tile_mask, arr[i].cout = o.data_ptr(), v.data_ptr(), self.tile_mask[l].data_ptr(), o.shape[1]
                arr[i].h, arr[i].w, arr[i].mask_th, arr[i].tile = o.shape[2], o.shape[3], self.H // 2, t
                if near[i] is not None:
                    k = int(near_kind[i])
                    dn, dl = self.dims[near[i]], self.dims[l]
                    assert t in (2, 6) and k in (0, 1, 2) and (dn == dl if k == 0 else (2 * dn[0], 2 * dn[1]) == tuple(dl))
                    arr[i].near_mask, arr[i].near_kind = self.tile_mask[near[i]].data_ptr(), k
            self._jobs = (key, arr)
        arr = self._jobs[1]
        check(lib.sessd_fill_inactive_tiles(arr, len(outs), self.batch, _stream()), "fill_inactive_tiles")


def pack_winograd(weight, adjoint=False):
    return _winograd_pack(weight, 0, adjoint)


def pack_deconv2d_s2(weight):
    w = weight.detach().to(torch.float32)
    ci, co, kh, kw = w.shape
    assert kh == 3 and kw == 3 and ci % 2 == 0
    sel = {0: [(1, 0)], 1: [(0, 1), (2, 0)]}
    launches = []
    w = w.contiguous()
    for py in (0, 1):
        for px in (0, 1):
            taps = [(ky, ey, kx, ex) for (ky, ey) in sel[py] for (kx, ex) in sel[px]]
            offs = [3 * ky + kx for (ky, ey, kx, ex) in taps]
            wpk = _pack_taps_view(w, 9, co * 9, offs, co, ci)
            launches.append(dict(wpk=wpk, dy=torch.tensor([t[1] for t in taps], dtype=torch.int32),
                                 dx=torch.tensor([t[3] for t in taps], dtype=torch.int32), in_mul=1, out_mul=2, py=py,
                                 px=px, ntaps=len(taps), view=(w, 9, co * 9, offs)))
    pc = PackedConv(launches, ci, co, "deconv", 2)
    import ctypes
    pc.wpk4 = (ctypes.c_void_p * 4)(*[la["wpk"].data_ptr() for la in launches])
    pc.ntaps4 = torch.tensor([la["ntaps"] for la in launches], dtype=torch.int32)
    pc.dy4 = torch.zeros((4, 4), dtype=torch.int32)
    pc.dx4 = torch.zeros((4, 4), dtype=torch.int32)
    for c, la in enumerate(launches):
        pc.dy4[c, :la["ntaps"]] = la["dy"]
        pc.dx4[c, :la["ntaps"]] = la["dx"]
    return pc


def deconv2d_s2_pair(x, pc_a, pc_b, scale_a, shift_a, scale_b, shift_b, relu, out_a, out_b, residual_a=None, residual_b=None, tile_cfg=4):
    import ctypes
    _req(x, torch.float32, "x")
    B, ci, H, W = x.shape
    assert pc_a.kind == pc_b.kind == "deconv" and pc_a.cin == pc_b.cin == ci and pc_a.cout == pc_b.cout
    check(lib.sessd_deconv2d_s2_mfma_pair(x.data_ptr(), B, ci, H, W, ctypes.cast(pc_a.wpk4, ctypes.c_void_p).value,
                                          ctypes.cast(pc_b.wpk4, ctypes.c_void_p).value, pc_a.ntaps4.data_ptr(), pc_a.dy4.data_ptr(),
                                          pc_a.dx4.data_ptr(), out_a.data_ptr(), out_b.data_ptr(), pc_a.cout, _p(scale_a), _p(shift_a),
                                          _p(scale_b), _p(shift_b), 1 if relu else 0, _p(residual_a), _p(residual_b), int(tile_cfg),
                                          _stream()), "deconv2d_s2_mfma_pair")
    return out_a, out_b


def conv2d(x, pc, scale=None, shift=None, relu=True, residual=None, out=None, tile_cfg=None, workspace=None, workgroups=0):
    _req(x, torch.float32, "x")
    B, ci, H, W = x.shape
    assert ci == pc.cin
    if pc.kind == "conv":
        Ho, Wo = (H + pc.stride - 1) // pc.stride, (W + pc.stride - 1) // pc.stride
        th, tw = Ho, Wo
    else:
        Ho, Wo = 2 * H, 2 * W
        th, tw = H, W
    if out is None:
        out = torch.empty((B, pc.cout, Ho, Wo), dtype=torch.float32, device=x.device)
    if tile_cfg in (22, 23, 24):
        shape = tile_cfg - 22
        upk = pc.upk_sk(shape) if pc.kind == "conv" else None
        if upk is None or (H & 1) or (W & 1):
            raise ValueError("tile_cfg 22/23/24 (stream-K Winograd) needs a 3x3 stride-1 conv with cin % 16 (22, 24) / 8 (23) == 0 and even H, W")
        if workspace is None:
            key = (x.device.index, _cache_scope(), shape, workgroups)
            need = int(lib.sessd_conv3x3_winograd_sk_workspace_bytes(B, H, W, pc.cout, shape, workgroups))
            workspace = _SK_WS.get(key)
            if workspace is None or workspace.numel() < need:
                if workspace is not None:
                    _SK_WS_RETIRED.append(workspace)
                workspace = _SK_WS[key] = torch.zeros(need, dtype=torch.uint8, device=x.device)
        check(lib.sessd_conv3x3_winograd_sk(x.data_ptr(), B, ci, H, W, upk.data_ptr(), out.data_ptr(), pc.cout, _p(scale),
                                            _p(shift), 1 if relu else 0, _p(residual), workspace.data_ptr(), workspace.numel(),
                                            shape, workgroups, _stream()), "conv3x3_winograd_sk")
        return out
    if tile_cfg == 30:
        sk = pc.sk_args()
        if sk is None:
            raise ValueError("tile_cfg 30 (LDS-tiled stream-K) needs cin % 16 == 0")
        la = pc.launches[0]
        need = int(lib.sessd_conv2d_sk_workspace_bytes(B, th, tw, pc.cout, sk["n"], workgroups))
        if workspace is None:
            key = (x.device.index, _cache_scope(), "csk", workgroups)
            workspace = _SK_WS.get(key)
            if workspace is None or workspace.numel() < need:
                if workspace is not None:
                    _SK_WS_RETIRED.append(workspace)
                workspace = _SK_WS[key] = torch.zeros(need, dtype=torch.uint8, device=x.device)
        elif workspace.numel() < need:
            raise ValueError("conv2d: stream-K workspace too small (%d < %d bytes)" % (workspace.numel(), need))
        import ctypes
        check(lib.sessd_conv2d_sk(x.data_ptr(), B, ci, H, W, sk["n"], ctypes.cast(sk["wptr"], ctypes.c_void_p).value,
                                  ctypes.cast(sk["ntaps"], ctypes.c_void_p).value, ctypes.cast(sk["dy"], ctypes.c_void_p).value,
                                  ctypes.cast(sk["dx"], ctypes.c_void_p).value, la["in_mul"], th, tw, out.data_ptr(), pc.cout,
                                  Ho, Wo, la["out_mul"], ctypes.cast(sk["py"], ctypes.c_void_p).value,
                                  ctypes.cast(sk["px"], ctypes.c_void_p).value, _p(scale), _p(shift), 1 if relu else 0,
                                  _p(residual), workspace.data_ptr(), workspace.numel(), workgroups, _stream()), "conv2d_sk")
        return out
    if tile_cfg in (20, 21):
        if getattr(pc, "upk", None) is None or (H & 1) or (W & 1):
            raise ValueError("tile_cfg 20/21 (Winograd) needs a 3x3 stride-1 conv with cin % 8 == 0 and even H, W")
        check(lib.sessd_conv3x3_winograd(x.data_ptr(), B, ci, H, W, pc.upk.data_ptr(), out.data_ptr(), pc.cout, _p(scale),
                                         _p(shift), 1 if relu else 0, _p(residual), tile_cfg - 20, _stream()),
              "conv3x3_winograd")
        return out
    if pc.kind == "deconv" and ci % 8 == 0:
        import ctypes
        cfg = tile_cfg if tile_cfg is not None else default_tile_cfg(pc.cout, th * tw, 4)
        check(lib.sessd_deconv2d_s2_mfma(x.data_ptr(), B, ci, H, W, ctypes.cast(pc.wpk4, ctypes.c_void_p).value,
                                         pc.ntaps4.data_ptr(), pc.dy4.data_ptr(), pc.dx4.data_ptr(), out.data_ptr(),
                                         pc.cout, _p(scale), _p(shift), 1 if relu else 0, _p(residual), cfg, _stream()),
              "deconv2d_s2_mfma")
        return out
    if tile_cfg is None and USE_WINOGRAD and pc.kind == "conv" and pc._w3 is not None and not (H & 1) and not (W & 1) \
            and H * W >= 4096 and ci % 8 == 0:
        return conv2d(x, pc, scale, shift, relu, residual, out, 20)
    for la in pc.launches:
        cfg = tile_cfg
        if cfg is None:
            cfg = default_tile_cfg(pc.cout, th * tw, la["ntaps"])
        check(lib.sessd_conv2d_mfma(x.data_ptr(), B, ci, H, W, la["wpk"].data_ptr(), la["ntaps"], la["dy"].data_ptr(),
                                    la["dx"].data_ptr(), la["in_mul"], th, tw, out.data_ptr(), pc.cout, Ho, Wo,
                                    la["out_mul"], la["py"], la["px"], _p(scale), _p(shift), 1 if relu else 0,
                                    _p(residual), cfg, _stream()), "conv2d_mfma")
    return out


_TILE_CFG_OVERRIDE = {}
WINOGRAD_CFGS = (20, 21, 22, 23, 24)
WINOGRAD_SK_CFGS = (22, 23, 24)


def winograd_mult_ratio(tile_cfg):
    return 16.0 / 36.0 if tile_cfg in WINOGRAD_CFGS else 1.0


USE_WINOGRAD = True


def assign_targets(anchors, gt_boxes, gt_classes=None, matched_threshold=0.6, unmatched_threshold=0.45):
    _req(anchors, torch.float32, "anchors")
    n, m = anchors.shape[0], gt_boxes.shape[0]
    dev = anchors.device
    g = gt_boxes.to(device=dev, dtype=torch.float32).contiguous() if m else torch.zeros((1, 7), dtype=torch.float32, device=dev)
    c = None if gt_classes is None or m == 0 else gt_classes.to(device=dev, dtype=torch.int32).contiguous()
    out = dict(labels=torch.empty((n,), dtype=torch.int32, device=dev), bbox_targets=torch.empty((n, 7), dtype=torch.float32, device=dev),
               bbox_outside_weights=torch.empty((n,), dtype=torch.float32, device=dev), gt_id=torch.empty((n,), dtype=torch.int32, device=dev))
    ws = workspace(lib.sessd_assign_targets_workspace_bytes(n), dev, "assign")
    check(lib.sessd_assign_targets(anchors.data_ptr(), n, g.data_ptr(), _p(c), m, float(matched_threshold), float(unmatched_threshold),
                                   out["labels"].data_ptr(), out["bbox_targets"].data_ptr(), out["bbox_outside_weights"].data_ptr(),
                                   out["gt_id"].data_ptr(), ws.data_ptr(), ws.numel(), _stream()), "assign_targets")
    return out


class OdiouFunction(torch.autograd.Function):

    @staticmethod
    def forward(ctx, gboxes, qboxes, weights, batch_size):
        g = gboxes.detach().float().contiguous()
        q = qboxes.detach().float().contiguous()
        _req(g, torch.float32, "gboxes")
        n = q.shape[0]
        term = torch.empty((n,), dtype=torch.float32, device=q.device)
        grad = torch.empty((n, 7), dtype=torch.float32, device=q.device)
        check(lib.sessd_odiou3d(g.data_ptr(), q.data_ptr(), n, term.data_ptr(), grad.data_ptr(), _stream()), "odiou3d")
        w = weights.detach().float()
        ctx.save_for_backward(grad, w)
        ctx.scale = 2.0 / float(batch_size)
        ctx.terms = term
        return (term * w).sum() * ctx.scale

    @staticmethod
    def backward(ctx, gl):
        grad, w = ctx.saved_tensors
        return None, grad * (w * (ctx.scale * gl)).unsqueeze(1), None, None


def odiou_3d_loss(gboxes, qboxes, weights, batch_size):
    return OdiouFunction.apply(gboxes, qboxes, weights, batch_size)


HEAD_LOSS_RECORD = {
    "total": 0, "loss": 1, "cls_loss_reduced": 2, "loc_loss_reduced": 3, "dir_loss_reduced": 4, "iou_pred_loss": 5, "ious_loss": 6,
    "consistency_loss": 7, "cls_pos_loss": 8, "cls_neg_loss": 9, "loc_loss_elem": slice(10, 17), "num_pos": 17, "num_neg": 18,
    "consistency_box": 19, "consistency_score": 20, "consistency_iou": 21, "matched_boxes": 22,
    "loss_ema": 24, "cls_loss_reduced_ema": 26, "loc_loss_reduced_ema": 27, "dir_loss_reduced_ema": 28, "iou_pred_loss_ema": 29,
    "cls_pos_loss_ema": 32, "cls_neg_loss_ema": 33, "loc_loss_elem_ema": slice(34, 41), "num_pos_ema": 41, "num_neg_ema": 42,
    "overflow": 48, "positives": 49, "positives_ema": 50, "candidates": 51, "candidates_ema": 52}


class HeadLoss:

    def __init__(self, batch, num_anchors, device, labels_i64, cfg, pos_capacity=None, cons_capacity=2048):
        from ._lib import HeadLossCfg
        self.B, self.A, self.dev = int(batch), int(num_anchors), device
        c = HeadLossCfg()
        c.batch, c.num_anchors, c.labels_i64 = self.B, self.A, 1 if labels_i64 else 0
        c.pos_capacity = int(pos_capacity or 1024 * self.B)
        c.cons_capacity = int(cons_capacity)
        for k in ("pos_cls_weight", "neg_cls_weight", "focal_alpha", "focal_gamma", "smooth_l1_sigma", "cls_loss_weight",
                  "loc_loss_weight", "dir_loss_weight", "direction_offset", "score_thresh", "match_iou_thresh"):
            setattr(c, k, float(cfg[k]))
        for i, v in enumerate(cfg["center_range"]):
            c.center_range[i] = float(v)
        self.cfg = c
        import ctypes as C
        self._cfg_p = C.addressof(c)
        need = int(lib.sessd_head_loss_workspace_bytes(self._cfg_p))
        if need == 0:
            raise ValueError("sessd_head_loss does not cover this configuration")
        f = lambda *sh: torch.zeros(sh, dtype=torch.float32, device=device)
        self.ws = torch.zeros(need, dtype=torch.uint8, device=device)
        self.g_box, self.g_cls, self.g_dir, self.g_iou = f(self.B, self.A, 7), f(self.B, self.A), f(self.B, self.A, 2), f(self.B, self.A)
        self.record = f(64)

    def run(self, stu, tea, anchors0, transformation, cons_weight):
# ... 359 lines not shown
```

Measured before the change: 1994.

## Add bf16x3 split-precision MFMA path to stream-K Winograd conv

Adds a new stream-K Winograd variant (shape 3) that splits both the transformed weights and the transformed input tiles into three bf16 terms and accumulates six bf16 MFMA products. This emulates fp32 accuracy on the bf16 matrix units, which offer higher throughput than the fp32 MFMA path it replaces. A new weight pack layout stores the three bf16 pieces, and the engine makes this variant the default for active-tile layers that used shape 0, controlled by an environment flag. It trades extra MFMAs, split work and register pressure for faster matrix instructions, and accuracy is slightly below true fp32.

```diff
diff --git a/se-ssd_amd/csrc/dense_conv.hip b/se-ssd_amd/csrc/dense_conv.hip
--- a/se-ssd_amd/csrc/dense_conv.hip
+++ b/se-ssd_amd/csrc/dense_conv.hip
@@ -786,8 +786,12 @@
   const int kp = (int)(r / A.nt);
   out[idx] = o < A.co ? A.w[(long long)o * A.so + (long long)(2 * kp + h) * A.sc + A.tap_off[t]] : 0.f;
 }
+__device__ __forceinline__ unsigned short bf16_rne_bits(float x) {
+  const unsigned u = __builtin_bit_cast(unsigned, x);
+  return (unsigned short)((u + 0x7FFFu + ((u >> 16) & 1u)) >> 16);
+}
 __device__ __forceinline__ void winograd_pack_body(const PackArgs& A, int flip, int layout, float* __restrict__ out, size_t idx) {
-  const int cpad = layout == 0 ? A.cp : ((layout == 1 || layout == 3) ? (A.co + 127) / 128 * 128 : (A.co + 63) / 64 * 64);
+  const int cpad = layout == 0 ? A.cp : ((layout == 1 || layout == 3 || layout == 4) ? (A.co + 127) / 128 * 128 : (A.co + 63) / 64 * 64);
   if (idx >= (size_t)cpad * A.ci) return;
   const int o = (int)(idx % cpad), c = (int)(idx / cpad);
   double g[3][3];
@@ -815,6 +819,20 @@
     for (int b = 0; b < 4; ++b) {
       const int xi = a * 4 + b;
       size_t dst;
+      if (layout == 4) {
+        const int grp = o >> 7, cb = (o >> 5) & 3, i = o & 31, wave = xi >> 1, xl = xi & 1;
+        const size_t step = (size_t)(c >> 4) * 8 + xl * 4 + cb;
+        dst = ((((size_t)grp * 8 + wave) * (size_t)(A.ci >> 1) + step) * 3) * 512 + (size_t)(((c >> 3) & 1) * 32 + i) * 8 + (c & 7);
+        unsigned short* o16 = reinterpret_cast<unsigned short*>(out);
+        const float f = (float)u[b];
+        const unsigned short t0 = bf16_rne_bits(f);
+        const float r = f - __builtin_bit_cast(float, (unsigned)t0 << 16);
+        const unsigned short t1 = bf16_rne_bits(r);
+        o16[dst] = t0;
+        o16[dst + 512] = t1;
+        o16[dst + 1024] = bf16_rne_bits(r - __builtin_bit_cast(float, (unsigned)t1 << 16));
+        continue;
+      }
       if (layout == 0) {
         dst = ((((size_t)kp * 4 + (xi >> 2)) * 2 + h) * cpad + o) * 4 + (xi & 3);
       } else if (layout == 1) {
@@ -886,11 +904,11 @@
 
 int sessd_conv3x3_winograd_pack(const float* w, long long out_stride, long long in_stride, int flip, int cout, int cin, int layout,
                                 float* out, hipStream_t stream) {
-  if (cout < 1 || cin < 2 || (cin & 1) || layout < 0 || layout > 3) return SESSD_EINVAL;
+  if (cout < 1 || cin < 2 || (cin & 1) || layout < 0 || layout > 4 || (layout == 4 && cin % 16)) return SESSD_EINVAL;
   PackArgs A;
   A.w = w; A.so = out_stride; A.sc = in_stride; A.co = cout; A.ci = cin; A.nt = 9; A.cp = sessd_divup(cout, 32) * 32;
   for (int t = 0; t < 16; ++t) A.tap_off[t] = 0;
-  const int cpad = layout == 0 ? A.cp : ((layout == 1 || layout == 3) ? sessd_divup(cout, 128) * 128 : sessd_divup(cout, 64) * 64);
+  const int cpad = layout == 0 ? A.cp : ((layout == 1 || layout == 3 || layout == 4) ? sessd_divup(cout, 128) * 128 : sessd_divup(cout, 64) * 64);
   const size_t total = (size_t)cpad * cin;
   SESSD_LAUNCH(winograd_pack_kernel, dim3((unsigned)((total + 255) / 256)), dim3(256), 0, stream, A, flip, layout, out);
   SESSD_CHECK_LAUNCH();
diff --git a/se-ssd_amd/csrc/dense_wino_sk.hip b/se-ssd_amd/csrc/dense_wino_sk.hip
--- a/se-ssd_amd/csrc/dense_wino_sk.hip
+++ b/se-ssd_amd/csrc/dense_wino_sk.hip
@@ -7,6 +7,8 @@
 using f32x4v = __attribute__((ext_vector_type(4))) float;
 using f32x2v = __attribute__((ext_vector_type(2))) float;
 typedef unsigned int u32x4g __attribute__((__vector_size__(16)));
+typedef __bf16 bf16x8 __attribute__((ext_vector_type(8)));
+typedef __bf16 bf16x2 __attribute__((ext_vector_type(2)));
 
 typedef __amdgpu_buffer_rsrc_t rsrc_t;
 __device__ __forceinline__ rsrc_t make_rsrc(const void* base, unsigned bytes) {
@@ -20,6 +22,17 @@
   float r;
   asm volatile("v_add_f32 %0, %1, %2" : "=v"(r) : "v"(a), "v"(b));
   return r;
+}
+
+__device__ __forceinline__ unsigned pk_bf16(float x0, float x1) {
+  return __builtin_bit_cast(unsigned, __builtin_convertvector((f32x2v){x0, x1}, bf16x2));
+}
+__device__ __forceinline__ void split3_pk(float x0, float x1, unsigned& t0, unsigned& t1, unsigned& t2) {
+  t0 = pk_bf16(x0, x1);
+  x0 -= __builtin_bit_cast(float, t0 << 16); x1 -= __builtin_bit_cast(float, t0 & 0xFFFF0000u);
+  t1 = pk_bf16(x0, x1);
+  x0 -= __builtin_bit_cast(float, t1 << 16); x1 -= __builtin_bit_cast(float, t1 & 0xFFFF0000u);
+  t2 = pk_bf16(x0, x1);
 }
 
 struct WinoArgs {
@@ -41,17 +54,19 @@
   int list_cap, min_rounds, batch;
 };
 
-template <int NW, int CBN, int VAR = 0, bool LIST = false>
+template <int NW, int CBN, int VAR = 0, bool LIST = false, bool SPLIT = false>
 __global__ __launch_bounds__(NW * 64, 8 / NW) void conv3x3s1_winograd_sk_kernel(WinoArgs A) {
   constexpr int XW = 16 / NW;
   static_assert(XW * CBN == 8, "8 accumulators per wave");
+  static_assert(!SPLIT || (NW == 8 && VAR == 0), "the split main loop is written for 8 waves (a round = one K = 16 MFMA)");
+  constexpr int VBUF_S = 3 * 16 * 64 * 4;
   constexpr int NT = NW * 64;
   constexpr unsigned WSTEP = NW * 2u * 32u * 32u;
   constexpr int VBUF = NW * 1024;
   constexpr int SLOT = CBN * 32 * 32 * 4;
   constexpr int NPT = 1024 / NT;
   constexpr int RING = NW;
-  __shared__ __attribute__((aligned(16))) float lds[16384];
+  __shared__ __attribute__((aligned(16))) float lds[SPLIT ? 2 * VBUF_S : 16384];
   __shared__ int s_last, s_pend;
   const int tid = threadIdx.x, lane = tid & 63;
   const int wave = __builtin_amdgcn_readfirstlane(tid >> 6);
@@ -201,6 +216,18 @@
     f32x4v pr[4];
     f32x4v ua[RING][2];
     float bv[2][XW];
+    f32x4v ps[2][3];
+    bf16x8 us[4][3], bs[3];
+    unsigned rs[3] = {SESSD_OOB, SESSD_OOB, SESSD_OOB};
+    if constexpr (SPLIT) {
+#pragma unroll
+      for (int q = 0; q < 3; ++q) {
+        const int y = y0 + (q == 0 ? 2 * h : (q == 1 ? 2 - h : 1 + 2 * h));
+        rs[q] = (tlive && y >= 0 && y < A.hin) ? img_off + (unsigned)((y * A.win + max(x0, 0)) * 4) : SESSD_OOB;
+      }
+    }
+    const rsrc_t wrs = SPLIT ? make_rsrc(A.upk + (size_t)wset * A.upk_stride + (size_t)cg * A.cin * 3072, (unsigned)A.cin * 12288u) : wr;
+    const unsigned wso = SPLIT ? (unsigned)(wave * A.cin * 1536 + lane * 16) : 0u;
 
 #define SESSD_SK_LOADP(ROUND)                                                                      \
   {                                                                                                \
@@ -286,15 +313,108 @@
     voff ^= VBUF;                                                                                  \
     ++rr;                                                                                          \
   }
-
-    SESSD_SK_LOADP(r0)
-    __builtin_amdgcn_sched_barrier(0);
-#pragma unroll
-    for (int s = 0; s < RING - 1; ++s) {
-      SESSD_SK_LOADU(s, r0 * NW + s)
+#define SESSD_SS_LOADP(ROUND)                                                                      \
+  {                                                                                                \
+    const unsigned xs = (unsigned)(min((ROUND), r1 - 1) * NW + wave) * xstep;                      \
+    _Pragma("unroll") for (int c = 0; c < 2; ++c)                                                  \
+      _Pragma("unroll") for (int q = 0; q < 3; ++q)                                                \
+        ps[c][q] = __builtin_bit_cast(f32x4v, __builtin_amdgcn_raw_buffer_load_b128(xr, (int)rs[q], (int)(xs + c * (xstep >> 1)), 0)); \
+  }
+#define SESSD_SS_LOADU(SET, KG)                                                                    \
+  {                                                                                                \
+    const unsigned ws = (unsigned)min((KG), klast) * 3072u;                                        \
+    _Pragma("unroll") for (int p = 0; p < 3; ++p)                                                  \
+      us[SET][p] = __builtin_bit_cast(bf16x8, __builtin_amdgcn_raw_buffer_load_b128(wrs, (int)(wso + 1024u * p), (int)ws, 0)); \
+  }
+#define SESSD_SS_TRANSFORM(VOFF)                                                                   \
+  {                                                                                                \
+    if (edge) {                                                                                    \
+      _Pragma("unroll") for (int c = 0; c < 2; ++c)                                                \
+        _Pragma("unroll") for (int q = 0; q < 3; ++q) {                                            \
+          const f32x4v p = ps[c][q];                                                               \
+          ps[c][q].x = mask_l ? 0.f : p.x; ps[c][q].y = mask_l ? p.x : p.y;                        \
+          ps[c][q].z = mask_l ? p.y : p.z; ps[c][q].w = mask_l ? p.z : (mask_r ? 0.f : p.w);       \
+        }                                                                                          \
+    }                                                                                              \
+    float vt[2][8];                                                                                \
+    _Pragma("unroll") for (int c = 0; c < 2; ++c) {                                                \
+      const f32x4v ra = ps[c][0] - ps[c][1];                                                       \
+      const f32x4v rb = ps[c][1] + (h ? -ps[c][2] : ps[c][2]);                                     \
+      vt[c][0] = ra.x - ra.z; vt[c][1] = ra.y + ra.z; vt[c][2] = ra.z - ra.y; vt[c][3] = ra.y - ra.w; \
+      vt[c][4] = rb.x - rb.z; vt[c][5] = rb.y + rb.z; vt[c][6] = rb.z - rb.y; vt[c][7] = rb.y - rb.w; \
+    }                                                                                              \
+    unsigned* dst = reinterpret_cast<unsigned*>(&lds[(VOFF) + ((8 * h) * 64 + (wave >> 2) * 32 + j) * 4 + (wave & 3)]); \
+    _Pragma("unroll") for (int e = 0; e < 8; ++e) {                                                \
+      unsigned t0, t1, t2;                                                                         \
+      split3_pk(vt[0][e], vt[1][e], t0, t1, t2);                                                   \
+      dst[e * 256] = t0; dst[(16 + e) * 256] = t1; dst[(32 + e) * 256] = t2;                       \
+    }                                                                                              \
+  }
+#define SESSD_SS_READV(VOFF, X)                                                                    \
+  {                                                                                                \
+    _Pragma("unroll") for (int p = 0; p < 3; ++p)                                                  \
+      bs[p] = __builtin_bit_cast(bf16x8, *static_cast<const u32x4g*>(__builtin_assume_aligned(                    \
+          &lds[(VOFF) + ((p * 16 + wave * XW + (X)) * 64 + lane) * 4], 16)));                     \
+  }
+#define SESSD_SS_MMA(SET, S)                                                                       \
+  {                                                                                                \
+    f32x16 a_ = acc[(S) >> 2][(S) & 3];                                                            \
+    a_ = __builtin_amdgcn_mfma_f32_32x32x16_bf16(us[SET][2], bs[0], a_, 0, 0, 0);                  \
+    a_ = __builtin_amdgcn_mfma_f32_32x32x16_bf16(us[SET][1], bs[1], a_, 0, 0, 0);                  \
+    a_ = __builtin_amdgcn_mfma_f32_32x32x16_bf16(us[SET][0], bs[2], a_, 0, 0, 0);                  \
+    a_ = __builtin_amdgcn_mfma_f32_32x32x16_bf16(us[SET][1], bs[0], a_, 0, 0, 0);                  \
+    a_ = __builtin_amdgcn_mfma_f32_32x32x16_bf16(us[SET][0], bs[1], a_, 0, 0, 0);                  \
+    a_ = __builtin_amdgcn_mfma_f32_32x32x16_bf16(us[SET][0], bs[0], a_, 0, 0, 0);                  \
+    acc[(S) >> 2][(S) & 3] = a_;                                                                   \
+  }
+#define SESSD_SS_STEP(KS)                                                                          \
+  {                                                                                                \
+    SESSD_SS_LOADU(((KS) + 3) & 3, kg0 + (KS) + 3)                                                 \
+    __builtin_amdgcn_sched_barrier(0);                                                             \
+    SESSD_SS_MMA((KS) & 3, KS)                                                                     \
+    __builtin_amdgcn_sched_barrier(0);                                                             \
+  }
+#define SESSD_SS_ROUND()                                                                           \
+  {                                                                                                \
+    const int kg0 = rr * 8;                                                                        \
+    SESSD_SS_READV(voff, 0)                                                                        \
+    __builtin_amdgcn_sched_barrier(0);                                                             \
+    SESSD_SS_STEP(0)                                                                               \
+    SESSD_SS_STEP(1)                                                                               \
+    SESSD_SS_STEP(2)                                                                               \
+    SESSD_SS_STEP(3)                                                                               \
+    SESSD_SS_LOADP(rr + 1)                                                                         \
+    SESSD_SS_READV(voff, 1)                                                                        \
+    __builtin_amdgcn_sched_barrier(0);                                                             \
+    SESSD_SS_STEP(4)                                                                               \
+    SESSD_SS_STEP(5)                                                                               \
+    SESSD_SS_STEP(6)                                                                               \
+    SESSD_SS_STEP(7)                                                                               \
+    SESSD_SS_TRANSFORM(voff ^ VBUF_S)                                                              \
+    __syncthreads();                                                                               \
+    voff ^= VBUF_S;                                                                                \
+    ++rr;                                                                                          \
+  }
+
+    if constexpr (SPLIT) {
+      SESSD_SS_LOADP(r0)
       __builtin_amdgcn_sched_barrier(0);
-    }
-    SESSD_SK_TRANSFORM(0)
+#pragma unroll
+      for (int s = 0; s < 3; ++s) {
+        SESSD_SS_LOADU(s, r0 * 8 + s)
+        __builtin_amdgcn_sched_barrier(0);
+      }
+      SESSD_SS_TRANSFORM(0)
+    } else {
+      SESSD_SK_LOADP(r0)
+      __builtin_amdgcn_sched_barrier(0);
+#pragma unroll
+      for (int s = 0; s < RING - 1; ++s) {
+        SESSD_SK_LOADU(s, r0 * NW + s)
+        __builtin_amdgcn_sched_barrier(0);
+      }
+      SESSD_SK_TRANSFORM(0)
+    }
     __syncthreads();
     if (pend_state == 1) {
       if (tid == 0) {
@@ -305,7 +425,11 @@
     }
     int voff = 0;
     int rr = r0;
-    while (rr < r1) SESSD_SK_ROUND()
+    if constexpr (SPLIT) {
+      while (rr < r1) SESSD_SS_ROUND()
+    } else {
+      while (rr < r1) SESSD_SK_ROUND()
+    }
 #undef SESSD_SK_LOADP
 #undef SESSD_SK_LOADU
 #undef SESSD_SK_TRANSFORM
@@ -313,6 +437,13 @@
 #undef SESSD_SK_MMA
 #undef SESSD_SK_STEP
 #undef SESSD_SK_ROUND
+#undef SESSD_SS_LOADP
+#undef SESSD_SS_LOADU
+#undef SESSD_SS_TRANSFORM
+#undef SESSD_SS_READV
+#undef SESSD_SS_MMA
+#undef SESSD_SS_STEP
+#undef SESSD_SS_ROUND
 
     if (pend_state == 3) {
       SESSD_LDS_BARRIER();
@@ -787,7 +918,7 @@
   return SESSD_OK;
 }
 
-template <int NW, int CBN>
+template <int NW, int CBN, bool SPLIT = false>
 int launch_sk(const float* in, int batch, int nsets, int cin, int h, int w, const float* upk, float* out, int cout, const float* scale,
               const float* shift, int relu, const float* residual, void* workspace, size_t workspace_bytes, int workgroups,
               hipStream_t stream, const int* tile_list = nullptr, const int* n_list = nullptr, int list_cap = 0, int min_rounds = 1) {
@@ -801,6 +932,7 @@
   A.rpu = cin / (2 * NW);
   A.bper = batch / nsets; A.ss_stride = nsets > 1 ? cout : 0;
   A.upk_stride = nsets > 1 ? (long long)sessd_divup(cout, CBN * 32) * (cin >> 1) * (NW * 2 * 32 * 32 / 4) : 0;
+  if (SPLIT && nsets > 1) A.upk_stride = (long long)sessd_divup(cout, CBN * 32) * cin * 3072;
   A.tile_list = tile_list; A.n_list = n_list; A.list_cap = list_cap; A.min_rounds = (min_rounds < 0 && tile_list) ? min_rounds : (min_rounds < 1 ? 1 : min_rounds); A.batch = batch;
   const long long units = (long long)batch * A.tblocks * A.ngroups;
   if (units * A.rpu > 0x7fffffffLL) return SESSD_EINVAL;
@@ -811,7 +943,12 @@
   A.counters = (unsigned*)workspace;
   A.scratch = (float*)((char*)workspace + sessd_align((size_t)units * 4, 256));
   if (tile_list) {
-    SESSD_LAUNCH((conv3x3s1_winograd_sk_kernel<NW, CBN, 0, true>), dim3(workgroups), dim3(NW * 64), 0, stream, A);
+    SESSD_LAUNCH((conv3x3s1_winograd_sk_kernel<NW, CBN, 0, true, SPLIT>), dim3(workgroups), dim3(NW * 64), 0, stream, A);
+    SESSD_CHECK_LAUNCH();
+    return SESSD_OK;
+  }
+  if constexpr (SPLIT) {
+    SESSD_LAUNCH((conv3x3s1_winograd_sk_kernel<NW, CBN, 0, false, true>), dim3(workgroups), dim3(NW * 64), 0, stream, A);
     SESSD_CHECK_LAUNCH();
     return SESSD_OK;
   }
@@ -839,7 +976,7 @@
 extern "C" {
 
 size_t sessd_conv3x3_winograd_sk_workspace_bytes(int batch, int h, int w, int cout, int shape, int workgroups) {
-  if (batch < 1 || h < 2 || w < 2 || cout < 1 || workgroups < 0 || shape < 0 || shape > 2) return 0;
+  if (batch < 1 || h < 2 || w < 2 || cout < 1 || workgroups < 0 || shape < 0 || shape > 3) return 0;
   if (workgroups == 0 && default_workgroups(shape, &workgroups) != SESSD_OK) return 0;
   const int cpu = shape == 1 ? 64 : 128;
   const size_t units = (size_t)batch * sessd_divup((h / 2) * (w / 2), 32) * sessd_divup(cout, cpu);
@@ -850,7 +987,7 @@
                                    int cout, const float* scale, const float* shift, int relu, const float* residual,
                                    void* workspace, size_t workspace_bytes, int shape, int workgroups, hipStream_t stream) {
   if ((h & 1) || (w & 1) || batch < 1 || nsets < 1 || batch % nsets || cout < 1 || workgroups < 0 || (workgroups & 7) || shape < 0 ||
-      shape > 2)
+      shape > 3)
     return SESSD_EINVAL;
   if (workgroups == 0) {
     const int rc = default_workgroups(shape, &workgroups);
@@ -860,6 +997,8 @@
     return launch_rk(in, batch, nsets, cin, h, w, upk, out, cout, scale, shift, relu, residual, workspace, workspace_bytes, workgroups, stream);
   if (shape == 1)
     return launch_sk<4, 2>(in, batch, nsets, cin, h, w, upk, out, cout, scale, shift, relu, residual, workspace, workspace_bytes, workgroups, stream);
+  if (shape == 3)
+    return launch_sk<8, 4, true>(in, batch, nsets, cin, h, w, upk, out, cout, scale, shift, relu, residual, workspace, workspace_bytes, workgroups, stream);
   return launch_sk<8, 4>(in, batch, nsets, cin, h, w, upk, out, cout, scale, shift, relu, residual, workspace, workspace_bytes, workgroups, stream);
 }
 
@@ -867,8 +1006,8 @@
                                      const float* scale, const float* shift, int relu, const float* residual,
                                      const int32_t* tile_list, const int32_t* n_list, int list_cap, int min_rounds, void* workspace,
                                      size_t workspace_bytes, int shape, int workgroups, hipStream_t stream) {
-  if ((h & 1) || (w & 1) || batch < 1 || cout < 1 || workgroups < 0 || (workgroups & 7) || shape < 0 || shape > 1 || !tile_list ||
-      !n_list || list_cap < 1)
+  if ((h & 1) || (w & 1) || batch < 1 || cout < 1 || workgroups < 0 || (workgroups & 7) || shape < 0 || shape > 3 || shape == 2 ||
+      !tile_list || !n_list || list_cap < 1)
     return SESSD_EINVAL;
   if (workgroups == 0) {
     const int rc = default_workgroups(shape, &workgroups);
@@ -877,6 +1016,9 @@
   if (shape == 1)
     return launch_sk<4, 2>(in, batch, 1, cin, h, w, upk, out, cout, scale, shift, relu, residual, workspace, workspace_bytes, workgroups,
                            stream, tile_list, n_list, list_cap, min_rounds);
+  if (shape == 3)
+    return launch_sk<8, 4, true>(in, batch, 1, cin, h, w, upk, out, cout, scale, shift, relu, residual, workspace, workspace_bytes,
+                                 workgroups, stream, tile_list, n_list, list_cap, min_rounds);
   return launch_sk<8, 4>(in, batch, 1, cin, h, w, upk, out, cout, scale, shift, relu, residual, workspace, workspace_bytes, workgroups,
                          stream, tile_list, n_list, list_cap, min_rounds);
 }
diff --git a/se-ssd_amd/sessd_hip/engine.py b/se-ssd_amd/sessd_hip/engine.py
--- a/se-ssd_amd/sessd_hip/engine.py
+++ b/se-ssd_amd/sessd_hip/engine.py
@@ -1,4 +1,5 @@
 import math
+import os
 
 import numpy as np
 import torch
@@ -18,6 +19,9 @@
     shift = b - bn.running_mean.detach().float() * scale
     return scale.contiguous(), shift.contiguous()
 
+
+WINO_SPLIT = os.environ.get("SESSD_WINO_SPLIT", "1") != "0"
+WINO_LIST_SHAPES = (0, 1, 3) if WINO_SPLIT else (0, 1)
 
 SPMIDDLE_LAYERS = [
     ("subm", 4, 16, 3, 1, 0, "subm0"), ("subm", 16, 16, 3, 1, 0, "subm0"),
@@ -435,6 +439,8 @@
         self.sk_ws = torch.zeros_like(other.sk_ws) if other.sk_ws is not None else None
 
     DEFAULT_ACTIVE_CFG = {0: (1, 4), 1: (0, 1), 2: (1, 2), 3: (30, 4), 4: (1, 2), 5: (0, 1), 6: (11, 0), 7: (30, 8), 8: (4, 0), 9: (0, 8)}
+    if WINO_SPLIT:
+        DEFAULT_ACTIVE_CFG = {l: ((3, mr) if shape == 0 else (shape, mr)) for l, (shape, mr) in DEFAULT_ACTIVE_CFG.items()}
 
     def force_active_tiles(self, active_cfg=None):
         if self.ta is None:
@@ -446,7 +452,14 @@
                    [int(lib.sessd_conv2d_sk_workspace_bytes(B, self.H, self.W, 256, 1, 0))])
         if self.sk_ws is None or self.sk_ws.numel() < need:
             self.sk_ws = torch.zeros(need, dtype=torch.uint8, device=self.dev)
-        self.active_cfg = dict(self.DEFAULT_ACTIVE_CFG if active_cfg is None else active_cfg)
+        cfg = dict(self.DEFAULT_ACTIVE_CFG if active_cfg is None else active_cfg)
+        for l, (shape, mr) in cfg.items():
+            if l in self.ACTIVE_SK or l == self.ACTIVE_PAIR:
+                continue
+            layers = self.ACTIVE_SLOTS[l][1] if l == self.ACTIVE_CONV else (self.ACTIVE_SLOTS[l][1],)
+            if any(pc.upk_sk(shape) is None for pc, _, _ in layers):
+                raise ValueError("active-tile layer %s: no stream-K Winograd packing for shape %d" % (self.ACTIVE_SLOTS[l][0], shape))
+        self.active_cfg = cfg
         return self.active_cfg
 
     def autotune(self, candidates=(1, 2, 3, 4, 6, 11, 12), reps=5):
@@ -497,7 +510,7 @@
                     cands.append(20)
                     if pc.cin % 32 == 0:
                         cands.append(21)
-                    for cfg, shape in ((22, 0), (23, 1)) if self.allow_streamk else ():
+                    for cfg, shape in ((22, 0), (23, 1)) + (((25, 3),) if WINO_SPLIT else ()) if self.allow_streamk else ():
                         if pc.upk_sk(shape) is not None:
                             need = int(lib.sessd_conv3x3_winograd_sk_workspace_bytes(x.shape[0], x.shape[2], x.shape[3], pc.cout, shape, 0))
                             if self.sk_ws is None or self.sk_ws.numel() < need:
@@ -581,13 +594,13 @@
             if l == self.ACTIVE_CONV:
                 (p0, s0, t0_), (p1, s1, t1_) = layer
                 c01 = self.tile_cfg.get("conv_0")
-                if self.merge_branch_convs and c01 in (22, 23, 24) and self.tile_cfg.get("conv_1") == c01 and self._branch_sets(c01 - 22) is not None:
+                if self.merge_branch_convs and c01 in (22, 23, 24, 25) and self.tile_cfg.get("conv_1") == c01 and self._branch_sets(c01 - 22) is not None:
                     sets = self._branch_sets(c01 - 22)
                     dense_t = timed(lambda: ops.conv2d_winograd_sk_sets(t["mid"], sets["upk"], 2, 128, sets["scale"], sets["shift"], True, t["o"],
                                                                         c01 - 22, self.sk_ws, self._wgs(c01 - 22)))
                 else:
                     dense_t = self.tune_report.get("conv_0", (None, 0.0))[1] + self.tune_report.get("conv_1", (None, 0.0))[1]
-                for shape in (0, 1):
+                for shape in WINO_LIST_SHAPES:
                     if p0.upk_sk(shape) is None or p1.upk_sk(shape) is None:
                         continue
                     need = int(lib.sessd_conv3x3_winograd_sk_workspace_bytes(self.B, self.H, self.W, p0.cout, shape, 0))
@@ -624,7 +637,7 @@
                         if tt < best[1]:
                             best = ((30, mr), tt)
             else:
-                for shape in (0, 1):
+                for shape in WINO_LIST_SHAPES:
                     if pc.upk_sk(shape) is None:
                         continue
                     need = int(lib.sessd_conv3x3_winograd_sk_workspace_bytes(self.B, x_in.shape[2], x_in.shape[3], pc.cout, shape, 0))
@@ -840,7 +853,7 @@
                 e1.record()
                 self._kmarks.append(("conv_0+conv_1", e0, e1))
             o0, o1 = t["o0"], t["o1"]
-        elif self.merge_branch_convs and c01 in (22, 23, 24) and self.tile_cfg.get("conv_1") == c01 and self._tuning is None \
+        elif self.merge_branch_convs and c01 in (22, 23, 24, 25) and self.tile_cfg.get("conv_1") == c01 and self._tuning is None \
                 and self.sk_ws is not None and self._branch_sets(c01 - 22) is not None:
             sets = self._branch_sets(c01 - 22)
             if self._kmarks is not None:
diff --git a/se-ssd_amd/sessd_hip/ops.py b/se-ssd_amd/sessd_hip/ops.py
--- a/se-ssd_amd/sessd_hip/ops.py
+++ b/se-ssd_amd/sessd_hip/ops.py
@@ -613,7 +613,7 @@
             if j["kind"] == 0:
                 total = (j["cin"] // 2) * len(j["taps"]) * 2 * cp
             else:
-                cpad = cp if j["layout"] == 0 else ((j["cout"] + 127) // 128 * 128 if j["layout"] == 1 else (j["cout"] + 63) // 64 * 64)
+                cpad = cp if j["layout"] == 0 else ((j["cout"] + 127) // 128 * 128 if j["layout"] in (1, 4) else (j["cout"] + 63) // 64 * 64)
                 total = cpad * j["cin"]
         else:
             a.kv, a.cin, a.cout, a.adjoint, a.reverse_k = j["kv"], j["cin"], j["cout"], j["adjoint"], j["reverse_k"]
@@ -1141,7 +1141,7 @@
         self.cin, self.cout, self.kind, self.stride = cin, cout, kind, stride
         self._w3 = None
         self._upk = None
-        self._upk_sk = [None, None, None]
+        self._upk_sk = [None, None, None, None]
         self._sk = None
         self._registry = None
 
@@ -1153,7 +1153,7 @@
         return self._upk
 
     def upk_sk(self, shape):
-        if self._upk_sk[shape] is None and self._w3 is not None and self.cin % (16, 8, 16)[shape] == 0:
+        if self._upk_sk[shape] is None and self._w3 is not None and self.cin % (16, 8, 16, 16)[shape] == 0:
             make = lambda: pack_winograd_sk(self._w3[0], shape, adjoint=self._w3[1])
             self._upk_sk[shape] = self._registry.create(make) if self._registry is not None else make()
         return self._upk_sk[shape]
@@ -1243,6 +1243,8 @@
         out = torch.empty((ci // 2, 4, 2, (co + 31) // 32 * 32, 4), dtype=torch.float32, device=w.device)
     elif layout == 3:
         out = torch.empty(((co + 127) // 128, ci // 2, 4, 2, 32, 16), dtype=torch.float32, device=w.device)
+    elif layout == 4:
+        out = torch.empty(((co + 127) // 128, 8, ci // 2, 3, 64, 8), dtype=torch.bfloat16, device=w.device)
     else:
         nw, c = ((8, 128), (4, 64))[layout - 1]
         out = torch.empty(((co + c - 1) // c, ci // 2, nw, 2, 32, c // 32, 16 // nw), dtype=torch.float32, device=w.device)
@@ -1475,11 +1477,12 @@
         th, tw = H, W
     if out is None:
         out = torch.empty((B, pc.cout, Ho, Wo), dtype=torch.float32, device=x.device)
-    if tile_cfg in (22, 23, 24):
+    if tile_cfg in (22, 23, 24, 25):
         shape = tile_cfg - 22
         upk = pc.upk_sk(shape) if pc.kind == "conv" else None
         if upk is None or (H & 1) or (W & 1):
-            raise ValueError("tile_cfg 22/23/24 (stream-K Winograd) needs a 3x3 stride-1 conv with cin % 16 (22, 24) / 8 (23) == 0 and even H, W")
+            raise ValueError("tile_cfg 22/23/24/25 (stream-K Winograd) needs a 3x3 stride-1 conv with cin % 16 (22, 24, 25) / 8 (23) == 0 "
+                             "and even H, W")
         if workspace is None:
             key = (x.device.index, _cache_scope(), shape, workgroups)
             need = int(lib.sessd_conv3x3_winograd_sk_workspace_bytes(B, H, W, pc.cout, shape, workgroups))
```

Measured after the change: 2087 (median of 6 runs). 1.05x the previous value.
